# moxime/joint-vae

Hardware: NVIDIA B200
Metric: train_images_per_sec (higher is better)
Workload: dtype bf16

## Files before the change

### include/jvae_b200.h

```cpp
#ifndef JVAE_B200_H
#define JVAE_B200_H

#include <stdint.h>
#include <stddef.h>

#ifdef __cplusplus
extern "C" {
#endif

#define JVAE_ABI_VERSION 16

enum jvae_status {
  JVAE_OK = 0,
  JVAE_ERR_INVALID = -1,
  JVAE_ERR_CUDA = -2,
  JVAE_ERR_UNSUPPORTED = -3,
  JVAE_ERR_NOGPU = -4
};

enum jvae_dtype { JVAE_F32 = 0, JVAE_BF16 = 1 };

enum jvae_var_dim { JVAE_VAR_SCALAR = 0, JVAE_VAR_DIAG = 1, JVAE_VAR_FULL = 2 };
enum jvae_prior_kind { JVAE_PRIOR_GAUSSIAN = 0, JVAE_PRIOR_TILTED = 1, JVAE_PRIOR_UNIFORM = 2 };

// ... 93 lines not shown

int jvae_conv_gather_gemm(const void* in, int N, int H, int W, int Cin, int ld_in, const void* wmat, int Cout_pad, int ldw,
                          int ntaps, const int16_t* tap_dy, const int16_t* tap_dx, int in_stride, int Hq, int Wq,
                          void* out, int Ho, int Wo, int Cout, int ld_out, int out_sy, int out_sx, int out_oy, int out_ox,
                          const float* bias, int act, double* stats, void* stream);
typedef struct jvae_bn_reduce {
  const void* y;
  int32_t ld_y;
  const float* save_mean_rstd;
  const float* gamma;
  const float* beta;
  int32_t act;
} jvae_bn_reduce;
int jvae_conv_gather_gemm_bn(const void* in, int N, int H, int W, int Cin, int ld_in, const void* wmat, int Cout_pad, int ldw,
                             int ntaps, const int16_t* tap_dy, const int16_t* tap_dx, int in_stride, int Hq, int Wq,
                             void* out, int Ho, int Wo, int Cout, int ld_out, int out_sy, int out_sx, int out_oy, int out_ox,
                             const float* bias, int act, double* stats, const jvae_bn_reduce* bn, int* bn_fused, void* stream);
#define JVAE_NOT_COVERED 1
int jvae_conv_subpixel_gemm(const void* in, int N, int H, int W, int Cin, int ld_in, const void* wmat, int Cout_pad, int ldw,
                            int nphases, const int16_t* phase_ntaps, const int16_t* phase_oy, const int16_t* phase_ox,
                            const int16_t* tap_dy, const int16_t* tap_dx, int Hq, int Wq, void* out, int Ho, int Wo, int Cout,
                            int ld_out, int out_s, const float* bias, int act, double* stats, void* stream);
int jvae_conv_halo_emulate(const float* in, int N, int H, int W, int Cin, int ld_in, const float* wmat, int Cout_pad, int ldw,
                           int nphases, const int16_t* phase_ntaps, const int16_t* phase_oy, const int16_t* phase_ox, int ntaps,
                           const int16_t* tap_dy, const int16_t* tap_dx, int in_stride, int Hq, int Wq, float* out, int Ho, int Wo,
                           int Cout, int ld_out, int out_sy, int out_sx, int out_oy, int out_ox, const float* bias, int act,
                           int* info);
int jvae_conv_wgrad_emulate(const float* dy, int N, int Hq, int Wq, int Cout, int ld_dy, const float* x, int H, int W, int Cin, int ld_x,
                            int ntaps, const int16_t* tap_dy, const int16_t* tap_dx, int in_stride, float* dw, int dw_ld_tap,
                            int dw_ld_co, int dw_ld_ci, int* launches);
int jvae_conv_wgrad(const void* dy, int N, int Hq, int Wq, int Cout, int ld_dy, const void* x, int H, int W, int Cin, int ld_x,
                    int ntaps, const int16_t* tap_dy, const int16_t* tap_dx, int in_stride, float* dw, int dw_ld_tap,
                    int dw_ld_co, int dw_ld_ci, void* stream);
enum jvae_conv_kernel { JVAE_KERNEL_CONV_HALO = 1, JVAE_KERNEL_CONV_TAPBOX = 2, JVAE_KERNEL_WGRAD_HALO = 3, JVAE_KERNEL_WGRAD_TAPBOX = 4 };
int jvae_last_conv_kernel(void);


int jvae_bn_stats(const void* y, size_t P, int C, int ld, double* stats, void* stream);
int jvae_bn_apply_fwd(const void* y, size_t P, int C, int ld_y, const double* stats, const float* gamma, const float* beta,
                      float eps, float momentum, float* running_mean, float* running_var, int64_t* num_batches, int training,
                      int act, void* out, int ld_out, float* save_mean_rstd, void* stream);
int jvae_bn_bwd(const void* da, int ld_da, const void* y, int ld_y, size_t P, int C, const float* save_mean_rstd,
                const float* gamma, const float* beta, int act, double* sums, void* dy, int ld_dy, float* dgamma, float* dbeta,
                int skip_reduce, void* stream);
int jvae_act_bwd(const void* da, int ld_da, const void* a_out, int ld_a, size_t P, int C, int act, void* dy, int ld_dy,
                 float* dbias, void* stream);
int jvae_maxpool_fwd(const void* in, int N, int H, int W, int C, int ld_in, int k, int stride, void* out, int ld_out, void* stream);
int jvae_maxpool_bwd(const void* in, int N, int H, int W, int C, int ld_in, int k, int stride, const void* dout, int ld_dout,
                     void* din, int ld_din, void* stream);
int jvae_maxpool_pad_fwd(const void* in, int N, int H, int W, int C, int ld_in, int k, int stride, int pad, void* out,
                         int ld_out, void* stream);
int jvae_maxpool_pad_bwd(const void* in, int N, int H, int W, int C, int ld_in, int k, int stride, int pad, const void* dout,
                         int ld_dout, void* din, int ld_din, void* stream);
int jvae_avgpool(const void* src, int ld_src, void* dst, int ld_dst, int N, int H, int W, int C, int k, int backward,
                 void* stream);
int jvae_vsum_rows(const void* T, int ld_t, int N, int H, int W, int k, int pad, int Co, const float* bias, int act, double* stats,
                   void* out, int ld_out, void* stream);
int jvae_vstack_rows(const void* dy, int ld_dy, int N, int H, int W, int k, int pad, int Co, void* U, int ld_u, void* stream);
int jvae_add_act(const void* a, int ld_a, const void* b, int ld_b, size_t P, int C, int act, void* out, int ld_out,
                 void* stream);
int jvae_upsample2(const void* src, int ld_src, void* dst, int ld_dst, int N, int H, int W, int C, int backward, void* stream);

int jvae_cast_f32_bf16(const float* src, void* dst, size_t n, void* stream);
int jvae_cast_bf16_f32(const void* src, float* dst, size_t n, void* stream);
int jvae_im2col_bf16(const void* x, int N, int H, int W, int C, int ld_x, int ntaps, const int16_t* tap_dy, const int16_t* tap_dx,
                     int in_stride, int Hq, int Wq, void* out, int ld_out, int tap_major, void* stream);
int jvae_nchw_to_nhwc_bf16(const float* src, void* dst, int n, int c, int h, int w, int c_pad, void* stream);
int jvae_nhwc_bf16_to_nchw(const void* src, float* dst, int n, int c, int h, int w, int c_pad, void* stream);

typedef struct jvae_pack_job {
  const float* src;
  void* dst;
  int64_t s_r1, s_r0, s_t, s_c1, s_c0;
  int32_t rows, rows_pad, R0;
// ... 41 lines not shown
```

### joint-vae_b200/_native.py

```python
import ctypes
import os

import torch

_HERE = os.path.dirname(os.path.abspath(__file__))
LIB_PATH = os.path.join(_HERE, 'libjvae_sm100.so')

F32, BF16 = 0, 1
VAR_DIM = {'scalar': 0, 'diag': 1, 'full': 2}
PRIOR_KIND = {'gaussian': 0, 'tilted': 1, 'uniform': 2}
ACT = {'none': 0, 'linear': 0, 'relu': 1, 'sigmoid': 2, 'leaky': 3}
OUT_F32, IN_F32 = 0x100, 0x200
LEAKY_SLOPE = 0.01
NSCORES, NPRED = 16, 4
SCORE_INDEX = {'elbo': 0, 'max': 0, 'sum': 1, 'mean': 2, 'iws': 3, 'soft': 4, 'softkl': 4, 'zdist': 5, 'kl': 6,
               'mse': 7, 'wmse': 8, 'logits': 9, 'baseline': 10, 'hyz': 11, 'std': 12, 'softiws': 13}
PRED_INDEX = {'loss': 0, 'esty': 1, 'closest': 2, 'iws': 3}

c_void_p, c_int, c_float, c_size_t = ctypes.c_void_p, ctypes.c_int, ctypes.c_float, ctypes.c_size_t
c_u64, c_i64 = ctypes.c_uint64, ctypes.c_int64


class ElboCfg(ctypes.Structure):
    _fields_ = [(n, ctypes.c_int32) for n in
                ('B', 'L', 'K', 'C', 'D', 'xreco_dtype', 'logits_dtype', 'var_dim', 'prior_kind', 'conditional',
                 'has_xreco', 'has_logits', 'sigma_is_log', 'sigma_is_rmse')] + \
               [(n, ctypes.c_float) for n in ('beta', 'gamma_w', 'var_w', 'tau', 'alpha')] + \
               [(n, ctypes.c_int32) for n in ('prior_stats_ready', 'categorical', 'cat_group', 'sigma_per_sample')]


class BnReduce(ctypes.Structure):
    _fields_ = [('y', ctypes.c_void_p), ('ld_y', ctypes.c_int32), ('save_mean_rstd', ctypes.c_void_p),
                ('gamma', ctypes.c_void_p), ('beta', ctypes.c_void_p), ('act', ctypes.c_int32)]


class BatchCfg(ctypes.Structure):
    _fields_ = [(n, ctypes.c_int32) for n in ('H', 'W', 'C', 'out_H', 'out_W', 'crop_pad', 'flip_first', 'post_off_y',
                                              'post_off_x')]


class PackJob(ctypes.Structure):
    _fields_ = [('src', ctypes.c_void_p), ('dst', ctypes.c_void_p)] + \
               [(n, ctypes.c_int64) for n in ('s_r1', 's_r0', 's_t', 's_c1', 's_c0')] + \
               [(n, ctypes.c_int32) for n in ('rows', 'rows_pad', 'R0', 'T', 'tap_off', 'cols', 'cols_pad', 'C0', 'dst_f32',
                                              'first_block')]


class NativeError(RuntimeError):
    pass


_lib = None


def lib():
    global _lib
    if _lib is not None:
        return _lib
    if not os.path.exists(LIB_PATH):
        raise NativeError(f'{LIB_PATH} is not built: run `python -c "import __graft_entry__ as g; g.build()"` '
                          'in a container with nvcc; there is no CPU fallback')
    L = ctypes.CDLL(LIB_PATH)
    L.jvae_last_error.restype = ctypes.c_char_p
    L.jvae_abi_version.restype = c_int
    L.jvae_launch_count.restype = c_i64
    L.jvae_device_info.argtypes = [c_int, ctypes.POINTER(c_int), ctypes.POINTER(c_int), ctypes.POINTER(c_int)]
    L.jvae_elbo_workspace_bytes.restype = c_size_t
    L.jvae_elbo_workspace_bytes.argtypes = [ctypes.POINTER(ElboCfg)]
    P = c_void_p
    L.jvae_elbo_train_fwd.argtypes = [ctypes.POINTER(ElboCfg)] + [P] * 19 + [c_size_t, P]
    L.jvae_elbo_train_bwd.argtypes = [ctypes.POINTER(ElboCfg)] + [P] * 19 + [c_size_t, P]
    L.jvae_elbo_eval_fwd.argtypes = [ctypes.POINTER(ElboCfg)] + [P] * 23 + [c_size_t, P]
    L.jvae_sample_fwd.argtypes = [c_int, c_int, c_int, P, P, c_u64, c_u64, P, c_int, c_int, P, P, P, P, P, P, P]
    L.jvae_sample_bwd.argtypes = [c_int, c_int, c_int, P, P, P, P, c_int, P, P, c_int, P, P]
    L.jvae_cast_f32_bf16.argtypes = [P, P, c_size_t, P]
    L.jvae_cast_bf16_f32.argtypes = [P, P, c_size_t, P]
    L.jvae_nchw_to_nhwc_bf16.argtypes = [P, P, c_int, c_int, c_int, c_int, c_int, P]
    L.jvae_nhwc_bf16_to_nchw.argtypes = [P, P, c_int, c_int, c_int, c_int, c_int, P]
    L.jvae_grad_sqnorm.argtypes = [P, c_int, c_size_t, P, P, P, P]
    L.jvae_adam_step.argtypes = [P, P, P, P, c_int, c_size_t, P, c_float, c_float, c_float, c_float, c_float,
                                 c_float, c_int, P, P, P, P, c_float, P]
    for name in ('jvae_gemm_bf16', 'jvae_selftest'):
        if not hasattr(L, name):
            raise NativeError(f'{LIB_PATH} does not export {name}: stale build')
    L.jvae_gemm_bf16.argtypes = [c_int, c_int, c_int, c_int, P, c_int, P, c_int, P, c_int, P, P, c_int, P, c_int, P]
    L.jvae_selftest.argtypes = [c_int]
    L.jvae_probe_descriptors.argtypes = [c_int]
    L.jvae_probe_poison.argtypes = [ctypes.c_uint, P]
    L.jvae_profile_enable.argtypes = [c_int]
    L.jvae_im2col_bf16.argtypes = [P, c_int, c_int, c_int, c_int, c_int, c_int, ctypes.POINTER(ctypes.c_int16), ctypes.POINTER(ctypes.c_int16), c_int, c_int, c_int, P, c_int, c_int, P]
    L.jvae_profile_drain.argtypes = [P, P, c_int]
    I16P = ctypes.POINTER(ctypes.c_int16)
    L.jvae_conv_gather_gemm.argtypes = [P, c_int, c_int, c_int, c_int, c_int, P, c_int, c_int, c_int, I16P, I16P, c_int,
                                        c_int, c_int, P, c_int, c_int, c_int, c_int, c_int, c_int, c_int, c_int, P, c_int,
                                        P, P]
    L.jvae_conv_gather_gemm_bn.argtypes = [P, c_int, c_int, c_int, c_int, c_int, P, c_int, c_int, c_int, I16P, I16P, c_int,
                                           c_int, c_int, P, c_int, c_int, c_int, c_int, c_int, c_int, c_int, c_int, P,
                                           c_int, P, ctypes.POINTER(BnReduce), ctypes.POINTER(c_int), P]
    L.jvae_conv_wgrad.argtypes = [P, c_int, c_int, c_int, c_int, c_int, P, c_int, c_int, c_int, c_int, c_int, I16P, I16P,
                                  c_int, P, c_int, c_int, c_int, P]
    L.jvae_conv_subpixel_gemm.argtypes = [P, c_int, c_int, c_int, c_int, c_int, P, c_int, c_int, c_int, I16P, I16P, I16P, I16P,
                                          I16P, c_int, c_int, P, c_int, c_int, c_int, c_int, c_int, P, c_int, P, P]
    L.jvae_conv_wgrad_emulate.argtypes = [P, c_int, c_int, c_int, c_int, c_int, P, c_int, c_int, c_int, c_int, c_int, I16P, I16P,
                                          c_int, P, c_int, c_int, c_int, ctypes.POINTER(c_int)]
    L.jvae_conv_halo_emulate.argtypes = [P, c_int, c_int, c_int, c_int, c_int, P, c_int, c_int, c_int, I16P, I16P, I16P, c_int,
                                         I16P, I16P, c_int, c_int, c_int, P, c_int, c_int, c_int, c_int, c_int, c_int, c_int,
                                         c_int, P, c_int, ctypes.POINTER(c_int)]
    L.jvae_bn_stats.argtypes = [P, c_size_t, c_int, c_int, P, P]
    L.jvae_bn_apply_fwd.argtypes = [P, c_size_t, c_int, c_int, P, P, P, c_float, c_float, P, P, P, c_int, c_int, P, c_int,
                                    P, P]
    L.jvae_bn_bwd.argtypes = [P, c_int, P, c_int, c_size_t, c_int, P, P, P, c_int, P, P, c_int, P, P, c_int, P]
    L.jvae_act_bwd.argtypes = [P, c_int, P, c_int, c_size_t, c_int, c_int, P, c_int, P, P]
    L.jvae_maxpool_fwd.argtypes = [P, c_int, c_int, c_int, c_int, c_int, c_int, c_int, P, c_int, P]
    L.jvae_maxpool_bwd.argtypes = [P, c_int, c_int, c_int, c_int, c_int, c_int, c_int, P, c_int, P, c_int, P]
    L.jvae_upsample2.argtypes = [P, c_int, P, c_int, c_int, c_int, c_int, c_int, c_int, P]
    L.jvae_maxpool_pad_fwd.argtypes = [P, c_int, c_int, c_int, c_int, c_int, c_int, c_int, c_int, P, c_int, P]
    L.jvae_maxpool_pad_bwd.argtypes = [P, c_int, c_int, c_int, c_int, c_int, c_int, c_int, c_int, P, c_int, P, c_int, P]
    L.jvae_avgpool.argtypes = [P, c_int, P, c_int, c_int, c_int, c_int, c_int, c_int, c_int, P]
    L.jvae_add_act.argtypes = [P, c_int, P, c_int, c_size_t, c_int, c_int, P, c_int, P]
    L.jvae_vsum_rows.argtypes = [P, c_int, c_int, c_int, c_int, c_int, c_int, c_int, P, c_int, P, P, c_int, P]
    L.jvae_vstack_rows.argtypes = [P, c_int, c_int, c_int, c_int, c_int, c_int, c_int, P, c_int, P]
    L.jvae_elbo_prior_stats.argtypes = [ctypes.POINTER(ElboCfg), P, P, P, c_size_t, P]
    L.jvae_batch_u8_to_f32.argtypes = [ctypes.POINTER(BatchCfg), P, ctypes.c_longlong, P, c_int, P, P, P, P]
    L.jvae_last_conv_kernel.restype = c_int
    L.jvae_pack_job_blocks.argtypes = [ctypes.c_longlong, c_int, c_int]
    L.jvae_pack_weights.argtypes = [P, c_int, P, c_int, P]
    if L.jvae_abi_version() != 16:
        raise NativeError('ABI version mismatch between _native.py and libjvae_sm100.so')
    _lib = L
    return L

# ... 400 lines not shown
        pn = poy = pox = None
        dy, dx = taps
        T, nph = len(dy), 0
    rc = lib().jvae_conv_halo_emulate(hp(inp), N, H, W, Cin, ld_in, hp(wmat), Cout_pad, wmat.shape[1], nph, pn, poy, pox, T, dy, dx,
                                      in_stride, Hq, Wq, hp(out), Ho, Wo, Cout, ld_out, out_s[0], out_s[1], out_o[0], out_o[1],
                                      hp(bias), act, info)
    if rc == NOT_COVERED:
        return None
    check(rc)
    return list(info)


def conv_wgrad_emulate(dy, Cout, x, Cin, taps, in_stride, dw, dw_ld_tap, dw_ld_co, dw_ld_ci=1):
    for t in (dy, x, dw):
        assert t.device.type == 'cpu' and t.dtype == torch.float32 and t.is_contiguous()
    N, Hq, Wq, ld_dy = dy.shape
    _, H, W, ld_x = x.shape
    n = c_int(0)
    rc = lib().jvae_conv_wgrad_emulate(c_void_p(dy.data_ptr()), N, Hq, Wq, Cout, ld_dy, c_void_p(x.data_ptr()), H, W, Cin, ld_x,
                                       len(taps[0]), taps[0], taps[1], in_stride, c_void_p(dw.data_ptr()), dw_ld_tap, dw_ld_co,
                                       dw_ld_ci, ctypes.byref(n))
    if rc == NOT_COVERED:
        return None
    check(rc)
    return n.value


def conv_wgrad(dy, N, Hq, Wq, Cout, ld_dy, x, H, W, Cin, ld_x, taps, in_stride, dw, dw_ld_tap, dw_ld_co, dw_ld_ci=1):
    with _timed_conv(2.0 * N * Hq * Wq * len(taps[0]) * Cin * Cout):
        check(lib().jvae_conv_wgrad(rawptr(dy), N, Hq, Wq, Cout, ld_dy, rawptr(x), H, W, Cin, ld_x, len(taps[0]), taps[0],
                                    taps[1], in_stride, rawptr(dw), dw_ld_tap, dw_ld_co, dw_ld_ci, stream()))


def bn_stats(y, P, C, ld, stats):
    check(lib().jvae_bn_stats(rawptr(y), P, C, ld, rawptr(stats), stream()))


def bn_apply_fwd(y, P, C, ld_y, stats, gamma, beta, eps, momentum, running_mean, running_var, num_batches, training, act,
                 out, ld_out, save):
    check(lib().jvae_bn_apply_fwd(rawptr(y), P, C, ld_y, rawptr(stats), rawptr(gamma), rawptr(beta), float(eps),
                                  float(momentum), rawptr(running_mean), rawptr(running_var), rawptr(num_batches),
                                  int(training), act, rawptr(out), ld_out, rawptr(save), stream()))


def bn_bwd(da, ld_da, y, ld_y, P, C, save, gamma, beta, act, sums, dy, ld_dy, dgamma, dbeta, skip_reduce=False):
    check(lib().jvae_bn_bwd(rawptr(da), ld_da, rawptr(y), ld_y, P, C, rawptr(save), rawptr(gamma), rawptr(beta), act,
                            rawptr(sums), rawptr(dy), ld_dy, rawptr(dgamma), rawptr(dbeta), int(skip_reduce), stream()))


def act_bwd(da, ld_da, a_out, ld_a, P, C, act, dy, ld_dy, dbias):
    check(lib().jvae_act_bwd(rawptr(da), ld_da, rawptr(a_out), ld_a, P, C, act, rawptr(dy), ld_dy, rawptr(dbias), stream()))


def maxpool_fwd(inp, N, H, W, C, ld_in, k, stride, out, ld_out):
    check(lib().jvae_maxpool_fwd(rawptr(inp), N, H, W, C, ld_in, k, stride, rawptr(out), ld_out, stream()))


def maxpool_bwd(inp, N, H, W, C, ld_in, k, stride, dout, ld_dout, din, ld_din):
    check(lib().jvae_maxpool_bwd(rawptr(inp), N, H, W, C, ld_in, k, stride, rawptr(dout), ld_dout, rawptr(din), ld_din,
                                 stream()))


def upsample2(src, ld_src, dst, ld_dst, N, H, W, C, backward=False):
    check(lib().jvae_upsample2(rawptr(src), ld_src, rawptr(dst), ld_dst, N, H, W, C, int(backward), stream()))


# ... 29 lines not shown
```

### joint-vae_b200/conv_engine.py

```python
import os

import torch
from torch import nn

from . import _native as nat
from . import engine


def r8(n):
    return (n + 7) & ~7


def cblk_of(c):
    return 64 if c > 32 else (32 if c > 16 else 16)


def cout_pad_of(c):
    return ((c + 255) // 256) * 256 if c > 256 else ((c + 15) // 16) * 16


_ACT_CODE = {nn.ReLU: 1, nn.Sigmoid: 2, nn.Identity: 0, nn.LeakyReLU: 3}

import os as _os
FUSE_BN_REDUCE = _os.environ.get('JVAE_FUSE_BN_REDUCE', '0') == '1'
DENSE_SMALL = _os.environ.get('JVAE_CONV_DENSE_SMALL', '0') == '1'
SEP_FWD_DIRECT = _os.environ.get('JVAE_HEAD_FWD_DIRECT', '1') != '0'
IM2COL_MAXPIX = int(_os.environ.get('JVAE_CONV_IM2COL_MAXPIX', '16'))


class NativeKernels:
    act_dtype = torch.bfloat16

    @staticmethod
    def empty(shape, like, dtype=torch.bfloat16):
        return torch.empty(shape, dtype=dtype, device=like.device)

    @staticmethod
    def zeros(shape, like, dtype=torch.float32):
        return torch.zeros(shape, dtype=dtype, device=like.device)

    @staticmethod
    def to_nhwc(x, c_pad):
        n, c, h, w = x.shape
        x = x.float().contiguous()
        if h * w == 1 and c_pad == c:
            return nat.cast_f32_bf16(x).view(n, 1, 1, c)
        return nat.nchw_to_nhwc_bf16(x, c_pad)

    @staticmethod
    def to_nchw(t, C):
        n, h, w, ld = t.shape
        if h * w == 1 and ld == C:
            return nat.cast_bf16_f32(t).view(n, C, 1, 1)
        return nat.nhwc_bf16_to_nchw(t, C)

    @staticmethod
    def gather(x, Cin, wmat, cout_pad, taps, in_stride, Hq, Wq, out, Cout, out_s, out_o, bias, act, stats, bn=None):
        N, H, W, ld_in = x.shape
        _, Ho, Wo, ld_out = out.shape
        return nat.conv_gather_gemm(x, N, H, W, Cin, ld_in, wmat, cout_pad, wmat.shape[1], taps, in_stride, Hq, Wq, out, Ho,
                                    Wo, Cout, ld_out, out_s, out_o, bias, act, stats, bn=bn)

    @staticmethod
    def wgrad(g, Cg, x, Cx, taps, in_stride, dw, swapped=False):
        N, Hq, Wq, ld_g = g.shape
        _, H, W, ld_x = x.shape
        T = len(taps[0])
        P = N * Hq * Wq
        small = Hq * Wq <= IM2COL_MAXPIX and Cx % 8 == 0 and Cg >= 128 and Cx >= 64 and T in (1, 4, 9, 25)
        if not swapped and small and dw.is_contiguous():
            cols = torch.empty((P, Cx * T), dtype=torch.bfloat16, device=g.device)
            nat.im2col(x, N, H, W, Cx, ld_x, taps, in_stride, Hq, Wq, cols)
            tiles = ((Cg + 127) // 128) * ((Cx * T + 127) // 128)
            ksplit = max(1, min(nat.sm_count() // tiles, (P + 511) // 512)) if tiles < 100 else 1
            nat.gemm_bf16(2, Cg, Cx * T, P, g.view(P, ld_g), ld_g, cols, Cx * T, out_f32=dw.view(Cg, Cx * T), ldd=Cx * T,
                          accumulate=ksplit if ksplit > 1 else True)
            return
        if swapped:
            nat.conv_wgrad(g, N, Hq, Wq, Cg, ld_g, x, H, W, Cx, ld_x, taps, in_stride, dw, 1, T, Cg * T)
        else:
            nat.conv_wgrad(g, N, Hq, Wq, Cg, ld_g, x, H, W, Cx, ld_x, taps, in_stride, dw, 1, Cx * T, T)

    @staticmethod
    def gemm(mode, M, N, K, a, b, bias=None, act=0, out_bf16=None, out_f32=None):
        nat.gemm_bf16(mode, M, N, K, a, a.stride(0), b, b.stride(0), bias=bias, act=act, out_bf16=out_bf16, out_f32=out_f32,
                      ldd=N)

    @staticmethod
    def phases_arg(ops):
        return nat.phases_arg(ops)

    @staticmethod
    def subpixel(x, Cin, wmat, cout_pad, phases, Hq, Wq, out, Cout, out_s, bias, act, stats):
        N, H, W, ld_in = x.shape
        _, Ho, Wo, ld_out = out.shape
        return nat.conv_subpixel_gemm(x, N, H, W, Cin, ld_in, wmat, cout_pad, wmat.shape[1], phases, Hq, Wq, out, Ho, Wo, Cout,
                                      ld_out, out_s, bias, act, stats)

    bn_stats = staticmethod(nat.bn_stats)
    bn_apply_fwd = staticmethod(nat.bn_apply_fwd)
    bn_bwd = staticmethod(nat.bn_bwd)
    act_bwd = staticmethod(nat.act_bwd)
    maxpool_fwd = staticmethod(nat.maxpool_fwd)
    maxpool_bwd = staticmethod(nat.maxpool_bwd)
    upsample2 = staticmethod(nat.upsample2)
    maxpool_pad_fwd = staticmethod(nat.maxpool_pad_fwd)
    maxpool_pad_bwd = staticmethod(nat.maxpool_pad_bwd)
    avgpool = staticmethod(nat.avgpool)
    add_act = staticmethod(nat.add_act)
    vsum_rows = staticmethod(nat.vsum_rows)
    vstack_rows = staticmethod(nat.vstack_rows)
    taps_arg = staticmethod(nat.taps_arg)


K = NativeKernels


def conv_form(k, p, s, Hq, Wq):
    taps = [(i - p, j - p) for i in range(k) for j in range(k)]
    return [dict(taps=taps, idx=list(range(k * k)), in_stride=s, Hq=Hq, Wq=Wq, out_s=(1, 1), out_o=(0, 0))]


def deconv_form(k, p, s, Ho, Wo, allow_empty=False):
    ops = []
    for fy in range(s):
        rows = [i for i in range(k) if (fy + p - i) % s == 0]
        for fx in range(s):
            cols = [j for j in range(k) if (fx + p - j) % s == 0]
            Hq, Wq = (Ho - fy + s - 1) // s, (Wo - fx + s - 1) // s
            if Hq <= 0 or Wq <= 0:
                continue
            if not rows or not cols:
                if allow_empty:
# ... 261 lines not shown
            if self.Ci % 8:
                t = torch.zeros((kk * self.Co, r8(self.Ci)), dtype=torch.bfloat16, device=w.device)
                t[:, :self.Ci] = d['bm']
                d['bm'] = t[:, :self.Ci]
            d['bias'] = b0.repeat(kk).contiguous() if b0 is not None else None
        else:
            if self.transposed:
                g_f = wd.permute(1, 2, 3, 0).reshape(self.Co, kk, self.Ci)
                g_b = wd.permute(0, 2, 3, 1).reshape(self.Ci, kk, self.Co)
            else:
                g_f = wd.permute(0, 2, 3, 1).reshape(self.Co, kk, self.Ci)
                g_b = wd.permute(1, 2, 3, 0).reshape(self.Ci, kk, self.Co)
            d['fwd'] = [pack_gather_weights(g_f, op['idx'], self.Ci) for op in self.fwd_ops]
            if self.merged_fwd:
                d['fwd_all'] = pack_gather_weights(g_f, self.fwd_all_idx, self.Ci)
            if self.dense_small:
                hw = self.H * self.W
                weff = torch.zeros((hw, self.Co, hw, self.Ci), dtype=torch.float32, device=w.device)
                for q, r, ty, tx in self.dense_pairs:
                    weff[q, :, r, :] = wd[:, :, ty, tx]
                d['dense'] = weff.view(hw * self.Co, hw * self.Ci).to(torch.bfloat16).contiguous()
                d['dense_bias'] = b0.repeat(hw).contiguous() if b0 is not None else None
            if self.separable:
                kq = self.k
                d['sep_fwd'] = pack_gather_weights(wd.permute(2, 0, 3, 1).reshape(kq * self.Co, kq, self.Ci),
                                                   list(range(kq)), self.Ci)
                d['sep_bwd'] = pack_gather_weights(wd.permute(1, 3, 2, 0).reshape(self.Ci, kq, kq * self.Co),
                                                   list(range(kq)), kq * self.Co)
            if want_bwd:
                d['bwd'] = [pack_gather_weights(g_b, op['idx'], self.Co) for op in self.dgrad_ops]
        setattr(self, slot, (key, d))
        return d

    def forward(self, x, st, training):
        N = x.shape[0]
        bn = self.bn
        bn_train = bn is not None and (training or not bn.track_running_stats)
        if bn is not None and not bn_train:
            return self._forward_folded(x, st)
        pk = self._pack()
        bias = self.conv.bias.detach() if self.conv.bias is not None else None
        fused_act = self.act if bn is None else 0
        y = K.empty((N, self.Ho, self.Wo, self.ld_y), x)
        stats = (st.pop('stats_buf', None) if bn_train else None)
        if bn_train and stats is None:
            stats = K.zeros((2, self.Co), x, torch.float64)
        if self.gemm1x1:
            kk = self.k * self.k
            a2 = x.view(N, x.shape[-1])
            K.gemm(nat.GEMM_NT, N, kk * self.Co, self.Ci, a2, pk['bm'], bias=pk['bias'], act=fused_act,
                   out_bf16=y.view(N, kk * self.Co))
            if bn_train:
                K.bn_stats(y, N * kk, self.Co, self.ld_y, stats)
        elif self.dense_small:
            hw = self.H * self.W
            K.gemm(nat.GEMM_NT, N, hw * self.Co, hw * self.Ci, x.view(N, hw * self.Ci), pk['dense'], bias=pk['dense_bias'],
                   act=fused_act, out_bf16=y.view(N, hw * self.Co))
            if bn_train:
                K.bn_stats(y, N * hw, self.Co, self.ld_y, stats)
        elif self.separable and not SEP_FWD_DIRECT:
            self._sep_forward(x, pk, bias, fused_act, stats, y)
        elif not self._merged_forward(x, pk, y, bias, fused_act, stats):
            for i, (op, wm) in enumerate(zip(self.fwd_ops, pk['fwd'])):
                K.gather(x, self.Ci, wm, wm.shape[0], self._taps(('f', i), op['taps']), op['in_stride'], op['Hq'], op['Wq'],
                         y, self.Co, op['out_s'], op['out_o'], bias, fused_act, stats)
        st['x'] = x
        if bn is None:
            st['a'] = y
            return y
        P = N * self.Ho * self.Wo
        a = K.empty((N, self.Ho, self.Wo, self.ld_a), x)
        save = K.empty((2, self.Co), x, torch.float32) if bn_train else None
        track = bn.track_running_stats and training
        K.bn_apply_fwd(y, P, self.Co, self.ld_y, stats, bn.weight.detach() if bn.affine else None,
                       bn.bias.detach() if bn.affine else None, bn.eps, bn.momentum if bn.momentum is not None else 0.1,
                       bn.running_mean if track or not bn_train else None, bn.running_var if track or not bn_train else None,
                       bn.num_batches_tracked if track else None, bn_train, self.act, a, self.ld_a, save)
        if track:
            engine.bump_stats()
        st['y'], st['save'], st['bn_train'] = y, save, bn_train
        return a

    def _merged_forward(self, x, pk, out, bias, act, stats):
        if not self.merged_fwd:
            return False
        ph = self._ctaps.get('fa')
        if ph is None:
            ph = self._ctaps['fa'] = K.phases_arg(self.fwd_ops)
        wm = pk['fwd_all']
        op = self.fwd_ops[0]
        return K.subpixel(x, self.Ci, wm, wm.shape[0], ph, op['Hq'], op['Wq'], out, self.Co, self.s, bias, act, stats)

    def _sep_forward(self, x, pk, bias, act, stats, out):
        N = x.shape[0]
        T = K.empty((N, self.H, self.W, self.sep_ld), x, torch.float32)
        wm = pk['sep_fwd']
        K.gather(x, self.Ci, wm, wm.shape[0], self._taps('sf', self.sep_fwd_taps), 1, self.H, self.W, T, self.sep_C, (1, 1),
                 (0, 0), None, nat.OUT_F32, None)
        K.vsum_rows(T, self.sep_ld, N, self.H, self.W, self.k, self.p, self.Co, bias, act | nat.IN_F32, stats, out,
                    out.shape[-1])

    def _forward_folded(self, x, st):
        N = x.shape[0]
        pk = self._pack(fold_bn=True)
        a = K.empty((N, self.Ho, self.Wo, self.ld_a), x)
        if self.gemm1x1:
            kk = self.k * self.k
            K.gemm(nat.GEMM_NT, N, kk * self.Co, self.Ci, x.view(N, x.shape[-1]), pk['bm'], bias=pk['bias'], act=self.act,
                   out_bf16=a.view(N, kk * self.Co))
        elif self.dense_small:
            hw = self.H * self.W
            K.gemm(nat.GEMM_NT, N, hw * self.Co, hw * self.Ci, x.view(N, hw * self.Ci), pk['dense'], bias=pk['dense_bias'],
                   act=self.act, out_bf16=a.view(N, hw * self.Co))
        elif self.separable and not SEP_FWD_DIRECT:
            self._sep_forward(x, pk, pk['b'], self.act, None, a)
        elif not self._merged_forward(x, pk, a, pk['b'], self.act, None):
            for i, (op, wm) in enumerate(zip(self.fwd_ops, pk['fwd'])):
                K.gather(x, self.Ci, wm, wm.shape[0], self._taps(('f', i), op['taps']), op['in_stride'], op['Hq'], op['Wq'],
                         a, self.Co, op['out_s'], op['out_o'], pk['b'], self.act, None)
        st['x'], st['a'], st['bn_train'], st['folded'] = x, a, False, True
        return a

    def backward(self, da, st, need_dx, prev_bn=None):
        x = st['x']
        N = x.shape[0]
        P = N * self.Ho * self.Wo
        bn = self.bn
        grads = {}
        folded = bool(st.get('folded'))
        if folded:
            a = st['a']
            if self.act == 0 and da.shape[-1] % 8 == 0:
                dy = da
            else:
                dy = K.zeros((N, self.Ho, self.Wo, r8(self.Co)), x, torch.bfloat16) if r8(self.Co) != self.Co \
                    else K.empty((N, self.Ho, self.Wo, self.Co), x)
                K.act_bwd(da, da.shape[-1], a, a.shape[-1], P, self.Co, self.act, dy, dy.shape[-1], None)
        elif bn is not None:
            y = st['y']
            dy = K.empty(y.shape, x)
            pre = st.get('bn_sums')
            sums = pre if pre is not None else K.empty((2, self.Co), x, torch.float64)
            dg = db = lg = lb = None
            if bn.affine:
                lg, lb = _live_grad(bn.weight, x), _live_grad(bn.bias, x)
                dg = lg if lg is not None else K.zeros((self.Co,), x)
                db = lb if lb is not None else K.zeros((self.Co,), x)
            K.bn_bwd(da, da.shape[-1], y, self.ld_y, P, self.Co, st['save'], bn.weight.detach() if bn.affine else None,
                     bn.bias.detach() if bn.affine else None, self.act, sums, dy, self.ld_y, dg, db,
                     **({'skip_reduce': True} if pre is not None else {}))
            grads['bn_w'], grads['bn_b'] = (None if lg is not None else dg), (None if lb is not None else db)
            grads['b'] = K.zeros((self.Co,), x) if (self.conv.bias is not None and
                                                     _live_grad(self.conv.bias, x) is None) else None
        else:
            lbias = _live_grad(self.conv.bias, x)
            dbias = lbias if lbias is not None else (K.zeros((self.Co,), x) if self.conv.bias is not None else None)
            if self.act == 0 and da.shape[-1] % 8 == 0:
# ... 21 lines not shown
            if need_dx:
                ldx = x.shape[-1]
                if ldx == self.Ci:
                    dx = K.empty(x.shape, x)
                    K.gemm(nat.GEMM_NN, N, self.Ci, kk * self.Co, dy2, pk['bm'], out_bf16=dx.view(N, ldx))
                else:
                    tmp = K.empty((N, self.Ci), x, torch.float32)
                    K.gemm(nat.GEMM_NN, N, self.Ci, kk * self.Co, dy2, pk['bm'], out_f32=tmp)
                    dx = K.zeros(x.shape, x, torch.bfloat16)
                    dx.view(N, ldx)[:, :self.Ci] = tmp
        elif self.dense_small:
            hw = self.H * self.W
            dy2, x2 = dy.view(N, hw * self.Co), x.view(N, hw * self.Ci)
            if not folded:
                dweff = K.empty((hw * self.Co, hw * self.Ci), x, torch.float32)
                K.gemm(nat.GEMM_TN, hw * self.Co, hw * self.Ci, N, dy2, x2, out_f32=dweff)
                dw4 = dweff.view(hw, self.Co, hw, self.Ci)
                w = self.conv.weight
                live = _live_grad(w, x)
                dw = live if live is not None else K.zeros(tuple(w.shape), x)
                for q, r, ty, tx in self.dense_pairs:
                    dw[:, :, ty, tx] += dw4[q, :, r, :]
                grads['w'] = None if live is not None else dw
            if need_dx:
                dx = K.empty(x.shape, x)
                K.gemm(nat.GEMM_NN, N, hw * self.Ci, hw * self.Co, dy2, pk['dense'], out_bf16=dx.view(N, hw * self.Ci))
        elif self.separable:
            kq = self.k
            U = K.empty((N, self.H, self.W, self.sep_ld), x)
            K.vstack_rows(dy, dy.shape[-1], N, self.H, self.W, kq, self.p, self.Co, U, self.sep_ld)
            if not folded:
                dwa = K.zeros((self.sep_C, self.Ci, kq), x)
                if cblk_of(self.sep_C) < cblk_of(min(self.Ci, 64)):
                    K.wgrad(x, self.Ci, U, self.sep_C, self._taps('sb', self.sep_bwd_taps), 1, dwa, swapped=True)
                else:
                    K.wgrad(U, self.sep_C, x, self.Ci, self._taps('sf', self.sep_fwd_taps), 1, dwa)
                upd = dwa.view(kq, self.Co, self.Ci, kq).permute(1, 2, 0, 3)
                live = _live_grad(self.conv.weight, x)
                if live is not None:
                    live.add_(upd)
                grads['w'] = None if live is not None else upd.contiguous()
            if need_dx:
                dx = K.empty(x.shape, x)
                wm = pk['sep_bwd']
                K.gather(U, self.sep_C, wm, wm.shape[0], self._taps('sb', self.sep_bwd_taps), 1, self.H, self.W, dx, self.Ci,
                         (1, 1), (0, 0), None, 0, None)
        else:
            w = self.conv.weight
            if not folded:
                live = _live_grad(w, x)
                dw = live if live is not None else K.zeros(tuple(w.shape), x)
                if self.transposed:
                    K.wgrad(x, self.Ci, dy, self.Co, self._taps('w', self.wgrad_taps), self.s, dw.view(self.Ci, self.Co, kk))
                elif self.wgrad_swapped:
                    K.wgrad(x, self.Ci, dy, self.Co, self._taps('wn', self.wgrad_taps_neg), 1, dw.view(self.Co, self.Ci, kk),
                            swapped=True)
                else:
                    K.wgrad(dy, self.Co, x, self.Ci, self._taps('w', self.wgrad_taps), self.s, dw.view(self.Co, self.Ci, kk))
                grads['w'] = None if live is not None else dw
            if need_dx:
                dx = K.zeros(x.shape, x, torch.bfloat16) if self.dgrad_sparse else K.empty(x.shape, x)
                fuse = FUSE_BN_REDUCE and prev_bn is not None and K is NativeKernels and \
                    prev_bn['y'].shape[:3] == dx.shape[:3]
                sums_prev = K.zeros((2, self.Ci), x, torch.float64) if fuse else None
                done = fuse
                for i, (op, wm) in enumerate(zip(self.dgrad_ops, pk['bwd'])):
                    r = K.gather(dy, self.Co, wm, wm.shape[0], self._taps(('b', i), op['taps']), op['in_stride'], op['Hq'],
                                 op['Wq'], dx, self.Ci, op['out_s'], op['out_o'], None, 0, sums_prev,
                                 **({'bn': prev_bn} if fuse else {}))
                    done = done and bool(r)
                if fuse and done:
                    prev_bn['sums'] = sums_prev
        out = [grads['w'], grads['b']]
        if bn is not None:
            out += [grads['bn_w'], grads['bn_b']]
        return dx, out


class PoolStep:

    def __init__(self, mod, in_shape):
        ks = mod.kernel_size if isinstance(mod.kernel_size, int) else mod.kernel_size[0]
        stv = mod.stride if isinstance(mod.stride, int) else mod.stride[0]
        pad = mod.padding if isinstance(mod.padding, int) else mod.padding[0]
        if mod.ceil_mode or mod.dilation not in (1, (1, 1)) or 2 * pad > ks:
            raise NotImplementedError('MaxPool2d with ceil_mode / dilation has no native kernel')
        self.k, self.s, self.p = ks, stv, pad
        self.general = pad != 0 or stv < ks
        self.C, self.H, self.W = in_shape
        self.Ho, self.Wo = (self.H + 2 * pad - ks) // stv + 1, (self.W + 2 * pad - ks) // stv + 1
        self.out_shape = (self.C, self.Ho, self.Wo)
# ... 216 lines not shown
            elif g[0] == 'avg':
                stp = AvgStep(g[1], shape)
            elif g[0] == 'res':
                stp = ResidualStep(g[1], shape)
            else:
                stp = UpStep(g[1], shape)
            steps.append(stp)
            shape = stp.out_shape
        self.steps = steps
        self.out_shape = shape
        self.parameters = [p for s in steps for p in s.params()]
        convs = []
        for stp in steps:
            if isinstance(stp, ConvStep):
                convs.append(stp)
            elif isinstance(stp, ResidualStep):
                convs += stp.chain + ([stp.ds] if stp.ds is not None else [])
        self.plan = PackPlan(convs)
        for c in convs:
            c.plan = self.plan

    def forward(self, x, training):
        C, H, W = self.in_shape
        N = x.shape[0]
        if K is NativeKernels and training:
            self.plan.ensure()
        t = K.to_nhwc(x.reshape(N, C, H, W), r8(C))
        state = []
        bn_steps = [s for s in self.steps if isinstance(s, ConvStep) and s.bn is not None and
                    (training or not s.bn.track_running_stats)]
        pool, off = None, 0
        if bn_steps:
            pool = K.zeros((sum(2 * s.Co for s in bn_steps),), t, torch.float64)
        for s in self.steps:
            st = {}
            if pool is not None and any(s is b for b in bn_steps):
                st['stats_buf'] = pool[off:off + 2 * s.Co].view(2, s.Co)
                off += 2 * s.Co
            t = s.forward(t, st, training)
            state.append(st)
        Co, Ho, Wo = self.out_shape
        if self.image_out and t.shape[-1] == Co:
            out = t.permute(0, 3, 1, 2)
        else:
            out = K.to_nchw(t, Co)
        return out, state, t.shape[-1]

    def backward(self, dout, state, ld_last, need_dx):
        Co, Ho, Wo = self.out_shape
        N = dout.shape[0]
        if self.image_out and ld_last == Co:
            g = dout
            if g.dtype != K.act_dtype:
                g = g.to(K.act_dtype)
            g = g.permute(0, 2, 3, 1)
            if not g.is_contiguous():
                g = g.contiguous()
        else:
            g = K.to_nhwc(dout, ld_last)
        grads = []
        for idx in range(len(self.steps) - 1, -1, -1):
            s = self.steps[idx]
            kw = {}
            prev = self.steps[idx - 1] if idx > 0 else None
            if isinstance(s, ConvStep) and isinstance(prev, ConvStep) and prev.bn is not None and \
                    state[idx - 1].get('bn_train') and not s.gemm1x1:
                pb = prev.bn
                kw['prev_bn'] = dict(y=state[idx - 1]['y'], ld_y=prev.ld_y, save=state[idx - 1]['save'],
                                     gamma=pb.weight.detach() if pb.affine else None,
                                     beta=pb.bias.detach() if pb.affine else None, act=prev.act)
            g, pg = s.backward(g, state[idx], need_dx or idx > 0, **kw)
            if 'prev_bn' in kw and kw['prev_bn'].get('sums') is not None:
# ... 56 lines not shown
```

### joint-vae_b200/csrc/common.cuh

```cuda
#pragma once
#include <cuda_runtime.h>
#include <cuda_bf16.h>
#include <cuda.h>
#include <stdint.h>
#include <stdio.h>
#include <string.h>
#include <atomic>

#include "../../include/jvae_b200.h"

namespace jvae {

void set_error(const char* fmt, ...);
extern std::atomic<long long> g_launches;
inline void count_launch(int n = 1) { g_launches.fetch_add(n, std::memory_order_relaxed); }

#define JVAE_CHECK_ARG(cond, msg)                                                   \
  do {                                                                              \
    if (!(cond)) {                                                                  \
      jvae::set_error("%s: invalid argument: %s (%s)", __func__, msg, #cond);       \
      return JVAE_ERR_INVALID;                                                      \
    }                                                                               \
  } while (0)

// ... 20 lines not shown

void* prof_begin(int tag, cudaStream_t st);
void prof_end(void* h, cudaStream_t st);

__device__ __forceinline__ float warp_sum(float v) {
#pragma unroll
  for (int o = 16; o > 0; o >>= 1) v += __shfl_xor_sync(0xffffffffu, v, o);
  return v;
}
__device__ __forceinline__ float warp_max(float v) {
#pragma unroll
  for (int o = 16; o > 0; o >>= 1) v = fmaxf(v, __shfl_xor_sync(0xffffffffu, v, o));
  return v;
}

__device__ __forceinline__ float block_sum(float v, float* red) {
  const int lane = threadIdx.x & 31, wid = threadIdx.x >> 5, nw = (blockDim.x + 31) >> 5;
  v = warp_sum(v);
  __syncthreads();
  if (lane == 0) red[wid] = v;
  __syncthreads();
  float r = (lane < nw) ? red[lane] : 0.f;
  r = warp_sum(r);
  return r;
}

__device__ __forceinline__ float bf16_lo(uint32_t u) { return __uint_as_float(u << 16); }
__device__ __forceinline__ float bf16_hi(uint32_t u) { return __uint_as_float(u & 0xffff0000u); }
__device__ __forceinline__ uint32_t pack_bf16(float a, float b) {
  __nv_bfloat162 t = __floats2bfloat162_rn(a, b);
  return *reinterpret_cast<uint32_t*>(&t);
}

__device__ __forceinline__ uint4 ld_stream16(const void* p) {
  uint4 r;
  asm volatile("ld.global.nc.L1::no_allocate.v4.u32 {%0,%1,%2,%3}, [%4];"
               : "=r"(r.x), "=r"(r.y), "=r"(r.z), "=r"(r.w) : "l"(p));
  return r;
}
__device__ __forceinline__ void st_stream16(void* p, uint4 v) {
  asm volatile("st.global.L1::no_allocate.v4.u32 [%0], {%1,%2,%3,%4};"
               :: "l"(p), "r"(v.x), "r"(v.y), "r"(v.z), "r"(v.w) : "memory");
}

}
```

### joint-vae_b200/csrc/conv.cu

```cuda
#include "tc_common.cuh"
#include <vector>
#include <algorithm>
#include <stdlib.h>

namespace jvae {

constexpr int CONV_THREADS = 192;
constexpr int CONV_MAX_TAPS = 64;
static thread_local int g_last_conv_kernel = 0;

struct ConvParams {
  int N, Hq, Wq;
  int TW, TH, NB;
  int tiles_x, tiles_y, tiles_n, num_tiles, n_tiles_n;
  int Cblk, nCk, ntaps;
  int in_stride;
  short dy[CONV_MAX_TAPS], dx[CONV_MAX_TAPS];
  int BN;
  int Ho, Wo, Cout, ldc;
  int out_sy, out_sx, out_oy, out_ox;
  int act;
  int out_f32;
  const float* bias;
  __nv_bfloat16* out;
// ... 222 lines not shown
        const int ch = i % p.cout_pad;
        const double val = s_stats[i];
        if (ch < p.Cout && val != 0.0) atomicAdd(&p.stats[(i / p.cout_pad) * p.Cout + ch], val);
      }
    }
  }
  tc_fence_before();
  __syncthreads();
  if (warp == 1) tmem_dealloc_dyn(tmem_base, p.tmem_cols);
}

constexpr int HALO_MAX_CK = 128;
struct HaloParams {
  int N, Hq, Wq;
  int RT, NBt, HHs, HWp, MT;
  int strips_x, blocks_y, blocks_n, num_boxes, n_tiles_n;
  int Cblk, ntaps, BN;
  int nkc;
  int dymin, dxmin;
  int in_stride, nplanes;
  short plane_ry[4], plane_rx[4];
  uint32_t plane_bytes;
  short dy[CONV_MAX_TAPS], dx[CONV_MAX_TAPS];
  uint32_t tap_off16[CONV_MAX_TAPS];
  int Ho, Wo, Cout, ldc, out_sy, out_sx, out_oy, out_ox, act;
  int out_f32;
  const float* bias;
  __nv_bfloat16* out;
  double* stats;
  int cout_pad;
  const __nv_bfloat16* bn_y;
  const float* bn_save; const float* bn_gamma; const float* bn_beta;
  int bn_ld, bn_act;
  uint32_t stage_bytes, box_bytes, w_tap_bytes, w_bytes, tmem_cols, acc_stride;
  int stages, resident, wstages;
  int G, nck;
  int PH;
  short ph_oy[4], ph_ox[4];
  uint4 ck[HALO_MAX_CK];
  short w_pos[CONV_MAX_TAPS];
};

__device__ __forceinline__ int2 lds_int2(uint32_t addr) {
  int2 v;
  asm volatile("ld.shared.v2.s32 {%0, %1}, [%2];" : "=r"(v.x), "=r"(v.y) : "r"(addr));
  return v;
}

__device__ __forceinline__ uint64_t desc64(uint32_t hi, uint32_t lo) {
  uint64_t d;
  asm("mov.b64 %0, {%1, %2};" : "=l"(d) : "r"(lo), "r"(hi));
  return d;
}

template <int KSTEPS, int MT>
__device__ __forceinline__ void halo_mma_box(const HaloParams& p, uint32_t d0, uint32_t a_hi, uint32_t a_lo0, uint32_t m_step16,
                                             uint32_t b_hi, uint32_t b_lo_base, uint32_t w_tap16, uint32_t idesc,
                                             uint64_t* wfull_bar, uint64_t* wempty_bar, uint32_t& ws, uint32_t& wph,
                                             uint32_t later_chunk) {
  uint32_t b_lo = b_lo_base;
  for (int t = 0; t < p.ntaps; ++t) {
    if (!p.resident) {
      mbar_wait(&wfull_bar[ws], wph);
      tc_fence_after();
      b_lo = b_lo_base + ws * w_tap16;
    }
    const uint32_t a_lo = a_lo0 + p.tap_off16[t];
    const uint32_t acc_first = (t != 0) | later_chunk;
#pragma unroll
    for (int m = 0; m < MT; ++m)
#pragma unroll
      for (int k = 0; k < KSTEPS; ++k)
        umma_bf16(d0 + (uint32_t)(m * p.BN), desc64(a_hi, a_lo + (uint32_t)m * m_step16 + 2u * k), desc64(b_hi, b_lo + 2u * k), idesc,
                  k == 0 ? acc_first : 1u);
    if (p.resident) {
      b_lo += w_tap16;
    } else {
      umma_commit(&wempty_bar[ws]);
      if (++ws == (uint32_t)p.wstages) { ws = 0; wph ^= 1; }
    }
  }
}

template <int KSTEPS>
__device__ __forceinline__ void halo_mma_box_g(const HaloParams& p, uint32_t d0, uint32_t a_hi, uint32_t a_lo0, uint32_t m_step16,
                                               uint32_t b_hi, uint32_t b_lo_base, uint32_t idesc0, uint32_t later_chunk) {
  const uint32_t gbn = (uint32_t)(p.G * p.PH * p.BN);
  for (int m = 0; m < p.MT; ++m) {
    const uint32_t a_m = a_lo0 + (uint32_t)m * m_step16;
    const uint32_t d_m = d0 + (uint32_t)m * gbn;
    for (int c = 0; c < p.nck; ++c) {
      const uint4 ck = p.ck[c];
      const uint32_t a_lo = a_m + ck.x, b_lo = b_lo_base + ck.y;
      const uint32_t d = d_m + (ck.w & 0x7fffffffu);
      const uint32_t idesc = ck.z;
      const uint32_t acc0 = ((ck.w >> 31) ^ 1u) | later_chunk;
#pragma unroll
      for (int k = 0; k < KSTEPS; ++k)
        umma_bf16(d, desc64(a_hi, a_lo + 2u * k), desc64(b_hi, b_lo + 2u * k), idesc, k == 0 ? acc0 : 1u);
    }
  }
}

template <int NCH, int MODE>
__device__ __forceinline__ void halo_epilogue_fast(const HaloParams& p, uint32_t tmem_base, uint64_t* tfull_bar, uint64_t* tempty_bar,
                                                   double* s_stats, const float* s_bias, const float* s_bn, int2* s_tab, int warp,
                                                   int lane, int nt, int box0, int box_step) {
  constexpr bool STATS = MODE != 0;
  constexpr bool BNRED = MODE == 2;
  constexpr int LC = (NCH + 1) / 2;
  const int set = (warp - 2) >> 2;
  const int q = warp & 3;
  const int mrow = q * 32 + lane;
  const int ch0 = nt * p.BN;
  const int per = p.G * p.PH;
  const int nblk = p.MT * per;
  const int c_first = NCH == 1 ? 0 : set;
  for (int i = threadIdx.x - 64; i < nblk * 16; i += 256) {
    const int blk = i >> 4;
    const int m = blk / per, r = blk - m * per;
    const int j = r / p.PH, ph = r - j * p.PH;
    const int slot = (m * 16 + (i & 15)) * p.G + j;
    const int nb = slot / p.HHs, yy = slot - nb * p.HHs;
    const bool valid = nb < p.NBt && yy < p.RT;
    s_tab[i] = make_int2(valid ? (nb * p.Ho + yy * p.out_sy + p.ph_oy[ph]) * p.Wo + p.ph_ox[ph] : -1,
                         yy | (nb << 16));
  }
  asm volatile("bar.sync 1, 256;" ::: "memory");
  float s1[STATS ? LC * 16 : 1], s2[STATS ? LC * 16 : 1];
  if (STATS) {
#pragma unroll
    for (int j = 0; j < LC * 16; ++j) s1[j] = s2[j] = 0.f;
  }
  const bool has_bias = p.bias != nullptr;
  const uint32_t sb = smem_u32(s_bias);
  const uint32_t stab = smem_u32(s_tab) + 8u * (uint32_t)(mrow >> 3);
  const bool vec_bf16 = (p.ldc & 7) == 0, vec_f32 = (p.ldc & 3) == 0;
  const bool al32 = (reinterpret_cast<uintptr_t>(p.out) & 31) == 0;
  const bool v8_bf16 = al32 && (p.ldc & 15) == 0, v8_f32 = al32 && (p.ldc & 7) == 0;
  uint32_t it = 0;
  int sx, by, mm, dsx, dby, dmm;
  {
    int t = box0;
    sx = t % p.strips_x; t /= p.strips_x;
    by = t % p.blocks_y; mm = t / p.blocks_y;
    t = box_step;
    dsx = t % p.strips_x; t /= p.strips_x;
    dby = t % p.blocks_y; dmm = t / p.blocks_y;
  }
  for (int box = box0; box < p.num_boxes; box += box_step, ++it) {
    const uint32_t acc = it & 1;
    if (it != 0) {
      sx += dsx;
      if (sx >= p.strips_x) { sx -= p.strips_x; ++by; }
      by += dby;
      if (by >= p.blocks_y) { by -= p.blocks_y; ++mm; }
      mm += dmm;
    }
    const int qx = sx * 8 + (mrow & 7);
    const bool pxok = qx < p.Wq;
    const int ylim = p.Hq - by * p.RT, nlim = p.N - mm * p.NBt;
    const size_t pix0 = ((size_t)(mm * p.NBt) * p.Ho + (size_t)(by * p.RT * p.out_sy + p.out_oy)) * p.Wo +
                        (size_t)(qx * p.out_sx + p.out_ox);
    mbar_wait(&tfull_bar[acc], (it >> 1) & 1);
    tc_fence_after();
    constexpr int BSTEP = NCH == 1 ? 2 : 1;
    int2 e_next = lds_int2(stab + 8u * (uint32_t)(NCH == 1 ? set : 0) * 16u);
    for (int blk = (NCH == 1 ? set : 0); blk < nblk; blk += BSTEP) {
      const int2 e = e_next;
      if (blk + BSTEP < nblk) e_next = lds_int2(stab + 8u * (uint32_t)(blk + BSTEP) * 16u);
      const bool ok = pxok && e.x >= 0 && (e.y & 0xffff) < ylim && (e.y >> 16) < nlim;
      if (!__any_sync(0xffffffffu, ok)) continue;
      const uint32_t t_addr = tmem_base + acc * p.acc_stride + (uint32_t)(blk * p.BN) + ((uint32_t)(q * 32) << 16);
      const size_t pix = pix0 + (size_t)(ok ? e.x : 0);
      uint4 yq[BNRED ? LC : 1][2];
      if (BNRED && ok) {
#pragma unroll
        for (int lc = 0; lc < LC; ++lc)
          if (c_first + 2 * lc < NCH && ch0 + (c_first + 2 * lc) * 16 < p.Cout) {
            const __nv_bfloat16* yp = p.bn_y + pix * (size_t)p.bn_ld + (size_t)(ch0 + (c_first + 2 * lc) * 16);
            yq[lc][0] = ld_stream16(yp);
            yq[lc][1] = ld_stream16(yp + 8);
          }
      }
      float bq[LC][16];
      if (has_bias) {
#pragma unroll
        for (int lc = 0; lc < LC; ++lc)
          if (c_first + 2 * lc < NCH) {
#pragma unroll
            for (int j = 0; j < 16; j += 4)
// ... 113 lines not shown
      int chn;
      const float t1 = warp_sum16(a, lane, &chn);
      const float t2 = warp_sum16(b, lane, &chn);
      if (c < NCH && (lane & 1) == 0 && ch0 + c * 16 + chn < p.Cout) {
        atomicAdd(&s_stats[ch0 + c * 16 + chn], (double)t1);
        atomicAdd(&s_stats[p.cout_pad + ch0 + c * 16 + chn], (double)t2);
      }
    }
    asm volatile("bar.sync 1, 256;" ::: "memory");
    const int t = threadIdx.x - 64;
    for (int i = t; i < 2 * p.cout_pad; i += 256) {
      const int ch = i % p.cout_pad;
      double val = s_stats[i];
      if (BNRED && i >= p.cout_pad && ch - ch0 >= 0 && ch - ch0 < p.BN)
        val = (double)s_bn[64 + ch - ch0] * (val - (double)s_bn[ch - ch0] * s_stats[ch]);
      if (ch < p.Cout && val != 0.0) atomicAdd(&p.stats[(i / p.cout_pad) * p.Cout + ch], val);
    }
  }
}

constexpr int HALO_THREADS = 320;
__global__ void __launch_bounds__(HALO_THREADS, 1)
conv_halo_kernel(const __grid_constant__ CUtensorMap tmap_in, const __grid_constant__ CUtensorMap tmap_w,
                 const __grid_constant__ HaloParams p) {
  extern __shared__ uint8_t smem_raw[];
  uint8_t* smem = reinterpret_cast<uint8_t*>((reinterpret_cast<uintptr_t>(smem_raw) + 1023) & ~(uintptr_t)1023);
  uint8_t* wsm = smem + (size_t)p.stages * p.stage_bytes;
  uint64_t* full_bar = reinterpret_cast<uint64_t*>(wsm + p.w_bytes);
  uint64_t* empty_bar = full_bar + 4;
  uint64_t* wfull_bar = empty_bar + 4;
  uint64_t* wempty_bar = wfull_bar + 8;
  uint64_t* tfull_bar = wempty_bar + 8;
  uint64_t* tempty_bar = tfull_bar + 2;
  uint32_t* tmem_slot = reinterpret_cast<uint32_t*>(tempty_bar + 2);
  double* s_stats = reinterpret_cast<double*>(tmem_slot + 4);
  float* s_bias = reinterpret_cast<float*>(s_stats + (p.stats ? 2 * p.cout_pad : 0));

  const int warp = threadIdx.x >> 5, lane = threadIdx.x & 31;
  const int nt = (int)blockIdx.x % p.n_tiles_n;
  float* s_bn = s_bias + 64;
  int2* s_tab = reinterpret_cast<int2*>(s_bn + 256);
  for (int i = threadIdx.x; i < p.BN; i += HALO_THREADS) {
    const int ch = nt * p.BN + i;
    s_bias[i] = (p.bias && ch < p.Cout) ? p.bias[ch] : 0.f;
    if (p.bn_y) {
      const bool live = ch < p.Cout;
      const float mean = live ? p.bn_save[ch] : 0.f, rstd = live ? p.bn_save[p.Cout + ch] : 0.f;
      const float g = (live && p.bn_gamma) ? p.bn_gamma[ch] : 1.f, b = (live && p.bn_beta) ? p.bn_beta[ch] : 0.f;
      s_bn[i] = mean; s_bn[64 + i] = rstd; s_bn[128 + i] = live ? g * rstd : 0.f; s_bn[192 + i] = live ? b - mean * g * rstd : 0.f;
    }
  }
  const int box0 = (int)blockIdx.x / p.n_tiles_n, box_step = (int)gridDim.x / p.n_tiles_n;
  const uint32_t rb = (uint32_t)p.Cblk * 2u;

  if (p.stats)
    for (int i = threadIdx.x; i < 2 * p.cout_pad; i += HALO_THREADS) s_stats[i] = 0.0;
  if (warp == 0 && lane == 0) {
    tma_prefetch_desc(&tmap_in);
    tma_prefetch_desc(&tmap_w);
    for (int s = 0; s < 4; ++s) { mbar_init(&full_bar[s], 1); mbar_init(&empty_bar[s], 1); }
    for (int s = 0; s < 8; ++s) { mbar_init(&wfull_bar[s], 1); mbar_init(&wempty_bar[s], 1); }
    for (int a = 0; a < 2; ++a) { mbar_init(&tfull_bar[a], 1); mbar_init(&tempty_bar[a], 8); }
    fence_barrier_init();
    fence_proxy_async();
  }
  if (warp == 1) tmem_alloc_dyn(tmem_slot, p.tmem_cols);
  tc_fence_before();
  __syncthreads();
  tc_fence_after();
  const uint32_t tmem_base = *tmem_slot;

  if (warp == 0) {
    if (elect_one()) {
      if (p.resident) {
        mbar_arrive_expect_tx(&wfull_bar[0], (uint32_t)(p.ntaps * p.nkc) * p.w_tap_bytes);
        for (int kc = 0; kc < p.nkc; ++kc)
          for (int t = 0; t < p.ntaps; ++t)
            tma_load_2d(wsm + (size_t)(kc * p.ntaps + (p.nck > 0 ? p.w_pos[t] : t)) * p.w_tap_bytes, &tmap_w, &wfull_bar[0],
                        (t * p.nkc + kc) * p.Cblk, nt * p.BN);
      }
      auto load_unit = [&](int box, int kc, uint32_t iu) {
        int m = box;
        const int sx = m % p.strips_x; m /= p.strips_x;
        const int by = m % p.blocks_y; m /= p.blocks_y;
        const int s = iu % p.stages;
        mbar_wait(&empty_bar[s], ((iu / p.stages) & 1) ^ 1);
        mbar_arrive_expect_tx(&full_bar[s], p.box_bytes);
        for (int pl = 0; pl < p.nplanes; ++pl)
          tma_load_4d(smem + (size_t)s * p.stage_bytes + (size_t)pl * p.plane_bytes, &tmap_in, &full_bar[s], kc * p.Cblk,
                      p.in_stride * (sx * 8 + p.dxmin) + p.plane_rx[pl], p.in_stride * (by * p.RT + p.dymin) + p.plane_ry[pl],
                      m * p.NBt);
      };
      uint32_t iu = 0, wit = 0;
      if (box0 < p.num_boxes) load_unit(box0, 0, 0);
      for (int box = box0; box < p.num_boxes; box += box_step) {
        for (int kc = 0; kc < p.nkc; ++kc, ++iu) {
          if (kc + 1 < p.nkc) load_unit(box, kc + 1, iu + 1);
          else if (box + box_step < p.num_boxes) load_unit(box + box_step, 0, iu + 1);
          if (!p.resident) {
            for (int t = 0; t < p.ntaps; ++t, ++wit) {
              const int ws = wit % p.wstages;
              mbar_wait(&wempty_bar[ws], ((wit / p.wstages) & 1) ^ 1);
              mbar_arrive_expect_tx(&wfull_bar[ws], p.w_tap_bytes);
              tma_load_2d(wsm + (size_t)ws * p.w_tap_bytes, &tmap_w, &wfull_bar[ws], (t * p.nkc + kc) * p.Cblk, nt * p.BN);
            }
          }
        }
      }
    }
  } else if (warp == 1) {
    if (elect_one()) {
      const uint32_t idesc = make_idesc_bf16(128, p.BN, false, false);
      const uint32_t swz = (p.Cblk == 64) ? SWZ_128B : (p.Cblk == 32 ? SWZ_64B : SWZ_32B);
      const uint32_t sbo_a = (uint32_t)(p.G * p.HWp) * rb, sbo_b = 8u * rb;
      const uint32_t a_hi = ((sbo_a >> 4) & 0x3fffu) | (1u << 14) | (swz << 29);
      const uint32_t b_hi = ((sbo_b >> 4) & 0x3fffu) | (1u << 14) | (swz << 29);
      const uint32_t m_step16 = (16u * sbo_a) >> 4, w_tap16 = p.w_tap_bytes >> 4;
      const int ksteps = p.Cblk >> 4;
      if (p.resident) { mbar_wait(&wfull_bar[0], 0); tc_fence_after(); }
      uint32_t it = 0, s = 0, sph = 0, ws = 0, wph = 0;
      for (int box = box0; box < p.num_boxes; box += box_step, ++it) {
        const uint32_t acc = it & 1;
        mbar_wait(&tempty_bar[acc], ((it >> 1) & 1) ^ 1);
        const uint32_t d0 = tmem_base + acc * p.acc_stride;
        const uint32_t b_lo = ((smem_u32(wsm) >> 4) & 0x3fffu) | (1u << 16);
        for (int kc = 0; kc < p.nkc; ++kc) {
          mbar_wait(&full_bar[s], sph);
          tc_fence_after();
          const uint32_t a_lo0 = ((smem_u32(smem + (size_t)s * p.stage_bytes) >> 4) & 0x3fffu) | (1u << 16);
          const uint32_t later = kc != 0;
#define HALO_BOX(KS, M) halo_mma_box<KS, M>(p, d0, a_hi, a_lo0, m_step16, b_hi, b_lo, w_tap16, idesc, wfull_bar, wempty_bar, ws, wph, later)
#define HALO_BOX_M(KS)                                                                 \
          switch (p.MT) {                                                              \
            case 1: HALO_BOX(KS, 1); break;                                            \
            case 2: HALO_BOX(KS, 2); break;                                            \
            case 3: HALO_BOX(KS, 3); break;                                            \
            case 4: HALO_BOX(KS, 4); break;                                            \
            default: HALO_BOX(KS, 5); break;                                           \
          }
          if (p.nck > 0) {
            const uint32_t idesc0 = make_idesc_bf16(128, 0, false, false);
            const uint32_t b_kc = b_lo + (uint32_t)(kc * p.ntaps) * w_tap16;
            if (ksteps == 2) halo_mma_box_g<2>(p, d0, a_hi, a_lo0, m_step16, b_hi, b_kc, idesc0, later);
            else if (ksteps == 4) halo_mma_box_g<4>(p, d0, a_hi, a_lo0, m_step16, b_hi, b_kc, idesc0, later);
            else halo_mma_box_g<1>(p, d0, a_hi, a_lo0, m_step16, b_hi, b_kc, idesc0, later);
          } else if (ksteps == 2) { HALO_BOX_M(2) } else if (ksteps == 4) { HALO_BOX_M(4) } else { HALO_BOX_M(1) }
#undef HALO_BOX_M
#undef HALO_BOX
          umma_commit(&empty_bar[s]);
          if (++s == (uint32_t)p.stages) { s = 0; sph ^= 1; }
        }
        umma_commit(&tfull_bar[acc]);
      }
    }
  } else {
#define HALO_EPI_FAST(NCH_)                                                                                                            \
    if (p.bn_y) halo_epilogue_fast<NCH_, 2>(p, tmem_base, tfull_bar, tempty_bar, s_stats, s_bias, s_bn, s_tab, warp, lane, nt, box0, box_step);    \
    else if (p.stats) halo_epilogue_fast<NCH_, 1>(p, tmem_base, tfull_bar, tempty_bar, s_stats, s_bias, s_bn, s_tab, warp, lane, nt, box0, box_step); \
    else halo_epilogue_fast<NCH_, 0>(p, tmem_base, tfull_bar, tempty_bar, s_stats, s_bias, s_bn, s_tab, warp, lane, nt, box0, box_step)
    switch (p.BN >> 4) {
      case 1: HALO_EPI_FAST(1); break;
      case 2: HALO_EPI_FAST(2); break;
      case 3: HALO_EPI_FAST(3); break;
      default: HALO_EPI_FAST(4); break;
    }
#undef HALO_EPI_FAST
  }
  tc_fence_before();
  __syncthreads();
  if (warp == 1) tmem_dealloc_dyn(tmem_base, p.tmem_cols);
}

struct WgradParams {
  int N, Hq, Wq, TW, TH, NB, tiles_x, tiles_y, tiles_n, num_tiles;
  int Cblk_y, Cblk_x;
  int Cy, Cx, ncx;
  int ntaps, tap0, taps_per_cta, in_stride;
  short dy[CONV_MAX_TAPS], dx[CONV_MAX_TAPS];
  float* dw;
  int dw_ld_tap, dw_ld_co, dw_ld_cx;
  uint32_t stage_bytes, a_bytes, tx_bytes, tmem_cols;
  int stages;
};

__global__ void __launch_bounds__(CONV_THREADS, 1)
conv_wgrad_kernel(const __grid_constant__ CUtensorMap tmap_dy, const __grid_constant__ CUtensorMap tmap_x,
                  const __grid_constant__ WgradParams p) {
  extern __shared__ uint8_t smem_raw[];
  uint8_t* smem = reinterpret_cast<uint8_t*>((reinterpret_cast<uintptr_t>(smem_raw) + 1023) & ~(uintptr_t)1023);
  uint64_t* full_bar = reinterpret_cast<uint64_t*>(smem + (size_t)p.stages * p.stage_bytes);
  uint64_t* empty_bar = full_bar + p.stages;
  uint64_t* done_bar = empty_bar + p.stages;
  uint32_t* tmem_slot = reinterpret_cast<uint32_t*>(done_bar + 1);
  const int warp = threadIdx.x >> 5, lane = threadIdx.x & 31;
  const int tap_lo = p.tap0 + blockIdx.y * p.taps_per_cta;
  const int ntap = min(p.taps_per_cta, p.ntaps - tap_lo);
  const int cy0 = ((int)blockIdx.z / p.ncx) * p.Cblk_y, cx0 = ((int)blockIdx.z % p.ncx) * p.Cblk_x;
  const int M_real = min(p.Cblk_y, p.Cy - cy0), N_real = min(p.Cblk_x, p.Cx - cx0);

// ... 78 lines not shown
          float* o = p.dw + (size_t)(tap_lo + t) * p.dw_ld_tap + (size_t)(cy0 + row) * p.dw_ld_co + (size_t)(cx0 + c0) * p.dw_ld_cx;
#pragma unroll
          for (int j = 0; j < 16; ++j)
            if (c0 + j < N_real) atomicAdd(o + (size_t)j * p.dw_ld_cx, __uint_as_float(r[j]));
        }
      }
    }
  }
  tc_fence_before();
  __syncthreads();
  if (warp == 1) tmem_dealloc_dyn(tmem_base, p.tmem_cols);
}

constexpr int WH_MAX_GROUPS = 64;
struct WHaloParams {
  int N, Hq, Wq;
  int NBt, HHs, HWp, MT, strips_x, num_boxes;
  int RT, blocks_y;
  uint32_t g_img_bytes;
  int Cblk_g, Cblk_x, ncx, Cg, Cx;
  int ngroups, groups_per_cta;
  int dymin, dxmin, ey;
  int in_stride, nplanes;
  short plane_ry[4], plane_rx[4];
  uint32_t plane_bytes;
  uint32_t grp_off16[WH_MAX_GROUPS];
  unsigned char grp_ntap[WH_MAX_GROUPS];
  unsigned char grp_nv[WH_MAX_GROUPS];
  uint32_t grp_boff16[WH_MAX_GROUPS];
  uint32_t grp_idesc[WH_MAX_GROUPS];
  unsigned short grp_col[WH_MAX_GROUPS];
  short grp_tap[WH_MAX_GROUPS][8][8];
  uint32_t g_gap_bytes;
  float* dw;
  int dw_ld_tap, dw_ld_co, dw_ld_cx;
  uint32_t x_stage_bytes, stage_bytes, x_box_bytes, g_box_bytes, tmem_cols;
  int stages;
};

__global__ void __launch_bounds__(CONV_THREADS, 1)
conv_wgrad_halo_kernel(const __grid_constant__ CUtensorMap tmap_g, const __grid_constant__ CUtensorMap tmap_x,
                       const __grid_constant__ WHaloParams p) {
  extern __shared__ uint8_t smem_raw[];
  uint8_t* smem = reinterpret_cast<uint8_t*>((reinterpret_cast<uintptr_t>(smem_raw) + 1023) & ~(uintptr_t)1023);
  uint64_t* full_bar = reinterpret_cast<uint64_t*>(smem + (size_t)p.stages * p.stage_bytes);
  uint64_t* empty_bar = full_bar + 8;
  uint64_t* done_bar = empty_bar + 8;
  uint32_t* tmem_slot = reinterpret_cast<uint32_t*>(done_bar + 1);
  const int warp = threadIdx.x >> 5, lane = threadIdx.x & 31;
  const int g_lo = (int)blockIdx.y * p.groups_per_cta;
  const int ng = min(p.groups_per_cta, p.ngroups - g_lo);
  const int cg0 = ((int)blockIdx.z / p.ncx) * p.Cblk_g, cx0 = ((int)blockIdx.z % p.ncx) * p.Cblk_x;
  const uint32_t rbx = (uint32_t)p.Cblk_x * 2u, rbg = (uint32_t)p.Cblk_g * 2u;

  for (uint32_t i = threadIdx.x; i < (uint32_t)p.stages * p.stage_bytes / 16u; i += CONV_THREADS)
    reinterpret_cast<uint4*>(smem)[i] = make_uint4(0u, 0u, 0u, 0u);
  if (warp == 0 && lane == 0) {
    tma_prefetch_desc(&tmap_g);
    tma_prefetch_desc(&tmap_x);
    for (int s = 0; s < 8; ++s) { mbar_init(&full_bar[s], 1); mbar_init(&empty_bar[s], 1); }
    mbar_init(done_bar, 1);
    fence_barrier_init();
  }
  fence_proxy_async();
  if (warp == 1) tmem_alloc_dyn(tmem_slot, p.tmem_cols);
  tc_fence_before();
  __syncthreads();
  tc_fence_after();
  const uint32_t tmem_base = *tmem_slot;

  if (warp == 0) {
    if (elect_one()) {
      uint32_t s = 0, ph = 0;
      for (int box = blockIdx.x; box < p.num_boxes; box += gridDim.x) {
        int m = box;
        const int sx = m % p.strips_x; m /= p.strips_x;
        const int by = m % p.blocks_y; const int nb = m / p.blocks_y;
        mbar_wait(&empty_bar[s], ph ^ 1);
        uint8_t* st = smem + (size_t)s * p.stage_bytes;
        mbar_arrive_expect_tx(&full_bar[s], p.x_box_bytes + p.g_box_bytes);
        for (int pl = 0; pl < p.nplanes; ++pl)
          tma_load_4d(st + (size_t)pl * p.plane_bytes, &tmap_x, &full_bar[s], cx0, p.in_stride * (sx * 8 + p.dxmin) + p.plane_rx[pl],
                      p.in_stride * (by * p.RT + p.dymin) + p.plane_ry[pl], nb * p.NBt);
        if (p.blocks_y == 1) {
          tma_load_4d(st + p.x_stage_bytes + p.g_gap_bytes, &tmap_g, &full_bar[s], cg0, sx * 8, 0, nb * p.NBt);
        } else {
          for (int i = 0; i < p.NBt; ++i)
            tma_load_4d(st + p.x_stage_bytes + p.g_gap_bytes + (size_t)i * p.HHs * 8u * rbg, &tmap_g, &full_bar[s], cg0, sx * 8,
                        by * p.RT, nb * p.NBt + i);
        }
        if (++s == (uint32_t)p.stages) { s = 0; ph ^= 1; }
      }
    }
  } else if (warp == 1) {
    if (elect_one()) {
      const uint32_t swx = (p.Cblk_x == 64) ? SWZ_128B : (p.Cblk_x == 32 ? SWZ_64B : SWZ_32B);
      const uint32_t swg = (p.Cblk_g == 64) ? SWZ_128B : (p.Cblk_g == 32 ? SWZ_64B : SWZ_32B);
      const uint32_t a_hi = (((uint32_t)p.HWp * rbx >> 4) & 0x3fffu) | (1u << 14) | (swx << 29);
      const uint32_t b_hi = (((8u * rbg) >> 4) & 0x3fffu) | (1u << 14) | (swg << 29);
      const uint32_t a_lbo = ((rbx >> 4) & 0x3fffu) << 16, b_lbo = (((8u * rbg) >> 4) & 0x3fffu) << 16;
      const uint32_t ak16 = (2u * (uint32_t)p.HWp * rbx) >> 4, bk16 = (16u * rbg) >> 4;
      const uint32_t am16 = (16u * (uint32_t)p.HWp * rbx) >> 4, bm16 = (128u * rbg) >> 4;
      const uint32_t ey_slots16 = ((uint32_t)p.ey * 8u * rbg) >> 4;
      uint32_t s = 0, ph = 0, first = 0;
      for (int box = blockIdx.x; box < p.num_boxes; box += gridDim.x) {
        mbar_wait(&full_bar[s], ph);
        tc_fence_after();
        const uint32_t sx_ = smem_u32(smem + (size_t)s * p.stage_bytes);
        const uint32_t a_lo0 = ((sx_ >> 4) & 0x3fffu) | a_lbo;
        const uint32_t b_lo0 = ((((sx_ + p.x_stage_bytes + p.g_gap_bytes) >> 4) - ey_slots16) & 0x3fffu) | b_lbo;
        for (int m = 0; m < p.MT; ++m) {
          const uint32_t b_lo = b_lo0 + (uint32_t)m * bm16;
          for (int g = 0; g < ng; ++g) {
            const uint32_t a_lo = a_lo0 + (uint32_t)m * am16 + p.grp_off16[g_lo + g];
            const uint32_t bg_lo = b_lo + p.grp_boff16[g_lo + g];
            const uint32_t idesc = p.grp_idesc[g_lo + g];
            const uint32_t d = tmem_base + (uint32_t)p.grp_col[g_lo + g];
#pragma unroll
            for (int k = 0; k < 8; ++k)
              umma_bf16(d, desc64(a_hi, a_lo + (uint32_t)k * ak16), desc64(b_hi, bg_lo + (uint32_t)k * bk16), idesc,
                        k == 0 ? first : 1u);
          }
          first = 1;
        }
        umma_commit(&empty_bar[s]);
        if (++s == (uint32_t)p.stages) { s = 0; ph ^= 1; }
      }
      umma_commit(done_bar);
    }
  } else {
    const int q = warp & 3;
    mbar_wait(done_bar, 0);
    tc_fence_after();
    const bool has_work = (int)blockIdx.x < p.num_boxes;
    const int Ng = min(p.Cblk_g, p.Cg - cg0), Nx = min(p.Cblk_x, p.Cx - cx0);
    for (int g = 0; g < ng && has_work; ++g) {
      const int ntap = p.grp_ntap[g_lo + g];
      const bool m128 = ntap * p.Cblk_x > 64;
      const int row = m128 ? q * 32 + lane : q * 16 + lane;
      const bool row_ok = m128 || lane < 16;
      const int j = row / p.Cblk_x, cx = row - j * p.Cblk_x;
      const bool live = row_ok && j < ntap && cx < Nx;
      const int nv = p.grp_nv[g_lo + g];
      for (int jv = 0; jv < nv; ++jv) {
        const int t = live ? p.grp_tap[g_lo + g][jv][j] : 0;
        for (int c0 = 0; c0 < p.Cblk_g; c0 += 16) {
          uint32_t r[16];
          tmem_ld_32x16(tmem_base + ((uint32_t)(q * 32) << 16) + (uint32_t)(p.grp_col[g_lo + g] + jv * p.Cblk_g + c0), r);
          tmem_ld_wait();
          if (live) {
            float* o = p.dw + (size_t)t * p.dw_ld_tap + (size_t)(cg0 + c0) * p.dw_ld_co + (size_t)(cx0 + cx) * p.dw_ld_cx;
#pragma unroll
            for (int i = 0; i < 16; ++i)
              if (c0 + i < Ng) atomicAdd(o + (size_t)i * p.dw_ld_co, __uint_as_float(r[i]));
          }
        }
      }
    }
  }
  tc_fence_before();
  __syncthreads();
  if (warp == 1) tmem_dealloc_dyn(tmem_base, p.tmem_cols);
}

static int pow2_floor(int v) { int p = 1; while (p * 2 <= v) p *= 2; return p; }
static int pow2_ceil(int v) { int p = 1; while (p < v) p *= 2; return p; }

static void tile_shape(int Hq, int Wq, int* TW, int* TH, int* NB) {
  int tw = pow2_floor(Wq); if (tw > 128) tw = 128;
  if (tw < Wq && tw * 2 <= 128 && (tw * 2 - Wq) * 4 <= Wq) tw *= 2;
  int th = pow2_ceil(Hq); if (th > 128 / tw) th = 128 / tw;
  *TW = tw; *TH = th; *NB = 128 / (tw * th);
}

static int cblk_of(int C) { return C > 32 ? 64 : (C > 16 ? 32 : 16); }

static int act_tmap(CUtensorMap* t, const void* base, int N, int H, int W, int C, int ldc, int Cblk, int TW, int TH, int NB,
                    int stride) {
  uint64_t dims[4] = {(uint64_t)C, (uint64_t)W, (uint64_t)H, (uint64_t)N};
  uint64_t strides[3] = {(uint64_t)ldc * 2, (uint64_t)W * ldc * 2, (uint64_t)H * W * ldc * 2};
  uint32_t box[4] = {(uint32_t)Cblk, (uint32_t)(TW * stride), (uint32_t)(TH * stride), (uint32_t)NB};
  uint32_t es[4] = {1, (uint32_t)stride, (uint32_t)stride, 1};
  return make_tmap_bf16(t, base, 4, dims, strides, box, es, Cblk * 2);
}

struct PhaseSpec { int n; const int16_t* ntaps; const int16_t* oy; const int16_t* ox; };

static int try_launch_halo(const void* in, int N, int H, int W, int Cin, int ld_in, const void* wmat, int Cout_pad, int ldw,
                           int ntaps, const int16_t* tap_dy, const int16_t* tap_dx, int in_stride, int Hq, int Wq, void* out,
                           int Ho, int Wo, int Cout, int ld_out, int out_sy, int out_sx, int out_oy, int out_ox,
                           const float* bias, int act, double* stats, const jvae_bn_reduce* bn, int* bn_fused,
                           cudaStream_t stream, const PhaseSpec* phs = nullptr, HaloParams* plan_out = nullptr,
                           int force_cblk = 0, double* score_out = nullptr) {
  if (Wq < 6) return 1;
  const bool wide = Cin > 64 || Cout_pad > 64;
  if (phs && (wide || in_stride != 1 || phs->n < 2 || phs->n > 4 || bn)) return 1;
  if (wide) {
    const bool wide_on = getenv("JVAE_CONV_WIDE") && atoi(getenv("JVAE_CONV_WIDE")) != 0;
    if (!wide_on || (Cout_pad > 64 && (Cout_pad % 64) != 0) || bn) return 1;
  }
  if (bn && !(out_sy == 1 && out_sx == 1 && out_oy == 0 && out_ox == 0 && Ho == Hq && Wo == Wq)) {
    bn = nullptr; stats = nullptr;
  }
  if (!phs && !wide && force_cblk == 0 && Cin > 32 && !(getenv("JVAE_CONV_KSPLIT") && atoi(getenv("JVAE_CONV_KSPLIT")) == 0)) {
    HaloParams pa, pb;
    double sa = 0.0, sb = 0.0;
    const int ra = try_launch_halo(in, N, H, W, Cin, ld_in, wmat, Cout_pad, ldw, ntaps, tap_dy, tap_dx, in_stride, Hq, Wq, out, Ho, Wo,
                                   Cout, ld_out, out_sy, out_sx, out_oy, out_ox, bias, act, stats, bn, nullptr, stream, nullptr, &pa, 64, &sa);
    const int rb2 = try_launch_halo(in, N, H, W, Cin, ld_in, wmat, Cout_pad, ldw, ntaps, tap_dy, tap_dx, in_stride, Hq, Wq, out, Ho, Wo,
                                    Cout, ld_out, out_sy, out_sx, out_oy, out_ox, bias, act, stats, bn, nullptr, stream, nullptr, &pb, 32, &sb);
    if (ra < 0) return ra;
    const int pick = (rb2 == 0 && (ra != 0 || sb > 1.15 * sa)) ? 32 : 64;
    if (score_out) *score_out = pick == 32 ? sb : sa;
    return try_launch_halo(in, N, H, W, Cin, ld_in, wmat, Cout_pad, ldw, ntaps, tap_dy, tap_dx, in_stride, Hq, Wq, out, Ho, Wo, Cout,
                           ld_out, out_sy, out_sx, out_oy, out_ox, bias, act, stats, bn, bn_fused, stream, nullptr, plan_out, pick, nullptr);
  }
  HaloParams p;
  memset(&p, 0, sizeof(p));
  p.PH = 1;
  const int st = in_stride;
  int tey[CONV_MAX_TAPS], tex[CONV_MAX_TAPS], tpl[CONV_MAX_TAPS];
  int dymin = 1 << 20, dymax = -(1 << 20), dxmin = 1 << 20, dxmax = -(1 << 20);
  p.in_stride = st; p.nplanes = 0;
  for (int t = 0; t < ntaps; ++t) {
    p.dy[t] = tap_dy[t]; p.dx[t] = tap_dx[t];
    const int ry = ((tap_dy[t] % st) + st) % st, rx = ((tap_dx[t] % st) + st) % st;
    tey[t] = (tap_dy[t] - ry) / st; tex[t] = (tap_dx[t] - rx) / st;
    int pl = -1;
    for (int i = 0; i < p.nplanes; ++i)
      if (p.plane_ry[i] == ry && p.plane_rx[i] == rx) pl = i;
    if (pl < 0) { pl = p.nplanes++; p.plane_ry[pl] = (short)ry; p.plane_rx[pl] = (short)rx; }
    tpl[t] = pl;
    dymin = min(dymin, tey[t]); dymax = max(dymax, tey[t]);
    dxmin = min(dxmin, tex[t]); dxmax = max(dxmax, tex[t]);
  }
  const int ey = dymax - dymin, ex = dxmax - dxmin;
  if (ey > 16 || ex > 16) return 1;
  p.N = N; p.Hq = Hq; p.Wq = Wq; p.dymin = dymin; p.dxmin = dxmin;
  p.Cblk = force_cblk ? force_cblk : cblk_of(Cin > 64 ? 64 : Cin); p.ntaps = ntaps;
  p.nkc = (Cin + p.Cblk - 1) / p.Cblk;
  p.BN = Cout_pad > 64 ? 64 : Cout_pad; p.n_tiles_n = Cout_pad / p.BN;
  const uint32_t rb = (uint32_t)p.Cblk * 2u;
  p.HWp = 8 + ex;
  p.RT = Hq <= 32 ? Hq : 32;
  p.HHs = p.RT + ey;
  p.w_tap_bytes = (uint32_t)p.BN * rb;
  const uint32_t budget = 200u * 1024u;
  const uint32_t stats_bytes = stats ? 2u * (uint32_t)Cout_pad * 8u : 0u;
  const uint32_t w_res = (uint32_t)ntaps * p.w_tap_bytes * (uint32_t)(wide ? 1 : p.nkc);
// ... 181 lines not shown
      ++nck;
    };
    std::vector<int> fresh_u;
    for (int jn = 0; jn < p.G;) {
      const int u = jn + cols[0].e_hi;
      fresh_u.push_back(u);
      jn = min(p.G - 1, u - cols[0].e_lo) + 1;
    }
    for (int u : fresh_u) add_chunk(0, u, 1);
    for (size_t ci = 0; ci < cols.size(); ++ci)
      for (int u = cols[ci].e_lo; u <= cols[ci].e_hi + p.G - 1; ++u) {
        if (ci == 0 && std::find(fresh_u.begin(), fresh_u.end(), u) != fresh_u.end()) continue;
        if (nck >= HALO_MAX_CK) return 1;
        add_chunk(ci, u, 0);
      }
    p.nck = nck;
    if ((((uint32_t)pos * p.w_tap_bytes) >> 4) > 0xffffu) return 1;
  }
  p.box_bytes = (uint32_t)p.nplanes * (uint32_t)(p.NBt * p.HHs) * p.HWp * rb;
  {
    const uint32_t bud = budget + (p.G > 1 ? 20u * 1024u : 0u);
    p.stages = (int)((bud - p.w_bytes - stats_bytes - 1792u - (uint32_t)(p.MT * p.G * p.PH) * 128u) / p.stage_bytes);
  }
  if (p.stages > 4) p.stages = 4;
  if (p.stages < 2) return 1;
  p.acc_stride = (uint32_t)(p.MT * p.G * p.PH * p.BN);
  p.tmem_cols = (uint32_t)pow2_ceil(2 * p.acc_stride < 32 ? 32 : 2 * p.acc_stride);
  p.strips_x = (Wq + 7) / 8; p.blocks_y = (Hq + p.RT - 1) / p.RT; p.blocks_n = (N + p.NBt - 1) / p.NBt;
  p.num_boxes = p.strips_x * p.blocks_y * p.blocks_n;
  p.Ho = Ho; p.Wo = Wo; p.Cout = Cout; p.ldc = ld_out;
  p.out_sy = out_sy; p.out_sx = out_sx; p.out_oy = out_oy; p.out_ox = out_ox;
  p.act = act & 0xff; p.out_f32 = (act & JVAE_OUT_F32) ? 1 : 0;
  p.bias = bias; p.out = reinterpret_cast<__nv_bfloat16*>(out); p.stats = stats; p.cout_pad = Cout_pad;
  if (plan_out) { *plan_out = p; return JVAE_OK; }
  CUtensorMap tin, tw;
  if (bn) {
    p.bn_y = reinterpret_cast<const __nv_bfloat16*>(bn->y); p.bn_ld = bn->ld_y; p.bn_save = bn->save_mean_rstd;
    p.bn_gamma = bn->gamma; p.bn_beta = bn->beta; p.bn_act = bn->act;
    if ((bn->ld_y % 8) != 0) { set_error("jvae_conv_gather_gemm_bn: bn.ld_y must be a multiple of 8"); return JVAE_ERR_INVALID; }
    if (!stats) { set_error("jvae_conv_gather_gemm_bn: the sums need the stats buffer"); return JVAE_ERR_INVALID; }
  }
  {
    uint64_t dims[4] = {(uint64_t)Cin, (uint64_t)W, (uint64_t)H, (uint64_t)N};
    uint64_t strides[3] = {(uint64_t)ld_in * 2, (uint64_t)W * ld_in * 2, (uint64_t)H * W * ld_in * 2};
    uint32_t box[4] = {(uint32_t)p.Cblk, (uint32_t)(p.HWp * st), (uint32_t)(p.HHs * st), (uint32_t)p.NBt};
    uint32_t es[4] = {1u, (uint32_t)st, (uint32_t)st, 1u};
    if (box[1] > 256 || box[2] > 256) return 1;
    int rc = make_tmap_bf16(&tin, in, 4, dims, strides, box, es, p.Cblk * 2);
    if (rc) return rc;
    const int Ktot = ntaps * p.nkc * p.Cblk;
    uint64_t wd[2] = {(uint64_t)Ktot, (uint64_t)Cout_pad};
    uint64_t ws[1] = {(uint64_t)ldw * 2};
    uint32_t wbox[2] = {(uint32_t)p.Cblk, (uint32_t)p.BN};
    if (ldw < Ktot) { set_error("jvae_conv_gather_gemm: weight matrix row shorter than taps*Cblk"); return JVAE_ERR_INVALID; }
    rc = make_tmap_bf16(&tw, wmat, 2, wd, ws, wbox, nullptr, p.Cblk * 2);
    if (rc) return rc;
  }
  const size_t tab_bytes = (size_t)p.MT * p.G * p.PH * 16 * sizeof(int2);
  const size_t smem = (size_t)p.stages * p.stage_bytes + p.w_bytes + 512 + stats_bytes +
                      256 + 1024 + 1024 + tab_bytes;
  if (smem > 227u * 1024u) return 1;
  static bool attr = false;
  if (!attr) {
    JVAE_CUDA(cudaFuncSetAttribute(conv_halo_kernel, cudaFuncAttributeMaxDynamicSharedMemorySize, 227 * 1024));
    attr = true;
  }
  int grid = p.num_boxes * p.n_tiles_n < sm_count() ? p.num_boxes * p.n_tiles_n : (sm_count() / p.n_tiles_n) * p.n_tiles_n;
  if (grid < p.n_tiles_n) return 1;
  void* prof = prof_begin(JVAE_PROF_CONV_HALO, stream);
  conv_halo_kernel<<<grid, HALO_THREADS, smem, stream>>>(tin, tw, p);
  prof_end(prof, stream);
  JVAE_LAUNCH_CHECK();
  g_last_conv_kernel = JVAE_KERNEL_CONV_HALO;
  if (bn && bn_fused) *bn_fused = 1;
  return JVAE_OK;
}

static int try_launch_wgrad_halo(const void* g, int N, int Hq, int Wq, int Cg, int ld_g, const void* x, int H, int W, int Cx,
                                 int ld_x, int ntaps, const int16_t* tap_dy, const int16_t* tap_dx, int in_stride, float* dw,
                                 int dw_ld_tap, int dw_ld_co, int dw_ld_cx, cudaStream_t stream, const int* tap_ids = nullptr,
                                 bool dry_run = false, WHaloParams* plan_out = nullptr) {
  if (Wq < 6) return 1;
  WHaloParams p;
  memset(&p, 0, sizeof(p));
  const int st = in_stride;
  std::vector<int> tey(ntaps), tex(ntaps), tpl(ntaps);
  int dymin = 1 << 20, dymax = -(1 << 20), dxmin = 1 << 20, dxmax = -(1 << 20);
  p.in_stride = st; p.nplanes = 0;
  for (int t = 0; t < ntaps; ++t) {
    const int ry = ((tap_dy[t] % st) + st) % st, rx = ((tap_dx[t] % st) + st) % st;
    tey[t] = (tap_dy[t] - ry) / st; tex[t] = (tap_dx[t] - rx) / st;
    int pl = -1;
    for (int i = 0; i < p.nplanes; ++i)
      if (p.plane_ry[i] == ry && p.plane_rx[i] == rx) pl = i;
    if (pl < 0) { pl = p.nplanes++; p.plane_ry[pl] = (short)ry; p.plane_rx[pl] = (short)rx; }
    tpl[t] = pl;
    dymin = min(dymin, tey[t]); dymax = max(dymax, tey[t]);
    dxmin = min(dxmin, tex[t]); dxmax = max(dxmax, tex[t]);
  }
  const int ey = dymax - dymin, ex = dxmax - dxmin;
  if (ey > 16 || ex > 16) return 1;
  p.N = N; p.Hq = Hq; p.Wq = Wq; p.dymin = dymin; p.dxmin = dxmin;
  p.Cg = Cg; p.Cx = Cx;
  p.Cblk_g = cblk_of(Cg > 64 ? 64 : Cg); p.Cblk_x = cblk_of(Cx > 64 ? 64 : Cx);
  const int ncg = (Cg + p.Cblk_g - 1) / p.Cblk_g;
  p.ncx = (Cx + p.Cblk_x - 1) / p.Cblk_x;
  const uint32_t rbx = (uint32_t)p.Cblk_x * 2u, rbg = (uint32_t)p.Cblk_g * 2u;
  p.RT = Hq <= 32 ? Hq : 32; p.blocks_y = (Hq + p.RT - 1) / p.RT;
  p.HWp = 8 + ex; p.HHs = p.RT + ey;
  const int tpm = 128 / p.Cblk_x;
  p.ey = ey;
  std::vector<int> tap_at((size_t)(ey + 1) * (ex + 1), -1);
  bool want = (cblk_of(Cg > 64 ? 64 : Cg) == 32 && ey + 1 >= 4) || (ey + 1 == 3 && Hq * Wq <= 64 && Cg >= 128);
  if (const char* e = getenv("JVAE_WGRAD_VSTACK")) want = atoi(e) != 0;
  bool full = want && st == 1 && p.nplanes == 1 && ntaps == (ey + 1) * (ex + 1);
// ... 68 lines not shown
    cols_max = max(cols_max, col);
  }
  p.tmem_cols = (uint32_t)pow2_ceil(cols_max < 32 ? 32 : cols_max);
  p.g_gap_bytes = ((uint32_t)E * 8u * rbg + 1023u) & ~1023u;
  p.ey = E;
  const uint32_t budget = 200u * 1024u;
  double best = 0.0;
  for (int nbt = 1; nbt <= 16 && nbt <= N; ++nbt) {
    const int S = nbt * p.HHs, MT = full ? (S + 15) / 16 : (S - ey + 15) / 16;
    const uint32_t plane = ((uint32_t)(16 * MT + ey + 1) * p.HWp * rbx + 1023u) & ~1023u;
    const uint32_t xs = plane * (uint32_t)p.nplanes;
    const uint32_t gs = p.g_gap_bytes + (((uint32_t)(16 * MT > S ? 16 * MT : S) * 8u * rbg + 1023u) & ~1023u);
    if (2u * (xs + gs) + 1024u > budget) break;
    if (nbt * p.HHs > 256) break;
    const double eff = (double)(nbt * p.RT) / (16.0 * MT);
    if (eff > best + 0.02) {
      best = eff; p.NBt = nbt; p.MT = MT; p.x_stage_bytes = xs; p.stage_bytes = xs + gs; p.plane_bytes = plane;
    }
  }
  if (best <= 0.0) return 1;
  if ((size_t)p.stage_bytes >= (1u << 18)) return 1;
  for (int gi = 0; gi < ngr && !full; ++gi) {
    const int t0 = grp_first[gi];
    p.grp_off16[gi] = ((uint32_t)tpl[t0] * p.plane_bytes + (uint32_t)((tey[t0] - dymin) * p.HWp + (tex[t0] - dxmin)) * rbx) >> 4;
  }
  p.x_box_bytes = (uint32_t)p.nplanes * (uint32_t)(p.NBt * p.HHs) * p.HWp * rbx;
  p.g_box_bytes = (uint32_t)(p.NBt * (p.blocks_y == 1 ? p.HHs : p.RT)) * 8u * rbg;
  p.stages = (int)((budget - 1024u) / p.stage_bytes);
  if (p.stages > 6) p.stages = 6;
  if (p.stages < 2) return 1;
  p.strips_x = (Wq + 7) / 8;
  p.num_boxes = p.strips_x * p.blocks_y * ((N + p.NBt - 1) / p.NBt);
  p.dw = dw; p.dw_ld_tap = dw_ld_tap; p.dw_ld_co = dw_ld_co; p.dw_ld_cx = dw_ld_cx;
  if (plan_out) *plan_out = p;
  if (dry_run) return JVAE_OK;
  CUtensorMap tg, tx;
  {
    uint64_t dg[4] = {(uint64_t)Cg, (uint64_t)Wq, (uint64_t)Hq, (uint64_t)N};
    uint64_t sg[3] = {(uint64_t)ld_g * 2, (uint64_t)Wq * ld_g * 2, (uint64_t)Hq * Wq * ld_g * 2};
    uint32_t bg[4] = {(uint32_t)p.Cblk_g, 8u, (uint32_t)(p.blocks_y == 1 ? p.HHs : p.RT), (uint32_t)(p.blocks_y == 1 ? p.NBt : 1)};
    int rc = make_tmap_bf16(&tg, g, 4, dg, sg, bg, nullptr, p.Cblk_g * 2);
    if (rc) return rc;
    uint64_t dx[4] = {(uint64_t)Cx, (uint64_t)W, (uint64_t)H, (uint64_t)N};
    uint64_t sx[3] = {(uint64_t)ld_x * 2, (uint64_t)W * ld_x * 2, (uint64_t)H * W * ld_x * 2};
    uint32_t bx[4] = {(uint32_t)p.Cblk_x, (uint32_t)(p.HWp * st), (uint32_t)(p.HHs * st), (uint32_t)p.NBt};
    uint32_t esx[4] = {1u, (uint32_t)st, (uint32_t)st, 1u};
    if (bx[1] > 256 || bx[2] > 256) return 1;
    rc = make_tmap_bf16(&tx, x, 4, dx, sx, bx, esx, p.Cblk_x * 2);
    if (rc) return rc;
  }
  const int nz = ncg * p.ncx;
  if (nz > 65535) return 1;
  int gx = (sm_count() + ysplit * nz - 1) / (ysplit * nz);
  if (gx < 1) gx = 1;
  if (gx > p.num_boxes) gx = p.num_boxes;
  const size_t smem = (size_t)p.stages * p.stage_bytes + 256 + 1024;
  static bool attr = false;
  if (!attr) {
    JVAE_CUDA(cudaFuncSetAttribute(conv_wgrad_halo_kernel, cudaFuncAttributeMaxDynamicSharedMemorySize, 227 * 1024));
    attr = true;
  }
  void* prof = prof_begin(JVAE_PROF_WGRAD_HALO, stream);
  conv_wgrad_halo_kernel<<<dim3(gx, ysplit, nz), CONV_THREADS, smem, stream>>>(tg, tx, p);
  prof_end(prof, stream);
  JVAE_LAUNCH_CHECK();
  g_last_conv_kernel = JVAE_KERNEL_WGRAD_HALO;
  return JVAE_OK;
}


static void wgrad_plan_emulate(const WHaloParams& p, const float* g, int ld_g, const float* x, int H, int W, int ld_x, float* dw) {
  const int ncg = (p.Cg + p.Cblk_g - 1) / p.Cblk_g;
  const size_t plane_rows = p.plane_bytes / ((size_t)p.Cblk_x * 2u);
  const size_t x_rows = plane_rows * p.nplanes;
  const int gap_slots = (int)(p.g_gap_bytes / (8u * (uint32_t)p.Cblk_g * 2u));
  const size_t g_slots = (size_t)gap_slots + (size_t)((p.stage_bytes - p.x_stage_bytes - p.g_gap_bytes) / (8u * (uint32_t)p.Cblk_g * 2u));
  std::vector<float> sx(x_rows * p.Cblk_x), sg(g_slots * 8 * p.Cblk_g);
  const float qnan = nanf("");
  for (int zg = 0; zg < ncg; ++zg)
    for (int zx = 0; zx < p.ncx; ++zx) {
      const int cg0 = zg * p.Cblk_g, cx0 = zx * p.Cblk_x;
      std::vector<double> D((size_t)p.ngroups * 128 * 8 * p.Cblk_g, 0.0);
      for (int box = 0; box < p.num_boxes; ++box) {
        int m0 = box;
        const int bx = m0 % p.strips_x; m0 /= p.strips_x;
        const int by = m0 % p.blocks_y; const int nb = m0 / p.blocks_y;
        std::fill(sx.begin(), sx.end(), 0.f);
        std::fill(sg.begin(), sg.end(), 0.f);
        for (int pl = 0; pl < p.nplanes; ++pl)
// ... 111 lines not shown
  p.stage_bytes = (p.tx_bytes + 1023u) & ~1023u;
  p.stages = (int)((200u * 1024u - stats_bytes) / p.stage_bytes);
  if (p.stages > 12) p.stages = 12;
  JVAE_CHECK_ARG(p.stages >= 2, "tile too large for shared memory");
  p.tmem_cols = (uint32_t)pow2_ceil(2 * p.BN < 32 ? 32 : 2 * p.BN);
  CUtensorMap tin, tw;
  int rc = act_tmap(&tin, in, N, H, W, Cin, ld_in, p.Cblk, p.TW, p.TH, p.NB, in_stride);
  if (rc) return rc;
  {
    const int Ktot = ntaps * p.nCk * p.Cblk;
    uint64_t dims[2] = {(uint64_t)Ktot, (uint64_t)Cout_pad};
    uint64_t strides[1] = {(uint64_t)ldw * 2};
    uint32_t box[2] = {(uint32_t)p.Cblk, (uint32_t)p.BN};
    JVAE_CHECK_ARG(ldw >= Ktot, "weight matrix row shorter than taps*chunks*Cblk");
    rc = make_tmap_bf16(&tw, wmat, 2, dims, strides, box, nullptr, p.Cblk * 2);
    if (rc) return rc;
  }
  const size_t smem = (size_t)p.stages * p.stage_bytes + 256 + stats_bytes + 1024;
  static bool attr = false;
  if (!attr) {
    JVAE_CUDA(cudaFuncSetAttribute(conv_gather_gemm_kernel, cudaFuncAttributeMaxDynamicSharedMemorySize, 227 * 1024));
    attr = true;
  }
  ConvParams pk = p;
  int grid = p.num_tiles < sm_count() ? p.num_tiles : sm_count();
  void* prof = prof_begin(JVAE_PROF_CONV_TAPBOX, (cudaStream_t)stream);
  conv_gather_gemm_kernel<<<grid, TAPBOX_THREADS, smem, (cudaStream_t)stream>>>(tin, tw, pk);
  prof_end(prof, (cudaStream_t)stream);
  JVAE_LAUNCH_CHECK();
  g_last_conv_kernel = JVAE_KERNEL_CONV_TAPBOX;
  return JVAE_OK;
}

int jvae_conv_subpixel_gemm(const void* in, int N, int H, int W, int Cin, int ld_in, const void* wmat, int Cout_pad, int ldw,
                            int nphases, const int16_t* phase_ntaps, const int16_t* phase_oy, const int16_t* phase_ox,
                            const int16_t* tap_dy, const int16_t* tap_dx, int Hq, int Wq, void* out, int Ho, int Wo, int Cout,
                            int ld_out, int out_s, const float* bias, int act, double* stats, void* stream) {
  JVAE_CHECK_ARG(in && wmat && out && tap_dy && tap_dx && phase_ntaps && phase_oy && phase_ox, "null pointer");
  JVAE_CHECK_ARG(nphases >= 1 && nphases <= 4, "1..4 phases");
  int ntaps = 0;
  for (int i = 0; i < nphases; ++i) {
    JVAE_CHECK_ARG(phase_ntaps[i] >= 1, "every phase needs a tap");
    JVAE_CHECK_ARG(phase_oy[i] >= 0 && phase_oy[i] < out_s && phase_ox[i] >= 0 && phase_ox[i] < out_s, "phase offset outside the stride");
    ntaps += phase_ntaps[i];
  }
  JVAE_CHECK_ARG(ntaps <= CONV_MAX_TAPS, "at most 64 taps over all phases");
  JVAE_CHECK_ARG((ld_in % 8) == 0 && (ldw % 8) == 0, "input / weight channel strides must be multiples of 8");
  JVAE_CHECK_ARG(ld_out >= Cout, "ld_out < Cout");
  JVAE_CHECK_ARG((Cout_pad % 16) == 0 && Cout_pad >= 16 && Cout_pad >= Cout, "Cout_pad must be a multiple of 16, >= Cout");
  JVAE_CHECK_ARG((((uintptr_t)in | (uintptr_t)wmat | (uintptr_t)out) & 15) == 0, "16-byte alignment");
  JVAE_CHECK_ARG(out_s >= 1 && (Hq - 1) * out_s + out_s <= Ho && (Wq - 1) * out_s + out_s <= Wo, "phase grid larger than the output");
  static const bool off = (getenv("JVAE_CONV_V1") != nullptr) || (getenv("JVAE_CONV_MERGE_PHASES") && atoi(getenv("JVAE_CONV_MERGE_PHASES")) == 0);
  if (off) return JVAE_NOT_COVERED;
  PhaseSpec ps = {nphases, phase_ntaps, phase_oy, phase_ox};
  const int rc = try_launch_halo(in, N, H, W, Cin, ld_in, wmat, Cout_pad, ldw, ntaps, tap_dy, tap_dx, 1, Hq, Wq, out, Ho, Wo, Cout,
                                 ld_out, out_s, out_s, 0, 0, bias, act, stats, nullptr, nullptr, (cudaStream_t)stream, &ps);
  return rc > 0 ? JVAE_NOT_COVERED : rc;
}

int jvae_conv_wgrad(const void* dy, int N, int Hq, int Wq, int Cout, int ld_dy, const void* x, int H, int W, int Cin, int ld_x,
                    int ntaps, const int16_t* tap_dy, const int16_t* tap_dx, int in_stride, float* dw, int dw_ld_tap,
                    int dw_ld_co, int dw_ld_ci, void* stream) {
  JVAE_CHECK_ARG(dy && x && dw && tap_dy && tap_dx, "null pointer");
  JVAE_CHECK_ARG(ntaps >= 1 && ntaps <= CONV_MAX_TAPS, "1..64 taps");
  JVAE_CHECK_ARG((ld_dy % 8) == 0 && (ld_x % 8) == 0, "channel strides must be multiples of 8");
  JVAE_CHECK_ARG(in_stride == 1 || in_stride == 2, "input stride 1 or 2");
  static const bool force_v1 = getenv("JVAE_CONV_V1") != nullptr;
  if (!force_v1) {
    const int rc = try_launch_wgrad_halo(dy, N, Hq, Wq, Cout, ld_dy, x, H, W, Cin, ld_x, ntaps, tap_dy, tap_dx, in_stride, dw,
                                         dw_ld_tap, dw_ld_co, dw_ld_ci, (cudaStream_t)stream);
    if (rc <= 0) return rc;
    static const bool split_off = getenv("JVAE_WGRAD_PLANE_SPLIT") && atoi(getenv("JVAE_WGRAD_PLANE_SPLIT")) == 0;
    if (in_stride == 2 && !split_off) {
      std::vector<int16_t> sdy[4], sdx[4];
      std::vector<int> ids[4];
      for (int t = 0; t < ntaps; ++t) {
        const int pl = (((tap_dy[t] % 2) + 2) % 2) * 2 + (((tap_dx[t] % 2) + 2) % 2);
        sdy[pl].push_back(tap_dy[t]); sdx[pl].push_back(tap_dx[t]); ids[pl].push_back(t);
      }
      bool covered = true;
      for (int pass = 0; pass < 2 && covered; ++pass)
        for (int pl = 0; pl < 4; ++pl) {
          if (ids[pl].empty()) continue;
          const int r2 = try_launch_wgrad_halo(dy, N, Hq, Wq, Cout, ld_dy, x, H, W, Cin, ld_x, (int)ids[pl].size(), sdy[pl].data(),
                                               sdx[pl].data(), 2, dw, dw_ld_tap, dw_ld_co, dw_ld_ci, (cudaStream_t)stream,
                                               ids[pl].data(), pass == 0);
          if (r2 < 0) return r2;
          if (r2 > 0) { covered = false; break; }
        }
      if (covered) return JVAE_OK;
    }
  }
  WgradParams p;
  memset(&p, 0, sizeof(p));
  p.N = N; p.Hq = Hq; p.Wq = Wq;
  tile_shape(Hq, Wq, &p.TW, &p.TH, &p.NB);
  p.tiles_x = (Wq + p.TW - 1) / p.TW; p.tiles_y = (Hq + p.TH - 1) / p.TH; p.tiles_n = (N + p.NB - 1) / p.NB;
  p.num_tiles = p.tiles_x * p.tiles_y * p.tiles_n;
  p.Cblk_y = cblk_of(Cout); p.Cblk_x = cblk_of(Cin);
  p.ntaps = ntaps; p.in_stride = in_stride;
  for (int t = 0; t < ntaps; ++t) { p.dy[t] = tap_dy[t]; p.dx[t] = tap_dx[t]; }
  p.dw = dw; p.dw_ld_tap = dw_ld_tap; p.dw_ld_co = dw_ld_co; p.dw_ld_cx = dw_ld_ci;
  p.a_bytes = 128u * 64u * 2u;
  p.stage_bytes = p.a_bytes + 128u * (uint32_t)p.Cblk_x * 2u;
  p.stage_bytes = (p.stage_bytes + 1023u) & ~1023u;
  p.tx_bytes = 128u * (uint32_t)p.Cblk_y * 2u + 128u * (uint32_t)p.Cblk_x * 2u;
  p.stages = (int)((200u * 1024u) / p.stage_bytes);
  if (p.stages > 8) p.stages = 8;
  p.taps_per_cta = 512 / p.Cblk_x;
  if (p.taps_per_cta > ntaps) p.taps_per_cta = ntaps;
  const int tap_groups = (ntaps + p.taps_per_cta - 1) / p.taps_per_cta;
  p.tmem_cols = (uint32_t)pow2_ceil(p.taps_per_cta * p.Cblk_x < 32 ? 32 : p.taps_per_cta * p.Cblk_x);
  CUtensorMap tdy, tx;
  static bool attr = false;
  if (!attr) {
    JVAE_CUDA(cudaFuncSetAttribute(conv_wgrad_kernel, cudaFuncAttributeMaxDynamicSharedMemorySize, 227 * 1024));
    attr = true;
  }
  const size_t smem = (size_t)p.stages * p.stage_bytes + 256 + 1024;
  const int ncy = (Cout + p.Cblk_y - 1) / p.Cblk_y;
  p.ncx = (Cin + p.Cblk_x - 1) / p.Cblk_x;
  p.Cy = Cout; p.Cx = Cin;
  const int nz = ncy * p.ncx;
  JVAE_CHECK_ARG(nz <= 65535, "too many channel blocks");
  int gx = (2 * sm_count() + tap_groups * nz - 1) / (tap_groups * nz);
// ... 442 lines not shown
```

### joint-vae_b200/csrc/gemm.cu

```cuda
#include "tc_common.cuh"
#include <mutex>

namespace jvae {

constexpr int GEMM_BM = 128;
constexpr int GEMM_BK = 64;
constexpr int GEMM_THREADS = 192;

struct GemmParams {
  int M, N, K, ldd, act, accumulate;
  int ksplit;
  int stages;
  const float* bias;
  __nv_bfloat16* out_bf16;
  float* out_f32;
};

template <int BN>
struct GemmSmem {
  static constexpr int A_BYTES = GEMM_BM * GEMM_BK * 2;
  static constexpr int B_BYTES = BN * GEMM_BK * 2;
  static constexpr int STAGE_BYTES = A_BYTES + B_BYTES;
  static constexpr int STAGES = (BN == 128) ? 6 : 8;
  static constexpr int BAR_OFFSET = STAGES * STAGE_BYTES;
// ... 163 lines not shown
#pragma unroll
          for (int j = 0; j < 32; j += 8) {
            uint4 t;
            t.x = pack_bf16(v[j], v[j + 1]); t.y = pack_bf16(v[j + 2], v[j + 3]);
            t.z = pack_bf16(v[j + 4], v[j + 5]); t.w = pack_bf16(v[j + 6], v[j + 7]);
            *reinterpret_cast<uint4*>(o + j) = t;
          }
        } else {
          for (int j = 0; j < 32; ++j)
            if (n0 + c0 + j < p.N) o[j] = __float2bfloat16(v[j]);
        }
      }
    }
  }
  tc_fence_before();
  __syncthreads();
  if (warp == 1) tmem_dealloc<BN>(tmem_base);
}

PFN_cuTensorMapEncodeTiled_v12000 get_tmap_encode() {
  static PFN_cuTensorMapEncodeTiled_v12000 fn = nullptr;
  static std::once_flag once;
  std::call_once(once, [] {
    void* p = nullptr;
    cudaDriverEntryPointQueryResult q;
    if (cudaGetDriverEntryPoint("cuTensorMapEncodeTiled", &p, cudaEnableDefault, &q) == cudaSuccess &&
        q == cudaDriverEntryPointSuccess)
      fn = reinterpret_cast<PFN_cuTensorMapEncodeTiled_v12000>(p);
  });
  return fn;
}

int make_tmap_bf16(CUtensorMap* out, const void* base, int rank, const uint64_t* dims, const uint64_t* strides_bytes,
                   const uint32_t* box, const uint32_t* elem_strides, int swizzle_bytes) {
  auto enc = get_tmap_encode();
  if (!enc) {
    set_error("cuTensorMapEncodeTiled is not available from this driver");
    return JVAE_ERR_CUDA;
  }
  CUtensorMapSwizzle sw = CU_TENSOR_MAP_SWIZZLE_NONE;
  if (swizzle_bytes == 128) sw = CU_TENSOR_MAP_SWIZZLE_128B;
  else if (swizzle_bytes == 64) sw = CU_TENSOR_MAP_SWIZZLE_64B;
  else if (swizzle_bytes == 32) sw = CU_TENSOR_MAP_SWIZZLE_32B;
  cuuint64_t gd[5], gs[5];
  cuuint32_t bx[5], es[5];
  for (int i = 0; i < rank; ++i) {
    gd[i] = dims[i];
    bx[i] = box[i];
    es[i] = elem_strides ? elem_strides[i] : 1;
    if (i > 0) gs[i - 1] = strides_bytes[i - 1];
  }
  CUresult r = enc(out, CU_TENSOR_MAP_DATA_TYPE_BFLOAT16, (cuuint32_t)rank, const_cast<void*>(base), gd, gs, bx, es,
                   CU_TENSOR_MAP_INTERLEAVE_NONE, sw, CU_TENSOR_MAP_L2_PROMOTION_L2_256B,
                   CU_TENSOR_MAP_FLOAT_OOB_FILL_NONE);
  if (r != CUDA_SUCCESS) {
    set_error("cuTensorMapEncodeTiled failed (CUresult %d): rank %d dims [%llu,%llu,..] stride0 %llu box [%u,%u,..]", (int)r,
              rank, (unsigned long long)dims[0], (unsigned long long)(rank > 1 ? dims[1] : 0),
              (unsigned long long)(rank > 1 ? strides_bytes[0] : 0), box[0], rank > 1 ? box[1] : 0);
    return JVAE_ERR_CUDA;
  }
  return JVAE_OK;
}

static int operand_tmap(CUtensorMap* t, const void* base, bool mn_major, int R, int K, int ld, int rows_box) {
  uint64_t dims[2], strides[1];
  uint32_t box[2];
  if (!mn_major) {
    dims[0] = (uint64_t)K; dims[1] = (uint64_t)R;
    box[0] = GEMM_BK; box[1] = (uint32_t)rows_box;
  } else {
    dims[0] = (uint64_t)R; dims[1] = (uint64_t)K;
    box[0] = 64; box[1] = GEMM_BK;
  }
  strides[0] = (uint64_t)ld * 2;
  return make_tmap_bf16(t, base, 2, dims, strides, box, nullptr, 128);
}

template <int BN, bool A_MN, bool B_MN>
static int launch_gemm(const CUtensorMap& ta, const CUtensorMap& tb, const GemmParams& p, cudaStream_t st) {
  using S = GemmSmem<BN>;
  static bool attr_done = false;
  if (!attr_done) {
    JVAE_CUDA(cudaFuncSetAttribute(gemm_bf16_kernel<BN, A_MN, B_MN>, cudaFuncAttributeMaxDynamicSharedMemorySize, S::TOTAL));
    attr_done = true;
  }
  dim3 grid((p.M + GEMM_BM - 1) / GEMM_BM, (p.N + BN - 1) / BN, p.ksplit > 1 ? p.ksplit : 1);
  GemmParams q = p;
// ... 55 lines not shown
```

### joint-vae_b200/csrc/norm.cu

```cuda
#include "common.cuh"
#include <mutex>
#include <unordered_map>
#include <initializer_list>

namespace jvae {

constexpr int NORM_MAX_THREADS = 256;

template <int V> struct Vec;
template <> struct Vec<8> {
  static __device__ __forceinline__ void load(const __nv_bfloat16* p, float (&v)[8]) {
    const uint4 u = *reinterpret_cast<const uint4*>(p);
    v[0] = bf16_lo(u.x); v[1] = bf16_hi(u.x); v[2] = bf16_lo(u.y); v[3] = bf16_hi(u.y);
    v[4] = bf16_lo(u.z); v[5] = bf16_hi(u.z); v[6] = bf16_lo(u.w); v[7] = bf16_hi(u.w);
  }
  static __device__ __forceinline__ void store(__nv_bfloat16* p, const float (&v)[8]) {
    uint4 u;
    u.x = pack_bf16(v[0], v[1]); u.y = pack_bf16(v[2], v[3]); u.z = pack_bf16(v[4], v[5]); u.w = pack_bf16(v[6], v[7]);
    *reinterpret_cast<uint4*>(p) = u;
  }
};
template <int V> struct Raw;
template <> struct Raw<8> {
  typedef uint4 T;
  static __device__ __forceinline__ T load(const __nv_bfloat16* p) { return ld_stream16(p); }
  static __device__ __forceinline__ T zero() { return make_uint4(0u, 0u, 0u, 0u); }
  static __device__ __forceinline__ void unpack(const T& u, float (&v)[8]) {
    v[0] = bf16_lo(u.x); v[1] = bf16_hi(u.x); v[2] = bf16_lo(u.y); v[3] = bf16_hi(u.y);
    v[4] = bf16_lo(u.z); v[5] = bf16_hi(u.z); v[6] = bf16_lo(u.w); v[7] = bf16_hi(u.w);
  }
};
template <> struct Raw<1> {
  typedef float T;
  static __device__ __forceinline__ T load(const __nv_bfloat16* p) { return __bfloat162float(*p); }
  static __device__ __forceinline__ T zero() { return 0.f; }
  static __device__ __forceinline__ void unpack(const T& u, float (&v)[1]) { v[0] = u; }
};
template <> struct Vec<1> {
  static __device__ __forceinline__ void load(const __nv_bfloat16* p, float (&v)[1]) { v[0] = __bfloat162float(*p); }
  static __device__ __forceinline__ void store(__nv_bfloat16* p, const float (&v)[1]) { *p = __float2bfloat16(v[0]); }
};

struct Geo {
  int nchunk, ppb, threads, grid;
};
static Geo make_geo(size_t P, int C, int V, int blocks_per_sm = 8) {
  Geo g;
  g.nchunk = C / V;
  g.ppb = NORM_MAX_THREADS / g.nchunk;
  if (g.ppb < 1) g.ppb = 1;
  g.threads = g.nchunk * g.ppb;
  size_t want = (P + g.ppb - 1) / g.ppb;
  const size_t cap = (size_t)sm_count() * blocks_per_sm;
  g.grid = (int)(want < cap ? (want ? want : 1) : cap);
  return g;
}

__device__ __forceinline__ float act_fwd(float z, int act) {
  if (act == JVAE_ACT_RELU) return fmaxf(z, 0.f);
  if (act == JVAE_ACT_SIGMOID) return 1.f / (1.f + __expf(-z));
  if (act == JVAE_ACT_LEAKY) return z > 0.f ? z : JVAE_LEAKY_SLOPE * z;
  return z;
}
__device__ __forceinline__ float act_grad_z(float z, int act) {
  if (act == JVAE_ACT_RELU) return z > 0.f ? 1.f : 0.f;
  if (act == JVAE_ACT_SIGMOID) { const float s = 1.f / (1.f + __expf(-z)); return s * (1.f - s); }
  if (act == JVAE_ACT_LEAKY) return z > 0.f ? 1.f : JVAE_LEAKY_SLOPE;
  return 1.f;
}

template <int V, int NK>
__device__ __forceinline__ void block_channel_reduce(float (&acc)[NK][V], int chunk, int C, double* s_acc, double* gout) {
  for (int i = threadIdx.x; i < NK * C; i += blockDim.x) s_acc[i] = 0.0;
  __syncthreads();
  const int nchunk = C / V;
  const bool fold = nchunk < 32 && (nchunk & (nchunk - 1)) == 0 && (blockDim.x & 31) == 0;
  if (fold) {
#pragma unroll
    for (int k = 0; k < NK; ++k)
#pragma unroll
      for (int j = 0; j < V; ++j) {
        float v = acc[k][j];
        for (int off = nchunk; off < 32; off <<= 1) v += __shfl_xor_sync(0xffffffffu, v, off);
        acc[k][j] = v;
      }
  }
  if (!fold || (threadIdx.x & 31) < nchunk) {
#pragma unroll
    for (int k = 0; k < NK; ++k)
#pragma unroll
      for (int j = 0; j < V; ++j) atomicAdd(&s_acc[k * C + chunk * V + j], (double)acc[k][j]);
  }
  __syncthreads();
  for (int i = threadIdx.x; i < NK * C; i += blockDim.x) atomicAdd(&gout[i], s_acc[i]);
}

// ... 15 lines not shown
  extern __shared__ double s_acc[];
  const int chunk = threadIdx.x % nchunk, pl = threadIdx.x / nchunk;
  float acc[2][V];
#pragma unroll
  for (int j = 0; j < V; ++j) acc[0][j] = acc[1][j] = 0.f;
  constexpr int U = 4;
  const size_t step = (size_t)gridDim.x * ppb;
  for (size_t p0 = (size_t)blockIdx.x * ppb + pl; p0 < P; p0 += U * step) {
    float v[U][V];
#pragma unroll
    for (int u = 0; u < U; ++u) {
      const size_t p = p0 + u * step;
      if (p < P) {
        Vec<V>::load(y + p * ld + chunk * V, v[u]);
      } else {
#pragma unroll
        for (int j = 0; j < V; ++j) v[u][j] = 0.f;
      }
    }
#pragma unroll
    for (int u = 0; u < U; ++u)
#pragma unroll
      for (int j = 0; j < V; ++j) { acc[0][j] += v[u][j]; acc[1][j] += v[u][j] * v[u][j]; }
  }
  block_channel_reduce<V, 2>(acc, chunk, C, s_acc, stats);
}

struct BnFwd {
  const __nv_bfloat16* y; __nv_bfloat16* out;
  size_t P; int C, ld_y, ld_out, nchunk, ppb, act, training;
  const double* stats; const float* gamma; const float* beta;
  float* running_mean; float* running_var; long long* num_batches; float* save;
  float eps, momentum;
};

template <int V>
__global__ void __launch_bounds__(NORM_MAX_THREADS) bn_apply_fwd_kernel(const BnFwd a) {
  const int chunk = threadIdx.x % a.nchunk, pl = threadIdx.x / a.nchunk;
  float scale[V], shift[V];
#pragma unroll
  for (int j = 0; j < V; ++j) {
    const int c = chunk * V + j;
    float mean, rstd;
    if (a.training) {
      const double inv = 1.0 / (double)a.P;
      const double mean_d = a.stats[c] * inv;
      mean = (float)mean_d;
      const float var = fmaxf((float)(a.stats[a.C + c] * inv - mean_d * mean_d), 0.f);
      rstd = rsqrtf(var + a.eps);
      if (blockIdx.x == 0 && pl == 0) {
        a.save[c] = mean; a.save[a.C + c] = rstd;
        if (a.running_mean) {
          const float unb = a.P > 1 ? var * (float)a.P / (float)(a.P - 1) : var;
          a.running_mean[c] = (1.f - a.momentum) * a.running_mean[c] + a.momentum * mean;
          a.running_var[c] = (1.f - a.momentum) * a.running_var[c] + a.momentum * unb;
        }
      }
    } else {
      mean = a.running_mean[c];
      rstd = rsqrtf(a.running_var[c] + a.eps);
    }
    const float g = a.gamma ? a.gamma[c] : 1.f, b = a.beta ? a.beta[c] : 0.f;
    scale[j] = g * rstd;
    shift[j] = b - mean * scale[j];
  }
  if (a.training && a.num_batches && blockIdx.x == 0 && threadIdx.x == 0) *a.num_batches += 1;
  constexpr int U = 4;
  const size_t step = (size_t)gridDim.x * a.ppb;
  for (size_t p0 = (size_t)blockIdx.x * a.ppb + pl; p0 < a.P; p0 += U * step) {
    typename Raw<V>::T yr[U];
#pragma unroll
    for (int u = 0; u < U; ++u) {
      const size_t p = p0 + u * step;
      yr[u] = p < a.P ? Raw<V>::load(a.y + p * a.ld_y + chunk * V) : Raw<V>::zero();
    }
#pragma unroll
    for (int u = 0; u < U; ++u) {
      const size_t p = p0 + u * step;
      if (p >= a.P) break;
      float v[V];
      Raw<V>::unpack(yr[u], v);
#pragma unroll
      for (int j = 0; j < V; ++j) v[j] = act_fwd(fmaf(v[j], scale[j], shift[j]), a.act);
      Vec<V>::store(a.out + p * a.ld_out + chunk * V, v);
    }
  }
}

constexpr int BN_REDUCE_BLOCKS = 3;
struct BnBwd {
  const __nv_bfloat16* da; const __nv_bfloat16* y; __nv_bfloat16* dy;
  size_t P; int C, ld_da, ld_y, ld_dy, nchunk, ppb, act;
  const float* save; const float* gamma; const float* beta;
  double* sums;
  float* dgamma; float* dbeta;
};

template <int V>
__global__ void __launch_bounds__(NORM_MAX_THREADS, BN_REDUCE_BLOCKS) bn_bwd_reduce_kernel(const BnBwd a) {
// ... 103 lines not shown
}
__device__ __forceinline__ void narrow_store_row(__nv_bfloat16* base, size_t p, int ld, int C, const float (&v)[8]) {
  if (ld == 8) {
    Vec<8>::store(base + p * 8, v);
  } else {
#pragma unroll
    for (int j = 0; j < 8; ++j)
      if (j < ld) base[p * ld + j] = __float2bfloat16(j < C ? v[j] : 0.f);
  }
}
template <int NK>
__device__ __forceinline__ void narrow_reduce(float (&acc)[NK][8], int C, double* s_acc, double* gout) {
  for (int i = threadIdx.x; i < NK * 8; i += blockDim.x) s_acc[i] = 0.0;
  __syncthreads();
#pragma unroll
  for (int k = 0; k < NK; ++k)
#pragma unroll
    for (int j = 0; j < 8; ++j) {
      float v = acc[k][j];
      for (int off = 16; off > 0; off >>= 1) v += __shfl_xor_sync(0xffffffffu, v, off);
      if ((threadIdx.x & 31) == 0 && j < C) atomicAdd(&s_acc[k * 8 + j], (double)v);
    }
  __syncthreads();
  for (int i = threadIdx.x; i < NK * 8; i += blockDim.x)
    if ((i & 7) < C) atomicAdd(&gout[(i >> 3) * C + (i & 7)], s_acc[i]);
}

__global__ void __launch_bounds__(NORM_MAX_THREADS) bn_apply_fwd_narrow_kernel(const BnFwd a) {
  float scale[8], shift[8];
#pragma unroll
  for (int c = 0; c < 8; ++c) {
    scale[c] = shift[c] = 0.f;
    if (c >= a.C) continue;
    float mean, rstd;
    if (a.training) {
      const double inv = 1.0 / (double)a.P;
      const double mean_d = a.stats[c] * inv;
      mean = (float)mean_d;
      const float var = fmaxf((float)(a.stats[a.C + c] * inv - mean_d * mean_d), 0.f);
      rstd = rsqrtf(var + a.eps);
      if (blockIdx.x == 0 && threadIdx.x == 0) {
        a.save[c] = mean; a.save[a.C + c] = rstd;
        if (a.running_mean) {
          const float unb = a.P > 1 ? var * (float)a.P / (float)(a.P - 1) : var;
          a.running_mean[c] = (1.f - a.momentum) * a.running_mean[c] + a.momentum * mean;
          a.running_var[c] = (1.f - a.momentum) * a.running_var[c] + a.momentum * unb;
        }
      }
    } else {
      mean = a.running_mean[c];
      rstd = rsqrtf(a.running_var[c] + a.eps);
    }
    const float g = a.gamma ? a.gamma[c] : 1.f, b = a.beta ? a.beta[c] : 0.f;
    scale[c] = g * rstd;
    shift[c] = b - mean * scale[c];
  }
  if (a.training && a.num_batches && blockIdx.x == 0 && threadIdx.x == 0) *a.num_batches += 1;
  constexpr int U = 4;
  const size_t step = (size_t)gridDim.x * blockDim.x;
  for (size_t p0 = (size_t)blockIdx.x * blockDim.x + threadIdx.x; p0 < a.P; p0 += U * step) {
    uint4 yr[U];
#pragma unroll
    for (int u = 0; u < U; ++u) yr[u] = p0 + u * step < a.P ? ld_stream16(a.y + (p0 + u * step) * 8) : make_uint4(0u, 0u, 0u, 0u);
#pragma unroll
    for (int u = 0; u < U; ++u) {
      const size_t p = p0 + u * step;
      if (p >= a.P) break;
      float v[8];
      Raw<8>::unpack(yr[u], v);
#pragma unroll
      for (int j = 0; j < 8; ++j) v[j] = j < a.C ? act_fwd(fmaf(v[j], scale[j], shift[j]), a.act) : 0.f;
      narrow_store_row(a.out, p, a.ld_out, a.C, v);
    }
  }
}

__global__ void __launch_bounds__(NORM_MAX_THREADS, BN_REDUCE_BLOCKS) bn_bwd_reduce_narrow_kernel(const BnBwd a) {
  __shared__ double s_acc[16];
  float scale[8], shift[8], acc[2][8];
#pragma unroll
  for (int c = 0; c < 8; ++c) {
    scale[c] = shift[c] = 0.f; acc[0][c] = acc[1][c] = 0.f;
    if (c < a.C) {
      const float mean = a.save[c], rstd = a.save[a.C + c];
      const float g = a.gamma ? a.gamma[c] : 1.f, b = a.beta ? a.beta[c] : 0.f;
      scale[c] = g * rstd; shift[c] = b - mean * scale[c];
    }
  }
  constexpr int U = 4;
  const size_t step = (size_t)gridDim.x * blockDim.x;
// ... 549 lines not shown
  {
    std::lock_guard<std::mutex> lk(mu);
    auto it = cache.find(key);
    if (it != cache.end()) occ = it->second;
  }
  if (occ == 0) {
    if (cudaOccupancyMaxActiveBlocksPerMultiprocessor(&occ, kern, threads, smem) != cudaSuccess || occ < 1) occ = 1;
    std::lock_guard<std::mutex> lk(mu);
    cache[key] = occ;
  }
  const long long cap = (long long)occ * sm_count();
  return (int)(want < cap ? want : cap);
}

#define NORM_DISPATCH(vec, kernel, geo, smem, st, ...)                                             \
  do {                                                                                             \
    if (vec) kernel<8><<<resident_grid(kernel<8>, geo.threads, smem, geo.grid), geo.threads, smem, st>>>(__VA_ARGS__);   \
    else kernel<1><<<resident_grid(kernel<1>, geo.threads, smem, geo.grid), geo.threads, smem, st>>>(__VA_ARGS__);       \
    JVAE_LAUNCH_CHECK();                                                                           \
  } while (0)

extern "C" {

int jvae_bn_stats(const void* y, size_t P, int C, int ld, double* stats, void* stream) {
  JVAE_CHECK_ARG(y && stats && P > 0 && C > 0 && ld >= C, "bad arguments");
  const bool vec = vec_ok(C, {ld}, {y});
  JVAE_CHECK_ARG(vec ? C <= 8 * NORM_MAX_THREADS : C <= NORM_MAX_THREADS, "too many channels for this layout");
  const Geo g = make_geo(P, C, vec ? 8 : 1);
  NORM_DISPATCH(vec, bn_stats_kernel, g, 2 * C * sizeof(double), (cudaStream_t)stream,
                reinterpret_cast<const __nv_bfloat16*>(y), P, C, ld, g.nchunk, g.ppb, stats);
  return JVAE_OK;
}

int jvae_bn_apply_fwd(const void* y, size_t P, int C, int ld_y, const double* stats, const float* gamma, const float* beta,
                      float eps, float momentum, float* running_mean, float* running_var, int64_t* num_batches, int training,
                      int act, void* out, int ld_out, float* save_mean_rstd, void* stream) {
  JVAE_CHECK_ARG(y && out && P > 0 && C > 0 && ld_y >= C && ld_out >= C, "bad arguments");
  JVAE_CHECK_ARG(training ? (stats && save_mean_rstd) : (running_mean && running_var), "statistics missing");
  const bool vec = vec_ok(C, {ld_y, ld_out}, {y, out});
  JVAE_CHECK_ARG(vec ? C <= 8 * NORM_MAX_THREADS : C <= NORM_MAX_THREADS, "too many channels for this layout");
  const Geo g = make_geo(P, C, vec ? 8 : 1);
  const bool narrow = !vec && C < 8 && ld_y == 8 && ld_out == 8 &&
                      ((reinterpret_cast<uintptr_t>(y) | reinterpret_cast<uintptr_t>(out)) & 15) == 0;
  BnFwd a;
  a.y = reinterpret_cast<const __nv_bfloat16*>(y); a.out = reinterpret_cast<__nv_bfloat16*>(out);
  a.P = P; a.C = C; a.ld_y = ld_y; a.ld_out = ld_out; a.nchunk = g.nchunk; a.ppb = g.ppb; a.act = act; a.training = training;
  a.stats = stats; a.gamma = gamma; a.beta = beta; a.running_mean = running_mean; a.running_var = running_var;
  a.num_batches = reinterpret_cast<long long*>(num_batches); a.save = save_mean_rstd; a.eps = eps; a.momentum = momentum;
  if (narrow) {
    const int want = (int)((P + NORM_MAX_THREADS * 4 - 1) / (NORM_MAX_THREADS * 4));
    const int cap = sm_count() * 8;
    bn_apply_fwd_narrow_kernel<<<want < cap ? (want ? want : 1) : cap, NORM_MAX_THREADS, 0, (cudaStream_t)stream>>>(a);
    JVAE_LAUNCH_CHECK();
    return JVAE_OK;
  }
  NORM_DISPATCH(vec, bn_apply_fwd_kernel, g, 0, (cudaStream_t)stream, a);
  return JVAE_OK;
}

int jvae_bn_bwd(const void* da, int ld_da, const void* y, int ld_y, size_t P, int C, const float* save_mean_rstd,
                const float* gamma, const float* beta, int act, double* sums, void* dy, int ld_dy, float* dgamma, float* dbeta,
                int skip_reduce, void* stream) {
  JVAE_CHECK_ARG(da && y && dy && sums && save_mean_rstd && P > 0 && C > 0, "bad arguments");
  JVAE_CHECK_ARG(ld_da >= C && ld_y >= C && ld_dy >= C, "leading dimension < C");
  const bool vec = vec_ok(C, {ld_da, ld_y, ld_dy}, {da, y, dy});
  JVAE_CHECK_ARG(vec ? C <= 8 * NORM_MAX_THREADS : C <= NORM_MAX_THREADS, "too many channels for this layout");
  const Geo g = make_geo(P, C, vec ? 8 : 1);
  BnBwd a;
  a.da = reinterpret_cast<const __nv_bfloat16*>(da); a.y = reinterpret_cast<const __nv_bfloat16*>(y);
  a.dy = reinterpret_cast<__nv_bfloat16*>(dy);
  a.P = P; a.C = C; a.ld_da = ld_da; a.ld_y = ld_y; a.ld_dy = ld_dy; a.nchunk = g.nchunk; a.ppb = g.ppb; a.act = act;
  a.save = save_mean_rstd; a.gamma = gamma; a.beta = beta; a.sums = sums; a.dgamma = dgamma; a.dbeta = dbeta;
  const bool narrow = !vec && C < 8 && ld_y == 8 && ld_dy == 8 && (ld_da == 8 || ld_da < 8) &&
                      ((reinterpret_cast<uintptr_t>(y) | reinterpret_cast<uintptr_t>(dy)) & 15) == 0 &&
                      (ld_da != 8 || (reinterpret_cast<uintptr_t>(da) & 15) == 0);
  if (narrow) {
    const int want_r = (int)((P + NORM_MAX_THREADS * 4 - 1) / (NORM_MAX_THREADS * 4));
    const int want_a = (int)((P + NORM_MAX_THREADS * 2 - 1) / (NORM_MAX_THREADS * 2));
    if (!skip_reduce) {
      JVAE_CUDA(cudaMemsetAsync(sums, 0, 2 * (size_t)C * sizeof(double), (cudaStream_t)stream));
      const int cap = sm_count() * BN_REDUCE_BLOCKS;
      bn_bwd_reduce_narrow_kernel<<<want_r < cap ? (want_r ? want_r : 1) : cap, NORM_MAX_THREADS, 0, (cudaStream_t)stream>>>(a);
      JVAE_LAUNCH_CHECK();
    }
    const int cap = sm_count() * 8;
    bn_bwd_apply_narrow_kernel<<<want_a < cap ? (want_a ? want_a : 1) : cap, NORM_MAX_THREADS, 0, (cudaStream_t)stream>>>(a);
    JVAE_LAUNCH_CHECK();
    return JVAE_OK;
  }
// ... 170 lines not shown
```

### joint-vae_b200/csrc/tc_common.cuh

```cuda
#pragma once
#include "common.cuh"
#include <cudaTypedefs.h>

namespace jvae {

__device__ __forceinline__ uint32_t smem_u32(const void* p) { return (uint32_t)__cvta_generic_to_shared(p); }

__device__ __forceinline__ bool elect_one() {
  uint32_t pred = 0;
  asm volatile(
      "{\n\t"
      ".reg .pred P;\n\t"
      "elect.sync _|P, 0xffffffff;\n\t"
      "selp.u32 %0, 1, 0, P;\n\t"
      "}\n"
      : "=r"(pred));
  return pred != 0;
}

__device__ __forceinline__ void mbar_init(uint64_t* bar, uint32_t count) {
  asm volatile("mbarrier.init.shared::cta.b64 [%0], %1;" ::"r"(smem_u32(bar)), "r"(count));
}
__device__ __forceinline__ void fence_barrier_init() { asm volatile("fence.mbarrier_init.release.cluster;" ::: "memory"); }
__device__ __forceinline__ void fence_proxy_async() { asm volatile("fence.proxy.async.shared::cta;" ::: "memory"); }
// ... 91 lines not shown
      "{%0, %1, %2, %3, %4, %5, %6, %7, %8, %9, %10, %11, %12, %13, %14, %15}, [%16];"
      : "=r"(r[0]), "=r"(r[1]), "=r"(r[2]), "=r"(r[3]), "=r"(r[4]), "=r"(r[5]), "=r"(r[6]), "=r"(r[7]), "=r"(r[8]),
        "=r"(r[9]), "=r"(r[10]), "=r"(r[11]), "=r"(r[12]), "=r"(r[13]), "=r"(r[14]), "=r"(r[15])
      : "r"(taddr));
}
__device__ __forceinline__ void tmem_ld_wait() { asm volatile("tcgen05.wait::ld.sync.aligned;" ::: "memory"); }

enum : uint32_t { SWZ_NONE = 0, SWZ_128B = 2, SWZ_64B = 4, SWZ_32B = 6 };
__device__ __forceinline__ uint64_t make_smem_desc(uint32_t saddr, uint32_t lbo_bytes, uint32_t sbo_bytes, uint32_t layout) {
  uint64_t d = 0;
  d |= (uint64_t)((saddr >> 4) & 0x3fff);
  d |= (uint64_t)((lbo_bytes >> 4) & 0x3fff) << 16;
  d |= (uint64_t)((sbo_bytes >> 4) & 0x3fff) << 32;
  d |= (uint64_t)1 << 46;
  d |= (uint64_t)(layout & 7) << 61;
  return d;
}
__device__ __forceinline__ void st_global_v8(void* ptr, uint32_t a, uint32_t b, uint32_t c, uint32_t d, uint32_t e, uint32_t f,
                                             uint32_t g, uint32_t h) {
  asm volatile("st.global.v8.b32 [%0], {%1, %2, %3, %4, %5, %6, %7, %8};"
               :: "l"(ptr), "r"(a), "r"(b), "r"(c), "r"(d), "r"(e), "r"(f), "r"(g), "r"(h) : "memory");
}

__host__ __device__ constexpr uint32_t make_idesc_bf16(int M, int N, bool a_mn_major, bool b_mn_major) {
  return (1u << 4)
         | (1u << 7)
         | (1u << 10)
         | ((a_mn_major ? 1u : 0u) << 15) | ((b_mn_major ? 1u : 0u) << 16) | ((uint32_t)(N >> 3) << 17) |
         ((uint32_t)(M >> 4) << 24);
}

PFN_cuTensorMapEncodeTiled_v12000 get_tmap_encode();
int make_tmap_bf16(CUtensorMap* out, const void* base, int rank, const uint64_t* dims, const uint64_t* strides_bytes,
                   const uint32_t* box, const uint32_t* elem_strides, int swizzle_bytes);

}
```

Before: 46010.

## Apply batchnorm+activation on operand load in consumer convolutions instead of materialising

Adds a deferred batchnorm path. The producer layer only finalizes per-channel scale/shift and keeps the raw pre-BN output. Consumer forward convs (gather/subpixel) and the wgrad kernels then apply scale, shift and activation while loading operands. This removes a full read/write pass over the activation tensor per BN layer. In exchange the conv loaders do extra elementwise work, unsupported shapes fall back to materialising, and a tensor-map OOB-NaN option is added to handle padding correctly. It is enabled by default through an environment flag.

```diff
diff --git a/include/jvae_b200.h b/include/jvae_b200.h
--- a/include/jvae_b200.h
+++ b/include/jvae_b200.h
@@ -149,6 +149,23 @@
 int jvae_conv_wgrad(const void* dy, int N, int Hq, int Wq, int Cout, int ld_dy, const void* x, int H, int W, int Cin, int ld_x,
                     int ntaps, const int16_t* tap_dy, const int16_t* tap_dx, int in_stride, float* dw, int dw_ld_tap,
                     int dw_ld_co, int dw_ld_ci, void* stream);
+typedef struct jvae_bn_operand {
+  const float* scale_shift;
+  int32_t act;
+  int32_t on_dy;
+} jvae_bn_operand;
+int jvae_conv_gather_gemm_bnin(const void* in, int N, int H, int W, int Cin, int ld_in, const void* wmat, int Cout_pad, int ldw,
+                               int ntaps, const int16_t* tap_dy, const int16_t* tap_dx, int in_stride, int Hq, int Wq,
+                               void* out, int Ho, int Wo, int Cout, int ld_out, int out_sy, int out_sx, int out_oy, int out_ox,
+                               const float* bias, int act, double* stats, const jvae_bn_operand* bn_in, void* stream);
+int jvae_conv_subpixel_gemm_bnin(const void* in, int N, int H, int W, int Cin, int ld_in, const void* wmat, int Cout_pad, int ldw,
+                                 int nphases, const int16_t* phase_ntaps, const int16_t* phase_oy, const int16_t* phase_ox,
+                                 const int16_t* tap_dy, const int16_t* tap_dx, int Hq, int Wq, void* out, int Ho, int Wo, int Cout,
+                                 int ld_out, int out_s, const float* bias, int act, double* stats, const jvae_bn_operand* bn_in,
+                                 void* stream);
+int jvae_conv_wgrad_bnin(const void* dy, int N, int Hq, int Wq, int Cout, int ld_dy, const void* x, int H, int W, int Cin, int ld_x,
+                         int ntaps, const int16_t* tap_dy, const int16_t* tap_dx, int in_stride, float* dw, int dw_ld_tap,
+                         int dw_ld_co, int dw_ld_ci, const jvae_bn_operand* bn_in, void* stream);
 enum jvae_conv_kernel { JVAE_KERNEL_CONV_HALO = 1, JVAE_KERNEL_CONV_TAPBOX = 2, JVAE_KERNEL_WGRAD_HALO = 3, JVAE_KERNEL_WGRAD_TAPBOX = 4 };
 int jvae_last_conv_kernel(void);
 
@@ -157,6 +174,11 @@
 int jvae_bn_apply_fwd(const void* y, size_t P, int C, int ld_y, const double* stats, const float* gamma, const float* beta,
                       float eps, float momentum, float* running_mean, float* running_var, int64_t* num_batches, int training,
                       int act, void* out, int ld_out, float* save_mean_rstd, void* stream);
+int jvae_bn_finalize(const double* stats, size_t P, int C, const float* gamma, const float* beta, float eps, float momentum,
+                     float* running_mean, float* running_var, int64_t* num_batches, float* save_mean_rstd, float* scale_shift,
+                     void* stream);
+int jvae_bn_apply_scaled(const void* y, size_t P, int C, int ld_y, const float* scale_shift, int act, void* out, int ld_out,
+                         void* stream);
 int jvae_bn_bwd(const void* da, int ld_da, const void* y, int ld_y, size_t P, int C, const float* save_mean_rstd,
                 const float* gamma, const float* beta, int act, double* sums, void* dy, int ld_dy, float* dgamma, float* dbeta,
                 int skip_reduce, void* stream);
diff --git a/joint-vae_b200/_native.py b/joint-vae_b200/_native.py
--- a/joint-vae_b200/_native.py
+++ b/joint-vae_b200/_native.py
@@ -32,6 +32,10 @@
 class BnReduce(ctypes.Structure):
     _fields_ = [('y', ctypes.c_void_p), ('ld_y', ctypes.c_int32), ('save_mean_rstd', ctypes.c_void_p),
                 ('gamma', ctypes.c_void_p), ('beta', ctypes.c_void_p), ('act', ctypes.c_int32)]
+
+
+class BnOperand(ctypes.Structure):
+    _fields_ = [('scale_shift', ctypes.c_void_p), ('act', ctypes.c_int32), ('on_dy', ctypes.c_int32)]
 
 
 class BatchCfg(ctypes.Structure):
@@ -97,6 +101,16 @@
     L.jvae_conv_gather_gemm_bn.argtypes = [P, c_int, c_int, c_int, c_int, c_int, P, c_int, c_int, c_int, I16P, I16P, c_int,
                                            c_int, c_int, P, c_int, c_int, c_int, c_int, c_int, c_int, c_int, c_int, P,
                                            c_int, P, ctypes.POINTER(BnReduce), ctypes.POINTER(c_int), P]
+    BOP = ctypes.POINTER(BnOperand)
+    L.jvae_conv_gather_gemm_bnin.argtypes = [P, c_int, c_int, c_int, c_int, c_int, P, c_int, c_int, c_int, I16P, I16P, c_int,
+                                             c_int, c_int, P, c_int, c_int, c_int, c_int, c_int, c_int, c_int, c_int, P,
+                                             c_int, P, BOP, P]
+    L.jvae_conv_subpixel_gemm_bnin.argtypes = [P, c_int, c_int, c_int, c_int, c_int, P, c_int, c_int, c_int, I16P, I16P, I16P,
+                                               I16P, I16P, c_int, c_int, P, c_int, c_int, c_int, c_int, c_int, P, c_int, P, BOP, P]
+    L.jvae_conv_wgrad_bnin.argtypes = [P, c_int, c_int, c_int, c_int, c_int, P, c_int, c_int, c_int, c_int, c_int, I16P, I16P,
+                                       c_int, P, c_int, c_int, c_int, BOP, P]
+    L.jvae_bn_finalize.argtypes = [P, c_size_t, c_int, P, P, c_float, c_float, P, P, P, P, P, P]
+    L.jvae_bn_apply_scaled.argtypes = [P, c_size_t, c_int, c_int, P, c_int, P, c_int, P]
     L.jvae_conv_wgrad.argtypes = [P, c_int, c_int, c_int, c_int, c_int, P, c_int, c_int, c_int, c_int, c_int, I16P, I16P,
                                   c_int, P, c_int, c_int, c_int, P]
     L.jvae_conv_subpixel_gemm.argtypes = [P, c_int, c_int, c_int, c_int, c_int, P, c_int, c_int, c_int, I16P, I16P, I16P, I16P,
@@ -563,6 +577,66 @@
                                     taps[1], in_stride, rawptr(dw), dw_ld_tap, dw_ld_co, dw_ld_ci, stream()))
 
 
+def _bn_operand(bn_in, on_dy=0):
+    return BnOperand(scale_shift=bn_in['ss'].data_ptr(), act=bn_in['act'], on_dy=on_dy)
+
+
+def conv_gather_gemm_bnin(inp, N, H, W, Cin, ld_in, wmat, Cout_pad, ldw, taps, in_stride, Hq, Wq, out, Ho, Wo, Cout, ld_out,
+                          out_s, out_o, bias, act, stats, bn_in):
+    d = _bn_operand(bn_in)
+    with _timed_conv(2.0 * N * Hq * Wq * len(taps[0]) * Cin * Cout) as tc:
+        rc = lib().jvae_conv_gather_gemm_bnin(rawptr(inp), N, H, W, Cin, ld_in, rawptr(wmat), Cout_pad, ldw, len(taps[0]),
+                                              taps[0], taps[1], in_stride, Hq, Wq, rawptr(out), Ho, Wo, Cout, ld_out, out_s[0],
+                                              out_s[1], out_o[0], out_o[1], rawptr(bias), act, rawptr(stats), ctypes.byref(d),
+                                              stream())
+        if rc == NOT_COVERED:
+            tc.cancel()
+    if rc == NOT_COVERED:
+        return False
+    check(rc)
+    return True
+
+
+def conv_subpixel_gemm_bnin(inp, N, H, W, Cin, ld_in, wmat, Cout_pad, ldw, phases, Hq, Wq, out, Ho, Wo, Cout, ld_out, out_s,
+                            bias, act, stats, bn_in):
+    pn, poy, pox, dy, dx, T = phases
+    d = _bn_operand(bn_in)
+    with _timed_conv(2.0 * N * Hq * Wq * T * Cin * Cout) as tc:
+        rc = lib().jvae_conv_subpixel_gemm_bnin(rawptr(inp), N, H, W, Cin, ld_in, rawptr(wmat), Cout_pad, ldw, len(pn), pn, poy,
+                                                pox, dy, dx, Hq, Wq, rawptr(out), Ho, Wo, Cout, ld_out, out_s, rawptr(bias), act,
+                                                rawptr(stats), ctypes.byref(d), stream())
+        if rc == NOT_COVERED:
+            tc.cancel()
+    if rc == NOT_COVERED:
+        return False
+    check(rc)
+    return True
+
+
+def conv_wgrad_bnin(dy, N, Hq, Wq, Cout, ld_dy, x, H, W, Cin, ld_x, taps, in_stride, dw, dw_ld_tap, dw_ld_co, dw_ld_ci, bn_in,
+                    on_dy):
+    d = _bn_operand(bn_in, on_dy)
+    with _timed_conv(2.0 * N * Hq * Wq * len(taps[0]) * Cin * Cout) as tc:
+        rc = lib().jvae_conv_wgrad_bnin(rawptr(dy), N, Hq, Wq, Cout, ld_dy, rawptr(x), H, W, Cin, ld_x, len(taps[0]), taps[0],
+                                        taps[1], in_stride, rawptr(dw), dw_ld_tap, dw_ld_co, dw_ld_ci, ctypes.byref(d), stream())
+        if rc == NOT_COVERED:
+            tc.cancel()
+    if rc == NOT_COVERED:
+        return False
+    check(rc)
+    return True
+
+
+def bn_finalize(stats, P, C, gamma, beta, eps, momentum, running_mean, running_var, num_batches, save, ss):
+    check(lib().jvae_bn_finalize(rawptr(stats), P, C, rawptr(gamma), rawptr(beta), float(eps), float(momentum),
+                                 rawptr(running_mean), rawptr(running_var), rawptr(num_batches), rawptr(save), rawptr(ss),
+                                 stream()))
+
+
+def bn_apply_scaled(y, P, C, ld_y, ss, act, out, ld_out):
+    check(lib().jvae_bn_apply_scaled(rawptr(y), P, C, ld_y, rawptr(ss), act, rawptr(out), ld_out, stream()))
+
+
 def bn_stats(y, P, C, ld, stats):
     check(lib().jvae_bn_stats(rawptr(y), P, C, ld, rawptr(stats), stream()))
 
diff --git a/joint-vae_b200/conv_engine.py b/joint-vae_b200/conv_engine.py
--- a/joint-vae_b200/conv_engine.py
+++ b/joint-vae_b200/conv_engine.py
@@ -26,6 +26,7 @@
 DENSE_SMALL = _os.environ.get('JVAE_CONV_DENSE_SMALL', '0') == '1'
 SEP_FWD_DIRECT = _os.environ.get('JVAE_HEAD_FWD_DIRECT', '1') != '0'
 IM2COL_MAXPIX = int(_os.environ.get('JVAE_CONV_IM2COL_MAXPIX', '16'))
+BN_ON_LOAD = _os.environ.get('JVAE_BN_ON_LOAD', '1') != '0'
 
 
 class NativeKernels:
@@ -55,19 +56,27 @@
         return nat.nhwc_bf16_to_nchw(t, C)
 
     @staticmethod
-    def gather(x, Cin, wmat, cout_pad, taps, in_stride, Hq, Wq, out, Cout, out_s, out_o, bias, act, stats, bn=None):
+    def gather(x, Cin, wmat, cout_pad, taps, in_stride, Hq, Wq, out, Cout, out_s, out_o, bias, act, stats, bn=None, bn_in=None):
         N, H, W, ld_in = x.shape
         _, Ho, Wo, ld_out = out.shape
+        if bn_in is not None:
+            return nat.conv_gather_gemm_bnin(x, N, H, W, Cin, ld_in, wmat, cout_pad, wmat.shape[1], taps, in_stride, Hq, Wq, out,
+                                             Ho, Wo, Cout, ld_out, out_s, out_o, bias, act, stats, bn_in)
         return nat.conv_gather_gemm(x, N, H, W, Cin, ld_in, wmat, cout_pad, wmat.shape[1], taps, in_stride, Hq, Wq, out, Ho,
                                     Wo, Cout, ld_out, out_s, out_o, bias, act, stats, bn=bn)
 
     @staticmethod
-    def wgrad(g, Cg, x, Cx, taps, in_stride, dw, swapped=False):
+    def wgrad(g, Cg, x, Cx, taps, in_stride, dw, swapped=False, bn_in=None, on_dy=0):
         N, Hq, Wq, ld_g = g.shape
         _, H, W, ld_x = x.shape
         T = len(taps[0])
         P = N * Hq * Wq
         small = Hq * Wq <= IM2COL_MAXPIX and Cx % 8 == 0 and Cg >= 128 and Cx >= 64 and T in (1, 4, 9, 25)
+        if bn_in is not None:
+            if not swapped and small and dw.is_contiguous():
+                return False
+            lds = (1, T, Cg * T) if swapped else (1, Cx * T, T)
+            return nat.conv_wgrad_bnin(g, N, Hq, Wq, Cg, ld_g, x, H, W, Cx, ld_x, taps, in_stride, dw, *lds, bn_in, on_dy)
         if not swapped and small and dw.is_contiguous():
             cols = torch.empty((P, Cx * T), dtype=torch.bfloat16, device=g.device)
             nat.im2col(x, N, H, W, Cx, ld_x, taps, in_stride, Hq, Wq, cols)
@@ -75,11 +84,12 @@
             ksplit = max(1, min(nat.sm_count() // tiles, (P + 511) // 512)) if tiles < 100 else 1
             nat.gemm_bf16(2, Cg, Cx * T, P, g.view(P, ld_g), ld_g, cols, Cx * T, out_f32=dw.view(Cg, Cx * T), ldd=Cx * T,
                           accumulate=ksplit if ksplit > 1 else True)
-            return
+            return True
         if swapped:
             nat.conv_wgrad(g, N, Hq, Wq, Cg, ld_g, x, H, W, Cx, ld_x, taps, in_stride, dw, 1, T, Cg * T)
         else:
             nat.conv_wgrad(g, N, Hq, Wq, Cg, ld_g, x, H, W, Cx, ld_x, taps, in_stride, dw, 1, Cx * T, T)
+        return True
 
     @staticmethod
     def gemm(mode, M, N, K, a, b, bias=None, act=0, out_bf16=None, out_f32=None):
@@ -91,14 +101,19 @@
         return nat.phases_arg(ops)
 
     @staticmethod
-    def subpixel(x, Cin, wmat, cout_pad, phases, Hq, Wq, out, Cout, out_s, bias, act, stats):
+    def subpixel(x, Cin, wmat, cout_pad, phases, Hq, Wq, out, Cout, out_s, bias, act, stats, bn_in=None):
         N, H, W, ld_in = x.shape
         _, Ho, Wo, ld_out = out.shape
+        if bn_in is not None:
+            return nat.conv_subpixel_gemm_bnin(x, N, H, W, Cin, ld_in, wmat, cout_pad, wmat.shape[1], phases, Hq, Wq, out, Ho, Wo,
+                                               Cout, ld_out, out_s, bias, act, stats, bn_in)
         return nat.conv_subpixel_gemm(x, N, H, W, Cin, ld_in, wmat, cout_pad, wmat.shape[1], phases, Hq, Wq, out, Ho, Wo, Cout,
                                       ld_out, out_s, bias, act, stats)
 
     bn_stats = staticmethod(nat.bn_stats)
     bn_apply_fwd = staticmethod(nat.bn_apply_fwd)
+    bn_finalize = staticmethod(nat.bn_finalize)
+    bn_apply_scaled = staticmethod(nat.bn_apply_scaled)
     bn_bwd = staticmethod(nat.bn_bwd)
     act_bwd = staticmethod(nat.act_bwd)
     maxpool_fwd = staticmethod(nat.maxpool_fwd)
@@ -426,7 +441,31 @@
         setattr(self, slot, (key, d))
         return d
 
-    def forward(self, x, st, training):
+    def takes_bn_on_load(self):
+        if self.gemm1x1 or self.dense_small or (self.separable and not SEP_FWD_DIRECT):
+            return False
+        return self.merged_fwd or (len(self.fwd_ops) == 1 and self.fwd_ops[0]['in_stride'] == 1)
+
+    @staticmethod
+    def materialise(y, x_bn):
+        N, H, W, ld = y.shape
+        a = K.empty(y.shape, y)
+        K.bn_apply_scaled(y, N * H * W, x_bn['C'], ld, x_bn['ss'], x_bn['act'], a, ld)
+        return a
+
+    def _forward_bn_on_load(self, y_in, x_bn, pk, out, bias, act, stats):
+        if self.merged_fwd:
+            ph = self._ctaps.get('fa')
+            if ph is None:
+                ph = self._ctaps['fa'] = K.phases_arg(self.fwd_ops)
+            wm, op = pk['fwd_all'], self.fwd_ops[0]
+            return K.subpixel(y_in, self.Ci, wm, wm.shape[0], ph, op['Hq'], op['Wq'], out, self.Co, self.s, bias, act, stats,
+                              bn_in=x_bn)
+        op, wm = self.fwd_ops[0], pk['fwd'][0]
+        return K.gather(y_in, self.Ci, wm, wm.shape[0], self._taps(('f', 0), op['taps']), op['in_stride'], op['Hq'], op['Wq'],
+                        out, self.Co, op['out_s'], op['out_o'], bias, act, stats, bn_in=x_bn)
+
+    def forward(self, x, st, training, x_bn=None, defer=False):
         N = x.shape[0]
         bn = self.bn
         bn_train = bn is not None and (training or not bn.track_running_stats)
@@ -439,7 +478,12 @@
         stats = (st.pop('stats_buf', None) if bn_train else None)
         if bn_train and stats is None:
             stats = K.zeros((2, self.Co), x, torch.float64)
-        if self.gemm1x1:
+        on_load = x_bn is not None and self._forward_bn_on_load(x, x_bn, pk, y, bias, fused_act, stats)
+        if x_bn is not None and not on_load:
+            x, x_bn = self.materialise(x, x_bn), None
+        if on_load:
+            st['x_bn'] = x_bn
+        elif self.gemm1x1:
             kk = self.k * self.k
             a2 = x.view(N, x.shape[-1])
             K.gemm(nat.GEMM_NT, N, kk * self.Co, self.Ci, a2, pk['bm'], bias=pk['bias'], act=fused_act,
@@ -463,9 +507,19 @@
             st['a'] = y
             return y
         P = N * self.Ho * self.Wo
-        a = K.empty((N, self.Ho, self.Wo, self.ld_a), x)
         save = K.empty((2, self.Co), x, torch.float32) if bn_train else None
         track = bn.track_running_stats and training
+        if defer and bn_train and self.act == 1 and self.ld_a == self.ld_y:
+            ss = K.empty((2, self.Co), x, torch.float32)
+            K.bn_finalize(stats, P, self.Co, bn.weight.detach() if bn.affine else None, bn.bias.detach() if bn.affine else None,
+                          bn.eps, bn.momentum if bn.momentum is not None else 0.1, bn.running_mean if track else None,
+                          bn.running_var if track else None, bn.num_batches_tracked if track else None, save, ss)
+            if track:
+                engine.bump_stats()
+            st['y'], st['save'], st['bn_train'] = y, save, bn_train
+            st['defer'] = dict(ss=ss, act=self.act, C=self.Co)
+            return y
+        a = K.empty((N, self.Ho, self.Wo, self.ld_a), x)
         K.bn_apply_fwd(y, P, self.Co, self.ld_y, stats, bn.weight.detach() if bn.affine else None,
                        bn.bias.detach() if bn.affine else None, bn.eps, bn.momentum if bn.momentum is not None else 0.1,
                        bn.running_mean if track or not bn_train else None, bn.running_var if track or not bn_train else None,
@@ -517,6 +571,11 @@
 
     def backward(self, da, st, need_dx, prev_bn=None):
         x = st['x']
+        x_bn = st.get('x_bn')
+
+        def wgrad_x(launch, on_dy=0):
+            if x_bn is None or not launch(x, bn_in=x_bn, on_dy=on_dy):
+                launch(x if x_bn is None else self.materialise(x, x_bn))
         N = x.shape[0]
         P = N * self.Ho * self.Wo
         bn = self.bn
@@ -604,9 +663,11 @@
             if not folded:
                 dwa = K.zeros((self.sep_C, self.Ci, kq), x)
                 if cblk_of(self.sep_C) < cblk_of(min(self.Ci, 64)):
-                    K.wgrad(x, self.Ci, U, self.sep_C, self._taps('sb', self.sep_bwd_taps), 1, dwa, swapped=True)
+                    wgrad_x(lambda xi, **b: K.wgrad(xi, self.Ci, U, self.sep_C, self._taps('sb', self.sep_bwd_taps), 1, dwa,
+                                                  swapped=True, **b), on_dy=1)
                 else:
-                    K.wgrad(U, self.sep_C, x, self.Ci, self._taps('sf', self.sep_fwd_taps), 1, dwa)
+                    wgrad_x(lambda xi, **b: K.wgrad(U, self.sep_C, xi, self.Ci, self._taps('sf', self.sep_fwd_taps), 1, dwa,
+                                                  **b))
                 upd = dwa.view(kq, self.Co, self.Ci, kq).permute(1, 2, 0, 3)
                 live = _live_grad(self.conv.weight, x)
                 if live is not None:
@@ -623,12 +684,14 @@
                 live = _live_grad(w, x)
                 dw = live if live is not None else K.zeros(tuple(w.shape), x)
                 if self.transposed:
-                    K.wgrad(x, self.Ci, dy, self.Co, self._taps('w', self.wgrad_taps), self.s, dw.view(self.Ci, self.Co, kk))
+                    wgrad_x(lambda xi, **b: K.wgrad(xi, self.Ci, dy, self.Co, self._taps('w', self.wgrad_taps), self.s,
+                                                  dw.view(self.Ci, self.Co, kk), **b), on_dy=1)
                 elif self.wgrad_swapped:
-                    K.wgrad(x, self.Ci, dy, self.Co, self._taps('wn', self.wgrad_taps_neg), 1, dw.view(self.Co, self.Ci, kk),
-                            swapped=True)
+                    wgrad_x(lambda xi, **b: K.wgrad(xi, self.Ci, dy, self.Co, self._taps('wn', self.wgrad_taps_neg), 1,
+                                                  dw.view(self.Co, self.Ci, kk), swapped=True, **b), on_dy=1)
                 else:
-                    K.wgrad(dy, self.Co, x, self.Ci, self._taps('w', self.wgrad_taps), self.s, dw.view(self.Co, self.Ci, kk))
+                    wgrad_x(lambda xi, **b: K.wgrad(dy, self.Co, xi, self.Ci, self._taps('w', self.wgrad_taps), self.s,
+                                                  dw.view(self.Co, self.Ci, kk), **b))
                 grads['w'] = None if live is not None else dw
             if need_dx:
                 dx = K.zeros(x.shape, x, torch.bfloat16) if self.dgrad_sparse else K.empty(x.shape, x)
@@ -911,12 +974,19 @@
         pool, off = None, 0
         if bn_steps:
             pool = K.zeros((sum(2 * s.Co for s in bn_steps),), t, torch.float64)
-        for s in self.steps:
+        x_bn = None
+        for i, s in enumerate(self.steps):
             st = {}
             if pool is not None and any(s is b for b in bn_steps):
                 st['stats_buf'] = pool[off:off + 2 * s.Co].view(2, s.Co)
                 off += 2 * s.Co
-            t = s.forward(t, st, training)
+            if isinstance(s, ConvStep):
+                nxt = self.steps[i + 1] if i + 1 < len(self.steps) else None
+                defer = BN_ON_LOAD and K is NativeKernels and training and isinstance(nxt, ConvStep) and nxt.takes_bn_on_load()
+                t = s.forward(t, st, training, x_bn=x_bn, defer=defer)
+                x_bn = st.pop('defer', None)
+            else:
+                t = s.forward(t, st, training)
             state.append(st)
         Co, Ho, Wo = self.out_shape
         if self.image_out and t.shape[-1] == Co:
diff --git a/joint-vae_b200/csrc/common.cuh b/joint-vae_b200/csrc/common.cuh
--- a/joint-vae_b200/csrc/common.cuh
+++ b/joint-vae_b200/csrc/common.cuh
@@ -76,6 +76,13 @@
   return *reinterpret_cast<uint32_t*>(&t);
 }
 
+__device__ __forceinline__ float act_fwd(float z, int act) {
+  if (act == JVAE_ACT_RELU) return fmaxf(z, 0.f);
+  if (act == JVAE_ACT_SIGMOID) return 1.f / (1.f + __expf(-z));
+  if (act == JVAE_ACT_LEAKY) return z > 0.f ? z : JVAE_LEAKY_SLOPE * z;
+  return z;
+}
+
 __device__ __forceinline__ uint4 ld_stream16(const void* p) {
   uint4 r;
   asm volatile("ld.global.nc.L1::no_allocate.v4.u32 {%0,%1,%2,%3}, [%4];"
diff --git a/joint-vae_b200/csrc/conv.cu b/joint-vae_b200/csrc/conv.cu
--- a/joint-vae_b200/csrc/conv.cu
+++ b/joint-vae_b200/csrc/conv.cu
@@ -278,6 +278,8 @@
   const __nv_bfloat16* bn_y;
   const float* bn_save; const float* bn_gamma; const float* bn_beta;
   int bn_ld, bn_act;
+  const float* in_ss;
+  int Cin;
   uint32_t stage_bytes, box_bytes, w_tap_bytes, w_bytes, tmem_cols, acc_stride;
   int stages, resident, wstages;
   int G, nck;
@@ -297,6 +299,30 @@
   uint64_t d;
   asm("mov.b64 %0, {%1, %2};" : "=l"(d) : "r"(lo), "r"(hi));
   return d;
+}
+
+__device__ __forceinline__ void bn_on_load(uint32_t base, uint32_t beg, uint32_t end, uint32_t rb, const float* s_scale,
+                                           const float* s_shift, int c0, int tid, int nthr) {
+  const uint32_t o0 = beg + 16u * (uint32_t)tid;
+  const int c = c0 + (int)((((o0 >> 4) ^ (o0 >> 7)) & (rb / 16u - 1u)) * 8u);
+  float sc[8], sh[8];
+#pragma unroll
+  for (int j = 0; j < 8; ++j) { sc[j] = s_scale[c + j]; sh[j] = s_shift[c + j]; }
+#pragma unroll 2
+  for (uint32_t o = o0; o < end; o += 16u * (uint32_t)nthr) {
+    uint32_t w[4];
+    asm volatile("ld.shared.v4.u32 {%0, %1, %2, %3}, [%4];" : "=r"(w[0]), "=r"(w[1]), "=r"(w[2]), "=r"(w[3]) : "r"(base + o));
+#pragma unroll
+    for (int i = 0; i < 4; ++i) {
+      const float y0 = bf16_lo(w[i]), y1 = bf16_hi(w[i]);
+      float z0 = act_fwd(fmaf(y0, sc[2 * i], sh[2 * i]), JVAE_ACT_RELU);
+      float z1 = act_fwd(fmaf(y1, sc[2 * i + 1], sh[2 * i + 1]), JVAE_ACT_RELU);
+      if (y0 != y0) z0 = 0.f;
+      if (y1 != y1) z1 = 0.f;
+      w[i] = pack_bf16(z0, z1);
+    }
+    asm volatile("st.shared.v4.u32 [%0], {%1, %2, %3, %4};" :: "r"(base + o), "r"(w[0]), "r"(w[1]), "r"(w[2]), "r"(w[3]) : "memory");
+  }
 }
 
 template <int KSTEPS, int MT>
@@ -351,7 +377,8 @@
 template <int NCH, int MODE>
 __device__ __forceinline__ void halo_epilogue_fast(const HaloParams& p, uint32_t tmem_base, uint64_t* tfull_bar, uint64_t* tempty_bar,
                                                    double* s_stats, const float* s_bias, const float* s_bn, int2* s_tab, int warp,
-                                                   int lane, int nt, int box0, int box_step) {
+                                                   int lane, int nt, int box0, int box_step, uint32_t smem_base,
+                                                   uint64_t* full_bar, uint64_t* ready_bar) {
   constexpr bool STATS = MODE != 0;
   constexpr bool BNRED = MODE == 2;
   constexpr int LC = (NCH + 1) / 2;
@@ -384,6 +411,22 @@
   const bool vec_bf16 = (p.ldc & 7) == 0, vec_f32 = (p.ldc & 3) == 0;
   const bool al32 = (reinterpret_cast<uintptr_t>(p.out) & 31) == 0;
   const bool v8_bf16 = al32 && (p.ldc & 15) == 0, v8_f32 = al32 && (p.ldc & 7) == 0;
+  uint32_t xu = 0;
+  auto transform_box = [&]() {
+    const uint32_t per_plane = p.box_bytes / (uint32_t)p.nplanes, rb = (uint32_t)p.Cblk * 2u;
+    for (int kc = 0; kc < p.nkc; ++kc, ++xu) {
+      const uint32_t s = xu % (uint32_t)p.stages;
+      mbar_wait(&full_bar[s], (xu / (uint32_t)p.stages) & 1u);
+      for (int pl = 0; pl < p.nplanes; ++pl) {
+        const uint32_t beg = s * p.stage_bytes + (uint32_t)pl * p.plane_bytes;
+        bn_on_load(smem_base, beg, beg + per_plane, rb, s_bn, s_bn + 128, kc * p.Cblk, (int)threadIdx.x - 64, 256);
+      }
+      fence_proxy_async();
+      __syncwarp();
+      if (lane == 0) mbar_arrive(&ready_bar[s]);
+    }
+  };
+  if (p.in_ss && box0 < p.num_boxes) transform_box();
   uint32_t it = 0;
   int sx, by, mm, dsx, dby, dmm;
   {
@@ -403,6 +446,7 @@
       if (by >= p.blocks_y) { by -= p.blocks_y; ++mm; }
       mm += dmm;
     }
+    if (p.in_ss && box + box_step < p.num_boxes) transform_box();
     const int qx = sx * 8 + (mrow & 7);
     const bool pxok = qx < p.Wq;
     const int ylim = p.Hq - by * p.RT, nlim = p.N - mm * p.NBt;
@@ -582,7 +626,8 @@
   uint64_t* wempty_bar = wfull_bar + 8;
   uint64_t* tfull_bar = wempty_bar + 8;
   uint64_t* tempty_bar = tfull_bar + 2;
-  uint32_t* tmem_slot = reinterpret_cast<uint32_t*>(tempty_bar + 2);
+  uint64_t* ready_bar = tempty_bar + 2;
+  uint32_t* tmem_slot = reinterpret_cast<uint32_t*>(ready_bar + 4);
   double* s_stats = reinterpret_cast<double*>(tmem_slot + 4);
   float* s_bias = reinterpret_cast<float*>(s_stats + (p.stats ? 2 * p.cout_pad : 0));
 
@@ -600,6 +645,11 @@
       s_bn[i] = mean; s_bn[64 + i] = rstd; s_bn[128 + i] = live ? g * rstd : 0.f; s_bn[192 + i] = live ? b - mean * g * rstd : 0.f;
     }
   }
+  if (p.in_ss)
+    for (int i = threadIdx.x; i < 128; i += HALO_THREADS) {
+      s_bn[i] = i < p.Cin ? p.in_ss[i] : 0.f;
+      s_bn[128 + i] = i < p.Cin ? p.in_ss[p.Cin + i] : 0.f;
+    }
   const int box0 = (int)blockIdx.x / p.n_tiles_n, box_step = (int)gridDim.x / p.n_tiles_n;
   const uint32_t rb = (uint32_t)p.Cblk * 2u;
 
@@ -611,6 +661,7 @@
     for (int s = 0; s < 4; ++s) { mbar_init(&full_bar[s], 1); mbar_init(&empty_bar[s], 1); }
     for (int s = 0; s < 8; ++s) { mbar_init(&wfull_bar[s], 1); mbar_init(&wempty_bar[s], 1); }
     for (int a = 0; a < 2; ++a) { mbar_init(&tfull_bar[a], 1); mbar_init(&tempty_bar[a], 8); }
+    for (int s = 0; s < 4; ++s) mbar_init(&ready_bar[s], 8);
     fence_barrier_init();
     fence_proxy_async();
   }
@@ -675,7 +726,7 @@
         const uint32_t d0 = tmem_base + acc * p.acc_stride;
         const uint32_t b_lo = ((smem_u32(wsm) >> 4) & 0x3fffu) | (1u << 16);
         for (int kc = 0; kc < p.nkc; ++kc) {
-          mbar_wait(&full_bar[s], sph);
+          mbar_wait(p.in_ss ? &ready_bar[s] : &full_bar[s], sph);
           tc_fence_after();
           const uint32_t a_lo0 = ((smem_u32(smem + (size_t)s * p.stage_bytes) >> 4) & 0x3fffu) | (1u << 16);
           const uint32_t later = kc != 0;
@@ -704,10 +755,12 @@
       }
     }
   } else {
-#define HALO_EPI_FAST(NCH_)                                                                                                            \
-    if (p.bn_y) halo_epilogue_fast<NCH_, 2>(p, tmem_base, tfull_bar, tempty_bar, s_stats, s_bias, s_bn, s_tab, warp, lane, nt, box0, box_step);    \
-    else if (p.stats) halo_epilogue_fast<NCH_, 1>(p, tmem_base, tfull_bar, tempty_bar, s_stats, s_bias, s_bn, s_tab, warp, lane, nt, box0, box_step); \
-    else halo_epilogue_fast<NCH_, 0>(p, tmem_base, tfull_bar, tempty_bar, s_stats, s_bias, s_bn, s_tab, warp, lane, nt, box0, box_step)
+    const uint32_t sbase = smem_u32(smem);
+#define HALO_EPI_ARGS p, tmem_base, tfull_bar, tempty_bar, s_stats, s_bias, s_bn, s_tab, warp, lane, nt, box0, box_step, sbase, full_bar, ready_bar
+#define HALO_EPI_FAST(NCH_)                                                              \
+    if (p.bn_y) halo_epilogue_fast<NCH_, 2>(HALO_EPI_ARGS);                              \
+    else if (p.stats) halo_epilogue_fast<NCH_, 1>(HALO_EPI_ARGS);                        \
+    else halo_epilogue_fast<NCH_, 0>(HALO_EPI_ARGS)
     switch (p.BN >> 4) {
       case 1: HALO_EPI_FAST(1); break;
       case 2: HALO_EPI_FAST(2); break;
@@ -715,6 +768,7 @@
       default: HALO_EPI_FAST(4); break;
     }
 #undef HALO_EPI_FAST
+#undef HALO_EPI_ARGS
   }
   tc_fence_before();
   __syncthreads();
@@ -859,6 +913,8 @@
   unsigned short grp_col[WH_MAX_GROUPS];
   short grp_tap[WH_MAX_GROUPS][8][8];
   uint32_t g_gap_bytes;
+  const float* bn_ss;
+  int bn_on, bn_C;
   float* dw;
   int dw_ld_tap, dw_ld_co, dw_ld_cx;
   uint32_t x_stage_bytes, stage_bytes, x_box_bytes, g_box_bytes, tmem_cols;
@@ -872,8 +928,10 @@
   uint8_t* smem = reinterpret_cast<uint8_t*>((reinterpret_cast<uintptr_t>(smem_raw) + 1023) & ~(uintptr_t)1023);
   uint64_t* full_bar = reinterpret_cast<uint64_t*>(smem + (size_t)p.stages * p.stage_bytes);
   uint64_t* empty_bar = full_bar + 8;
-  uint64_t* done_bar = empty_bar + 8;
+  uint64_t* ready_bar = empty_bar + 8;
+  uint64_t* done_bar = ready_bar + 8;
   uint32_t* tmem_slot = reinterpret_cast<uint32_t*>(done_bar + 1);
+  float* s_ss = reinterpret_cast<float*>(tmem_slot + 4);
   const int warp = threadIdx.x >> 5, lane = threadIdx.x & 31;
   const int g_lo = (int)blockIdx.y * p.groups_per_cta;
   const int ng = min(p.groups_per_cta, p.ngroups - g_lo);
@@ -885,10 +943,17 @@
   if (warp == 0 && lane == 0) {
     tma_prefetch_desc(&tmap_g);
     tma_prefetch_desc(&tmap_x);
-    for (int s = 0; s < 8; ++s) { mbar_init(&full_bar[s], 1); mbar_init(&empty_bar[s], 1); }
+    for (int s = 0; s < 8; ++s) { mbar_init(&full_bar[s], 1); mbar_init(&empty_bar[s], 1); mbar_init(&ready_bar[s], 4); }
     mbar_init(done_bar, 1);
     fence_barrier_init();
   }
+  const int bn_c0 = p.bn_on == 1 ? cx0 : cg0;
+  if (p.bn_on)
+    for (int i = threadIdx.x; i < 64; i += CONV_THREADS) {
+      const int ch = bn_c0 + i;
+      s_ss[i] = ch < p.bn_C ? p.bn_ss[ch] : 0.f;
+      s_ss[64 + i] = ch < p.bn_C ? p.bn_ss[p.bn_C + ch] : 0.f;
+    }
   fence_proxy_async();
   if (warp == 1) tmem_alloc_dyn(tmem_slot, p.tmem_cols);
   tc_fence_before();
@@ -931,7 +996,7 @@
       const uint32_t ey_slots16 = ((uint32_t)p.ey * 8u * rbg) >> 4;
       uint32_t s = 0, ph = 0, first = 0;
       for (int box = blockIdx.x; box < p.num_boxes; box += gridDim.x) {
-        mbar_wait(&full_bar[s], ph);
+        mbar_wait(p.bn_on ? &ready_bar[s] : &full_bar[s], ph);
         tc_fence_after();
         const uint32_t sx_ = smem_u32(smem + (size_t)s * p.stage_bytes);
         const uint32_t a_lo0 = ((sx_ >> 4) & 0x3fffu) | a_lbo;
@@ -957,6 +1022,27 @@
     }
   } else {
     const int q = warp & 3;
+    if (p.bn_on) {
+      const uint32_t base = smem_u32(smem);
+      uint32_t s = 0, ph = 0;
+      for (int box = blockIdx.x; box < p.num_boxes; box += gridDim.x) {
+        mbar_wait(&full_bar[s], ph);
+        if (p.bn_on == 1) {
+          const uint32_t per_plane = p.x_box_bytes / (uint32_t)p.nplanes;
+          for (int pl = 0; pl < p.nplanes; ++pl) {
+            const uint32_t beg = s * p.stage_bytes + (uint32_t)pl * p.plane_bytes;
+            bn_on_load(base, beg, beg + per_plane, rbx, s_ss, s_ss + 64, 0, (int)threadIdx.x - 64, 128);
+          }
+        } else {
+          const uint32_t beg = s * p.stage_bytes + p.x_stage_bytes + p.g_gap_bytes;
+          bn_on_load(base, beg, beg + p.g_box_bytes, rbg, s_ss, s_ss + 64, 0, (int)threadIdx.x - 64, 128);
+        }
+        fence_proxy_async();
+        __syncwarp();
+        if (lane == 0) mbar_arrive(&ready_bar[s]);
+        if (++s == (uint32_t)p.stages) { s = 0; ph ^= 1; }
+      }
+    }
     mbar_wait(done_bar, 0);
     tc_fence_after();
     const bool has_work = (int)blockIdx.x < p.num_boxes;
@@ -1018,8 +1104,9 @@
                            int Ho, int Wo, int Cout, int ld_out, int out_sy, int out_sx, int out_oy, int out_ox,
                            const float* bias, int act, double* stats, const jvae_bn_reduce* bn, int* bn_fused,
                            cudaStream_t stream, const PhaseSpec* phs = nullptr, HaloParams* plan_out = nullptr,
-                           int force_cblk = 0, double* score_out = nullptr) {
+                           int force_cblk = 0, double* score_out = nullptr, const jvae_bn_operand* bn_in = nullptr) {
   if (Wq < 6) return 1;
+  if (bn_in && (bn_in->act != JVAE_ACT_RELU || in_stride != 1 || Cin > 128 || bn)) return 1;
   const bool wide = Cin > 64 || Cout_pad > 64;
   if (phs && (wide || in_stride != 1 || phs->n < 2 || phs->n > 4 || bn)) return 1;
   if (wide) {
@@ -1033,15 +1120,17 @@
     HaloParams pa, pb;
     double sa = 0.0, sb = 0.0;
     const int ra = try_launch_halo(in, N, H, W, Cin, ld_in, wmat, Cout_pad, ldw, ntaps, tap_dy, tap_dx, in_stride, Hq, Wq, out, Ho, Wo,
-                                   Cout, ld_out, out_sy, out_sx, out_oy, out_ox, bias, act, stats, bn, nullptr, stream, nullptr, &pa, 64, &sa);
+                                   Cout, ld_out, out_sy, out_sx, out_oy, out_ox, bias, act, stats, bn, nullptr, stream, nullptr, &pa, 64, &sa, bn_in);
     const int rb2 = try_launch_halo(in, N, H, W, Cin, ld_in, wmat, Cout_pad, ldw, ntaps, tap_dy, tap_dx, in_stride, Hq, Wq, out, Ho, Wo,
-                                    Cout, ld_out, out_sy, out_sx, out_oy, out_ox, bias, act, stats, bn, nullptr, stream, nullptr, &pb, 32, &sb);
+                                    Cout, ld_out, out_sy, out_sx, out_oy, out_ox, bias, act, stats, bn, nullptr, stream, nullptr, &pb, 32, &sb, bn_in);
     if (ra < 0) return ra;
     const int pick = (rb2 == 0 && (ra != 0 || sb > 1.15 * sa)) ? 32 : 64;
     if (score_out) *score_out = pick == 32 ? sb : sa;
     return try_launch_halo(in, N, H, W, Cin, ld_in, wmat, Cout_pad, ldw, ntaps, tap_dy, tap_dx, in_stride, Hq, Wq, out, Ho, Wo, Cout,
-                           ld_out, out_sy, out_sx, out_oy, out_ox, bias, act, stats, bn, bn_fused, stream, nullptr, plan_out, pick, nullptr);
-  }
+                           ld_out, out_sy, out_sx, out_oy, out_ox, bias, act, stats, bn, bn_fused, stream, nullptr, plan_out, pick, nullptr,
+                           bn_in);
+  }
+  if (bn_in && wide) return 1;
   HaloParams p;
   memset(&p, 0, sizeof(p));
   p.PH = 1;
@@ -1289,6 +1378,7 @@
   p.out_sy = out_sy; p.out_sx = out_sx; p.out_oy = out_oy; p.out_ox = out_ox;
   p.act = act & 0xff; p.out_f32 = (act & JVAE_OUT_F32) ? 1 : 0;
   p.bias = bias; p.out = reinterpret_cast<__nv_bfloat16*>(out); p.stats = stats; p.cout_pad = Cout_pad;
+  if (bn_in) { p.in_ss = bn_in->scale_shift; p.Cin = Cin; }
   if (plan_out) { *plan_out = p; return JVAE_OK; }
   CUtensorMap tin, tw;
   if (bn) {
@@ -1303,7 +1393,7 @@
     uint32_t box[4] = {(uint32_t)p.Cblk, (uint32_t)(p.HWp * st), (uint32_t)(p.HHs * st), (uint32_t)p.NBt};
     uint32_t es[4] = {1u, (uint32_t)st, (uint32_t)st, 1u};
     if (box[1] > 256 || box[2] > 256) return 1;
-    int rc = make_tmap_bf16(&tin, in, 4, dims, strides, box, es, p.Cblk * 2);
+    int rc = make_tmap_bf16(&tin, in, 4, dims, strides, box, es, p.Cblk * 2, bn_in != nullptr);
     if (rc) return rc;
     const int Ktot = ntaps * p.nkc * p.Cblk;
     uint64_t wd[2] = {(uint64_t)Ktot, (uint64_t)Cout_pad};
@@ -1336,8 +1426,10 @@
 static int try_launch_wgrad_halo(const void* g, int N, int Hq, int Wq, int Cg, int ld_g, const void* x, int H, int W, int Cx,
                                  int ld_x, int ntaps, const int16_t* tap_dy, const int16_t* tap_dx, int in_stride, float* dw,
                                  int dw_ld_tap, int dw_ld_co, int dw_ld_cx, cudaStream_t stream, const int* tap_ids = nullptr,
-                                 bool dry_run = false, WHaloParams* plan_out = nullptr) {
+                                 bool dry_run = false, WHaloParams* plan_out = nullptr,
+                                 const jvae_bn_operand* bn_in = nullptr) {
   if (Wq < 6) return 1;
+  if (bn_in && bn_in->act != JVAE_ACT_RELU) return 1;
   WHaloParams p;
   memset(&p, 0, sizeof(p));
   const int st = in_stride;
@@ -1472,6 +1564,10 @@
   p.strips_x = (Wq + 7) / 8;
   p.num_boxes = p.strips_x * p.blocks_y * ((N + p.NBt - 1) / p.NBt);
   p.dw = dw; p.dw_ld_tap = dw_ld_tap; p.dw_ld_co = dw_ld_co; p.dw_ld_cx = dw_ld_cx;
+  if (bn_in) {
+    if (bn_in->on_dy && p.blocks_y != 1) return 1;
+    p.bn_ss = bn_in->scale_shift; p.bn_on = bn_in->on_dy ? 2 : 1; p.bn_C = bn_in->on_dy ? Cg : Cx;
+  }
   if (plan_out) *plan_out = p;
   if (dry_run) return JVAE_OK;
   CUtensorMap tg, tx;
@@ -1479,14 +1575,14 @@
     uint64_t dg[4] = {(uint64_t)Cg, (uint64_t)Wq, (uint64_t)Hq, (uint64_t)N};
     uint64_t sg[3] = {(uint64_t)ld_g * 2, (uint64_t)Wq * ld_g * 2, (uint64_t)Hq * Wq * ld_g * 2};
     uint32_t bg[4] = {(uint32_t)p.Cblk_g, 8u, (uint32_t)(p.blocks_y == 1 ? p.HHs : p.RT), (uint32_t)(p.blocks_y == 1 ? p.NBt : 1)};
-    int rc = make_tmap_bf16(&tg, g, 4, dg, sg, bg, nullptr, p.Cblk_g * 2);
+    int rc = make_tmap_bf16(&tg, g, 4, dg, sg, bg, nullptr, p.Cblk_g * 2, p.bn_on == 2);
     if (rc) return rc;
     uint64_t dx[4] = {(uint64_t)Cx, (uint64_t)W, (uint64_t)H, (uint64_t)N};
     uint64_t sx[3] = {(uint64_t)ld_x * 2, (uint64_t)W * ld_x * 2, (uint64_t)H * W * ld_x * 2};
     uint32_t bx[4] = {(uint32_t)p.Cblk_x, (uint32_t)(p.HWp * st), (uint32_t)(p.HHs * st), (uint32_t)p.NBt};
     uint32_t esx[4] = {1u, (uint32_t)st, (uint32_t)st, 1u};
     if (bx[1] > 256 || bx[2] > 256) return 1;
-    rc = make_tmap_bf16(&tx, x, 4, dx, sx, bx, esx, p.Cblk_x * 2);
+    rc = make_tmap_bf16(&tx, x, 4, dx, sx, bx, esx, p.Cblk_x * 2, p.bn_on == 1);
     if (rc) return rc;
   }
   const int nz = ncg * p.ncx;
@@ -1494,7 +1590,7 @@
   int gx = (sm_count() + ysplit * nz - 1) / (ysplit * nz);
   if (gx < 1) gx = 1;
   if (gx > p.num_boxes) gx = p.num_boxes;
-  const size_t smem = (size_t)p.stages * p.stage_bytes + 256 + 1024;
+  const size_t smem = (size_t)p.stages * p.stage_bytes + 256 + 1024 + (p.bn_on ? 512 : 0);
   static bool attr = false;
   if (!attr) {
     JVAE_CUDA(cudaFuncSetAttribute(conv_wgrad_halo_kernel, cudaFuncAttributeMaxDynamicSharedMemorySize, 227 * 1024));
@@ -1672,11 +1768,43 @@
   return JVAE_OK;
 }
 
+int jvae_conv_gather_gemm_bnin(const void* in, int N, int H, int W, int Cin, int ld_in, const void* wmat, int Cout_pad, int ldw,
+                               int ntaps, const int16_t* tap_dy, const int16_t* tap_dx, int in_stride, int Hq, int Wq,
+                               void* out, int Ho, int Wo, int Cout, int ld_out, int out_sy, int out_sx, int out_oy, int out_ox,
+                               const float* bias, int act, double* stats, const jvae_bn_operand* bn_in, void* stream) {
+  if (!bn_in)
+    return jvae_conv_gather_gemm(in, N, H, W, Cin, ld_in, wmat, Cout_pad, ldw, ntaps, tap_dy, tap_dx, in_stride, Hq, Wq, out, Ho, Wo,
+                                 Cout, ld_out, out_sy, out_sx, out_oy, out_ox, bias, act, stats, stream);
+  JVAE_CHECK_ARG(in && wmat && out && tap_dy && tap_dx && bn_in->scale_shift, "null pointer");
+  JVAE_CHECK_ARG(ntaps >= 1 && ntaps <= CONV_MAX_TAPS, "1..64 taps");
+  JVAE_CHECK_ARG((ld_in % 8) == 0 && (ldw % 8) == 0, "input / weight channel strides must be multiples of 8");
+  JVAE_CHECK_ARG(ld_out >= Cout, "ld_out < Cout");
+  JVAE_CHECK_ARG((Cout_pad % 16) == 0 && Cout_pad >= 16 && Cout_pad >= Cout, "Cout_pad must be a multiple of 16, >= Cout");
+  JVAE_CHECK_ARG(!stats || Cout_pad <= 2048, "statistics epilogue supports up to 2048 channels");
+  JVAE_CHECK_ARG(in_stride == 1 || in_stride == 2, "input stride 1 or 2");
+  JVAE_CHECK_ARG((((uintptr_t)in | (uintptr_t)wmat | (uintptr_t)out) & 15) == 0, "16-byte alignment");
+  if (getenv("JVAE_CONV_V1") != nullptr) return JVAE_NOT_COVERED;
+  const int rc = try_launch_halo(in, N, H, W, Cin, ld_in, wmat, Cout_pad, ldw, ntaps, tap_dy, tap_dx, in_stride, Hq, Wq, out, Ho, Wo,
+                                 Cout, ld_out, out_sy, out_sx, out_oy, out_ox, bias, act, stats, nullptr, nullptr,
+                                 (cudaStream_t)stream, nullptr, nullptr, 0, nullptr, bn_in);
+  return rc > 0 ? JVAE_NOT_COVERED : rc;
+}
+
 int jvae_conv_subpixel_gemm(const void* in, int N, int H, int W, int Cin, int ld_in, const void* wmat, int Cout_pad, int ldw,
                             int nphases, const int16_t* phase_ntaps, const int16_t* phase_oy, const int16_t* phase_ox,
                             const int16_t* tap_dy, const int16_t* tap_dx, int Hq, int Wq, void* out, int Ho, int Wo, int Cout,
                             int ld_out, int out_s, const float* bias, int act, double* stats, void* stream) {
+  return jvae_conv_subpixel_gemm_bnin(in, N, H, W, Cin, ld_in, wmat, Cout_pad, ldw, nphases, phase_ntaps, phase_oy, phase_ox, tap_dy,
+                                      tap_dx, Hq, Wq, out, Ho, Wo, Cout, ld_out, out_s, bias, act, stats, nullptr, stream);
+}
+
+int jvae_conv_subpixel_gemm_bnin(const void* in, int N, int H, int W, int Cin, int ld_in, const void* wmat, int Cout_pad, int ldw,
+                                 int nphases, const int16_t* phase_ntaps, const int16_t* phase_oy, const int16_t* phase_ox,
+                                 const int16_t* tap_dy, const int16_t* tap_dx, int Hq, int Wq, void* out, int Ho, int Wo, int Cout,
+                                 int ld_out, int out_s, const float* bias, int act, double* stats, const jvae_bn_operand* bn_in,
+                                 void* stream) {
   JVAE_CHECK_ARG(in && wmat && out && tap_dy && tap_dx && phase_ntaps && phase_oy && phase_ox, "null pointer");
+  JVAE_CHECK_ARG(!bn_in || bn_in->scale_shift, "null pointer");
   JVAE_CHECK_ARG(nphases >= 1 && nphases <= 4, "1..4 phases");
   int ntaps = 0;
   for (int i = 0; i < nphases; ++i) {
@@ -1694,21 +1822,30 @@
   if (off) return JVAE_NOT_COVERED;
   PhaseSpec ps = {nphases, phase_ntaps, phase_oy, phase_ox};
   const int rc = try_launch_halo(in, N, H, W, Cin, ld_in, wmat, Cout_pad, ldw, ntaps, tap_dy, tap_dx, 1, Hq, Wq, out, Ho, Wo, Cout,
-                                 ld_out, out_s, out_s, 0, 0, bias, act, stats, nullptr, nullptr, (cudaStream_t)stream, &ps);
+                                 ld_out, out_s, out_s, 0, 0, bias, act, stats, nullptr, nullptr, (cudaStream_t)stream, &ps, nullptr, 0,
+                                 nullptr, bn_in);
   return rc > 0 ? JVAE_NOT_COVERED : rc;
 }
 
 int jvae_conv_wgrad(const void* dy, int N, int Hq, int Wq, int Cout, int ld_dy, const void* x, int H, int W, int Cin, int ld_x,
                     int ntaps, const int16_t* tap_dy, const int16_t* tap_dx, int in_stride, float* dw, int dw_ld_tap,
                     int dw_ld_co, int dw_ld_ci, void* stream) {
+  return jvae_conv_wgrad_bnin(dy, N, Hq, Wq, Cout, ld_dy, x, H, W, Cin, ld_x, ntaps, tap_dy, tap_dx, in_stride, dw, dw_ld_tap, dw_ld_co,
+                              dw_ld_ci, nullptr, stream);
+}
+
+int jvae_conv_wgrad_bnin(const void* dy, int N, int Hq, int Wq, int Cout, int ld_dy, const void* x, int H, int W, int Cin, int ld_x,
+                         int ntaps, const int16_t* tap_dy, const int16_t* tap_dx, int in_stride, float* dw, int dw_ld_tap,
+                         int dw_ld_co, int dw_ld_ci, const jvae_bn_operand* bn_in, void* stream) {
   JVAE_CHECK_ARG(dy && x && dw && tap_dy && tap_dx, "null pointer");
+  JVAE_CHECK_ARG(!bn_in || bn_in->scale_shift, "null pointer");
   JVAE_CHECK_ARG(ntaps >= 1 && ntaps <= CONV_MAX_TAPS, "1..64 taps");
   JVAE_CHECK_ARG((ld_dy % 8) == 0 && (ld_x % 8) == 0, "channel strides must be multiples of 8");
   JVAE_CHECK_ARG(in_stride == 1 || in_stride == 2, "input stride 1 or 2");
   static const bool force_v1 = getenv("JVAE_CONV_V1") != nullptr;
   if (!force_v1) {
     const int rc = try_launch_wgrad_halo(dy, N, Hq, Wq, Cout, ld_dy, x, H, W, Cin, ld_x, ntaps, tap_dy, tap_dx, in_stride, dw,
-                                         dw_ld_tap, dw_ld_co, dw_ld_ci, (cudaStream_t)stream);
+                                         dw_ld_tap, dw_ld_co, dw_ld_ci, (cudaStream_t)stream, nullptr, false, nullptr, bn_in);
     if (rc <= 0) return rc;
     static const bool split_off = getenv("JVAE_WGRAD_PLANE_SPLIT") && atoi(getenv("JVAE_WGRAD_PLANE_SPLIT")) == 0;
     if (in_stride == 2 && !split_off) {
@@ -1724,13 +1861,14 @@
           if (ids[pl].empty()) continue;
           const int r2 = try_launch_wgrad_halo(dy, N, Hq, Wq, Cout, ld_dy, x, H, W, Cin, ld_x, (int)ids[pl].size(), sdy[pl].data(),
                                                sdx[pl].data(), 2, dw, dw_ld_tap, dw_ld_co, dw_ld_ci, (cudaStream_t)stream,
-                                               ids[pl].data(), pass == 0);
+                                               ids[pl].data(), pass == 0, nullptr, bn_in);
           if (r2 < 0) return r2;
           if (r2 > 0) { covered = false; break; }
         }
       if (covered) return JVAE_OK;
     }
   }
+  if (bn_in) return JVAE_NOT_COVERED;
   WgradParams p;
   memset(&p, 0, sizeof(p));
   p.N = N; p.Hq = Hq; p.Wq = Wq;
diff --git a/joint-vae_b200/csrc/gemm.cu b/joint-vae_b200/csrc/gemm.cu
--- a/joint-vae_b200/csrc/gemm.cu
+++ b/joint-vae_b200/csrc/gemm.cu
@@ -219,7 +219,7 @@
 }
 
 int make_tmap_bf16(CUtensorMap* out, const void* base, int rank, const uint64_t* dims, const uint64_t* strides_bytes,
-                   const uint32_t* box, const uint32_t* elem_strides, int swizzle_bytes) {
+                   const uint32_t* box, const uint32_t* elem_strides, int swizzle_bytes, bool oob_nan) {
   auto enc = get_tmap_encode();
   if (!enc) {
     set_error("cuTensorMapEncodeTiled is not available from this driver");
@@ -239,7 +239,7 @@
   }
   CUresult r = enc(out, CU_TENSOR_MAP_DATA_TYPE_BFLOAT16, (cuuint32_t)rank, const_cast<void*>(base), gd, gs, bx, es,
                    CU_TENSOR_MAP_INTERLEAVE_NONE, sw, CU_TENSOR_MAP_L2_PROMOTION_L2_256B,
-                   CU_TENSOR_MAP_FLOAT_OOB_FILL_NONE);
+                   oob_nan ? CU_TENSOR_MAP_FLOAT_OOB_FILL_NAN_REQUEST_ZERO_FMA : CU_TENSOR_MAP_FLOAT_OOB_FILL_NONE);
   if (r != CUDA_SUCCESS) {
     set_error("cuTensorMapEncodeTiled failed (CUresult %d): rank %d dims [%llu,%llu,..] stride0 %llu box [%u,%u,..]", (int)r,
               rank, (unsigned long long)dims[0], (unsigned long long)(rank > 1 ? dims[1] : 0),
diff --git a/joint-vae_b200/csrc/norm.cu b/joint-vae_b200/csrc/norm.cu
--- a/joint-vae_b200/csrc/norm.cu
+++ b/joint-vae_b200/csrc/norm.cu
@@ -56,12 +56,6 @@
   return g;
 }
 
-__device__ __forceinline__ float act_fwd(float z, int act) {
-  if (act == JVAE_ACT_RELU) return fmaxf(z, 0.f);
-  if (act == JVAE_ACT_SIGMOID) return 1.f / (1.f + __expf(-z));
-  if (act == JVAE_ACT_LEAKY) return z > 0.f ? z : JVAE_LEAKY_SLOPE * z;
-  return z;
-}
 __device__ __forceinline__ float act_grad_z(float z, int act) {
   if (act == JVAE_ACT_RELU) return z > 0.f ? 1.f : 0.f;
   if (act == JVAE_ACT_SIGMOID) { const float s = 1.f / (1.f + __expf(-z)); return s * (1.f - s); }
@@ -143,7 +137,43 @@
   const double* stats; const float* gamma; const float* beta;
   float* running_mean; float* running_var; long long* num_batches; float* save;
   float eps, momentum;
+  const float* ss;
+  float* ss_out;
 };
+
+__device__ __forceinline__ void bn_scale_shift(const BnFwd& a, int c, bool owner, float& scale, float& shift) {
+  float mean, rstd;
+  if (a.training) {
+    const double inv = 1.0 / (double)a.P;
+    const double mean_d = a.stats[c] * inv;
+    mean = (float)mean_d;
+    const float var = fmaxf((float)(a.stats[a.C + c] * inv - mean_d * mean_d), 0.f);
+    rstd = rsqrtf(var + a.eps);
+    if (owner) {
+      a.save[c] = mean; a.save[a.C + c] = rstd;
+      if (a.running_mean) {
+        const float unb = a.P > 1 ? var * (float)a.P / (float)(a.P - 1) : var;
+        a.running_mean[c] = (1.f - a.momentum) * a.running_mean[c] + a.momentum * mean;
+        a.running_var[c] = (1.f - a.momentum) * a.running_var[c] + a.momentum * unb;
+      }
+    }
+  } else {
+    mean = a.running_mean[c];
+    rstd = rsqrtf(a.running_var[c] + a.eps);
+  }
+  const float g = a.gamma ? a.gamma[c] : 1.f, b = a.beta ? a.beta[c] : 0.f;
+  scale = g * rstd;
+  shift = b - mean * scale;
+}
+
+__global__ void bn_finalize_kernel(const BnFwd a) {
+  for (int c = threadIdx.x; c < a.C; c += blockDim.x) {
+    float scale, shift;
+    bn_scale_shift(a, c, true, scale, shift);
+    a.ss_out[c] = scale; a.ss_out[a.C + c] = shift;
+  }
+  if (a.num_batches && threadIdx.x == 0) *a.num_batches += 1;
+}
 
 template <int V>
 __global__ void __launch_bounds__(NORM_MAX_THREADS) bn_apply_fwd_kernel(const BnFwd a) {
@@ -152,30 +182,10 @@
 #pragma unroll
   for (int j = 0; j < V; ++j) {
     const int c = chunk * V + j;
-    float mean, rstd;
-    if (a.training) {
-      const double inv = 1.0 / (double)a.P;
-      const double mean_d = a.stats[c] * inv;
-      mean = (float)mean_d;
-      const float var = fmaxf((float)(a.stats[a.C + c] * inv - mean_d * mean_d), 0.f);
-      rstd = rsqrtf(var + a.eps);
-      if (blockIdx.x == 0 && pl == 0) {
-        a.save[c] = mean; a.save[a.C + c] = rstd;
-        if (a.running_mean) {
-          const float unb = a.P > 1 ? var * (float)a.P / (float)(a.P - 1) : var;
-          a.running_mean[c] = (1.f - a.momentum) * a.running_mean[c] + a.momentum * mean;
-          a.running_var[c] = (1.f - a.momentum) * a.running_var[c] + a.momentum * unb;
-        }
-      }
-    } else {
-      mean = a.running_mean[c];
-      rstd = rsqrtf(a.running_var[c] + a.eps);
-    }
-    const float g = a.gamma ? a.gamma[c] : 1.f, b = a.beta ? a.beta[c] : 0.f;
-    scale[j] = g * rstd;
-    shift[j] = b - mean * scale[j];
-  }
-  if (a.training && a.num_batches && blockIdx.x == 0 && threadIdx.x == 0) *a.num_batches += 1;
+    if (a.ss) { scale[j] = a.ss[c]; shift[j] = a.ss[a.C + c]; }
+    else bn_scale_shift(a, c, blockIdx.x == 0 && pl == 0, scale[j], shift[j]);
+  }
+  if (!a.ss && a.training && a.num_batches && blockIdx.x == 0 && threadIdx.x == 0) *a.num_batches += 1;
   constexpr int U = 4;
   const size_t step = (size_t)gridDim.x * a.ppb;
   for (size_t p0 = (size_t)blockIdx.x * a.ppb + pl; p0 < a.P; p0 += U * step) {
@@ -345,30 +355,10 @@
   for (int c = 0; c < 8; ++c) {
     scale[c] = shift[c] = 0.f;
     if (c >= a.C) continue;
-    float mean, rstd;
-    if (a.training) {
-      const double inv = 1.0 / (double)a.P;
-      const double mean_d = a.stats[c] * inv;
-      mean = (float)mean_d;
-      const float var = fmaxf((float)(a.stats[a.C + c] * inv - mean_d * mean_d), 0.f);
-      rstd = rsqrtf(var + a.eps);
-      if (blockIdx.x == 0 && threadIdx.x == 0) {
-        a.save[c] = mean; a.save[a.C + c] = rstd;
-        if (a.running_mean) {
-          const float unb = a.P > 1 ? var * (float)a.P / (float)(a.P - 1) : var;
-          a.running_mean[c] = (1.f - a.momentum) * a.running_mean[c] + a.momentum * mean;
-          a.running_var[c] = (1.f - a.momentum) * a.running_var[c] + a.momentum * unb;
-        }
-      }
-    } else {
-      mean = a.running_mean[c];
-      rstd = rsqrtf(a.running_var[c] + a.eps);
-    }
-    const float g = a.gamma ? a.gamma[c] : 1.f, b = a.beta ? a.beta[c] : 0.f;
-    scale[c] = g * rstd;
-    shift[c] = b - mean * scale[c];
-  }
-  if (a.training && a.num_batches && blockIdx.x == 0 && threadIdx.x == 0) *a.num_batches += 1;
+    if (a.ss) { scale[c] = a.ss[c]; shift[c] = a.ss[a.C + c]; }
+    else bn_scale_shift(a, c, blockIdx.x == 0 && threadIdx.x == 0, scale[c], shift[c]);
+  }
+  if (!a.ss && a.training && a.num_batches && blockIdx.x == 0 && threadIdx.x == 0) *a.num_batches += 1;
   constexpr int U = 4;
   const size_t step = (size_t)gridDim.x * blockDim.x;
   for (size_t p0 = (size_t)blockIdx.x * blockDim.x + threadIdx.x; p0 < a.P; p0 += U * step) {
@@ -984,11 +974,11 @@
   return JVAE_OK;
 }
 
-int jvae_bn_apply_fwd(const void* y, size_t P, int C, int ld_y, const double* stats, const float* gamma, const float* beta,
-                      float eps, float momentum, float* running_mean, float* running_var, int64_t* num_batches, int training,
-                      int act, void* out, int ld_out, float* save_mean_rstd, void* stream) {
+static int bn_apply(const void* y, size_t P, int C, int ld_y, const double* stats, const float* gamma, const float* beta,
+                    float eps, float momentum, float* running_mean, float* running_var, int64_t* num_batches, int training,
+                    int act, void* out, int ld_out, float* save_mean_rstd, const float* scale_shift, void* stream) {
   JVAE_CHECK_ARG(y && out && P > 0 && C > 0 && ld_y >= C && ld_out >= C, "bad arguments");
-  JVAE_CHECK_ARG(training ? (stats && save_mean_rstd) : (running_mean && running_var), "statistics missing");
+  JVAE_CHECK_ARG(scale_shift || (training ? (stats && save_mean_rstd) : (running_mean && running_var)), "statistics missing");
   const bool vec = vec_ok(C, {ld_y, ld_out}, {y, out});
   JVAE_CHECK_ARG(vec ? C <= 8 * NORM_MAX_THREADS : C <= NORM_MAX_THREADS, "too many channels for this layout");
   const Geo g = make_geo(P, C, vec ? 8 : 1);
@@ -999,6 +989,7 @@
   a.P = P; a.C = C; a.ld_y = ld_y; a.ld_out = ld_out; a.nchunk = g.nchunk; a.ppb = g.ppb; a.act = act; a.training = training;
   a.stats = stats; a.gamma = gamma; a.beta = beta; a.running_mean = running_mean; a.running_var = running_var;
   a.num_batches = reinterpret_cast<long long*>(num_batches); a.save = save_mean_rstd; a.eps = eps; a.momentum = momentum;
+  a.ss = scale_shift; a.ss_out = nullptr;
   if (narrow) {
     const int want = (int)((P + NORM_MAX_THREADS * 4 - 1) / (NORM_MAX_THREADS * 4));
     const int cap = sm_count() * 8;
@@ -1007,6 +998,34 @@
     return JVAE_OK;
   }
   NORM_DISPATCH(vec, bn_apply_fwd_kernel, g, 0, (cudaStream_t)stream, a);
+  return JVAE_OK;
+}
+
+int jvae_bn_apply_fwd(const void* y, size_t P, int C, int ld_y, const double* stats, const float* gamma, const float* beta,
+                      float eps, float momentum, float* running_mean, float* running_var, int64_t* num_batches, int training,
+                      int act, void* out, int ld_out, float* save_mean_rstd, void* stream) {
+  return bn_apply(y, P, C, ld_y, stats, gamma, beta, eps, momentum, running_mean, running_var, num_batches, training, act, out,
+                  ld_out, save_mean_rstd, nullptr, stream);
+}
+
+int jvae_bn_apply_scaled(const void* y, size_t P, int C, int ld_y, const float* scale_shift, int act, void* out, int ld_out,
+                         void* stream) {
+  JVAE_CHECK_ARG(scale_shift, "null pointer");
+  return bn_apply(y, P, C, ld_y, nullptr, nullptr, nullptr, 0.f, 0.f, nullptr, nullptr, nullptr, 1, act, out, ld_out, nullptr,
+                  scale_shift, stream);
+}
+
+int jvae_bn_finalize(const double* stats, size_t P, int C, const float* gamma, const float* beta, float eps, float momentum,
+                     float* running_mean, float* running_var, int64_t* num_batches, float* save_mean_rstd, float* scale_shift,
+                     void* stream) {
+  JVAE_CHECK_ARG(stats && save_mean_rstd && scale_shift && P > 0 && C > 0, "bad arguments");
+  BnFwd a;
+  memset(&a, 0, sizeof(a));
+  a.P = P; a.C = C; a.training = 1; a.stats = stats; a.gamma = gamma; a.beta = beta; a.running_mean = running_mean;
+  a.running_var = running_var; a.num_batches = reinterpret_cast<long long*>(num_batches); a.save = save_mean_rstd; a.eps = eps;
+  a.momentum = momentum; a.ss_out = scale_shift;
+  bn_finalize_kernel<<<1, C < 1024 ? ((C + 31) & ~31) : 1024, 0, (cudaStream_t)stream>>>(a);
+  JVAE_LAUNCH_CHECK();
   return JVAE_OK;
 }
 
diff --git a/joint-vae_b200/csrc/tc_common.cuh b/joint-vae_b200/csrc/tc_common.cuh
--- a/joint-vae_b200/csrc/tc_common.cuh
+++ b/joint-vae_b200/csrc/tc_common.cuh
@@ -147,6 +147,6 @@
 
 PFN_cuTensorMapEncodeTiled_v12000 get_tmap_encode();
 int make_tmap_bf16(CUtensorMap* out, const void* base, int rank, const uint64_t* dims, const uint64_t* strides_bytes,
-                   const uint32_t* box, const uint32_t* elem_strides, int swizzle_bytes);
+                   const uint32_t* box, const uint32_t* elem_strides, int swizzle_bytes, bool oob_nan = false);
 
 }
```

Result: no change. 46180, median of 6 (+0.4%).
